# adelacvg/NS2VC

Measured on AMD Instinct MI355X. Metric: denoiser-steps/sec (10s@24kHz Vocos latent, bs32), higher is better.
Workload: dtype fp16; 1 GPU; 10 s utterance (T=938 Vocos frames), batch 32/GPU, prompt Lp=469, 20-step unipc order 2, hipGraph-captured loop, fp16 MFMA operands; timed job = set_condition + 20 steps; global_batch=32, frames=938, prompt_frames=469, solver=unipc, parallelism=dp1

## Files before the change

### include/ns2vc_hip.h

```cpp
#ifndef NS2VC_HIP_H
#define NS2VC_HIP_H

#include <stddef.h>
#include <stdint.h>

#ifdef __cplusplus
extern "C" {
#endif

#define NS2VC_ABI_VERSION 7
#define NS2VC_MAX_LEVELS 8
#define NS2VC_NCOEF 12

typedef struct ns2vc_unet ns2vc_unet;

typedef struct ns2vc_unet_cfg {
  int32_t latent_channels;
  int32_t content_channels;
  int32_t n_levels;
  int32_t block_out_channels[NS2VC_MAX_LEVELS];
  int32_t norm_num_groups;
  int32_t cross_attention_dim;
  int32_t heads;
  int32_t layers_per_block;
// ... 34 lines not shown
int ns2vc_unet_set_condition(ns2vc_unet* h, const float* content_bct, const float* prompt_blc, const uint8_t* mask_bl, void* stream);
int ns2vc_unet_set_content(ns2vc_unet* h, const float* content_bct, void* stream);
int ns2vc_unet_set_prompt(ns2vc_unet* h, const float* prompt_blc, const uint8_t* mask_bl, void* stream);
int ns2vc_unet_set_mask(ns2vc_unet* h, const uint8_t* mask_bl, void* stream);
int ns2vc_unet_set_lengths(ns2vc_unet* h, const int32_t* lengths_b, void* stream);
int ns2vc_unet_set_prompt_lengths(ns2vc_unet* h, const int32_t* plens_b, void* stream);

int ns2vc_unet_forward(ns2vc_unet* h, const float* x_bct, const float* t_b, float* out_bct, void* stream);

int ns2vc_sampler_load(ns2vc_unet* h, int steps, const float* coef_host);
int ns2vc_sampler_load_items(ns2vc_unet* h, int n_tables, const int32_t* table_rows, const float* coef_host, int n_items, const int32_t* item_table,
                             const int32_t* item_start, void* stream);
int ns2vc_sampler_run(ns2vc_unet* h, float* x_inout_bct, int use_graph, void* stream);
int ns2vc_sampler_begin(ns2vc_unet* h, const float* x_T_bct, void* stream);
int ns2vc_sampler_steps(ns2vc_unet* h, int n_steps, int use_graph, void* stream);
int ns2vc_sampler_end(ns2vc_unet* h, float* x_out_bct, void* stream);
int ns2vc_sampler_handoff(ns2vc_unet* dst, ns2vc_unet* src, void* stream);
int ns2vc_sampler_set_seeds(ns2vc_unet* h, const uint64_t* seeds_b, void* stream);
int ns2vc_sampler_set_guidance(ns2vc_unet* h, const float* scale_host, int n, void* stream);
int ns2vc_sampler_set_x0_correction(ns2vc_unet* h, int mode, float ratio, float max_val);
int ns2vc_sampler_peek(ns2vc_unet* h, float* x_out_bct, void* stream);
int ns2vc_unet_attn_fallbacks(ns2vc_unet* h, unsigned long long* count, int reset, void* stream);
int ns2vc_unet_gn_coop_alone(ns2vc_unet* h, unsigned long long* count, int reset, void* stream);
int ns2vc_unet_graph_captures(ns2vc_unet* h, unsigned long long* count);

int ns2vc_unet_set_debug(ns2vc_unet* h, int enable);
int ns2vc_unet_num_taps(ns2vc_unet* h);
int ns2vc_unet_tap_info(ns2vc_unet* h, int idx, char* name, int buflen, int* rows, int* cols);
int ns2vc_unet_tap_read(ns2vc_unet* h, int idx, float* host_dst);
int ns2vc_unet_num_launches(ns2vc_unet* h, int* per_forward, int* per_condition);
int ns2vc_unet_op_info(ns2vc_unet* h, int which, int idx, char* name, int buflen, int* kind, double* flops, double* bytes);
int ns2vc_unet_profile_forward(ns2vc_unet* h, float* ms, int n_ms, int reps, void* stream);

int ns2vc_dev_malloc(void** out, size_t bytes);
int ns2vc_dev_free(void* p);
int ns2vc_memcpy_h2d(void* dst, const void* src, size_t bytes);
int ns2vc_memcpy_d2h(void* dst, const void* src, size_t bytes);
int ns2vc_dev_sync(void);
int ns2vc_stream_create(void** out);
int ns2vc_stream_destroy(void* stream);
int ns2vc_stream_sync(void* stream);
int ns2vc_stream_create_cu_mask(void** out, const uint32_t* mask_words, int n_words);
int ns2vc_event_create(void** out);
int ns2vc_event_destroy(void* ev);
int ns2vc_event_record(void* ev, void* stream);
int ns2vc_event_elapsed_ms(void* start, void* stop, float* ms);

typedef struct ns2vc_gemm_args {
  const void* a0; const void* a1;
  int32_t lda0, lda1, c0, c1;
  int32_t B, Tin, Tout, M;
  int32_t taps, tmode;
  const void* w; int32_t K;
  int32_t N;
  const float* bias;
  const float* res; int32_t ldres;
  int32_t geglu;
  float* out_f32; int32_t ldo_f32;
  void* out_op; int32_t ldo_op;
  long long* stats;
  const void* a2; int32_t lda2, c2;
  float* rowstats;
  const float* ln_stats; const float* ln_wsum; float ln_eps; int32_t ln_dim;
  unsigned* ln_health;
  const float* gnp_x; int32_t gnp_ldx;
  const long long* gnp_stats; const float* gnp_gamma; const float* gnp_beta;
  const float* gnp_temb; int32_t gnp_ldtemb;
  float gnp_eps; int32_t gnp_G, gnp_silu;
  unsigned* gnp_sync;
  unsigned* gnp_alone;
  const float* gnp_x1; int32_t gnp_ldx1, gnp_c1;
  const long long* gnp_stats1;
  void* gnp_raw;
  int32_t algo;
  const void* w_tiled;
  const float* sol_coef; const int32_t* sol_step; int32_t sol_ncoef;
  float* sol_xe; void* sol_xe_op; float* sol_xbar; float* sol_d1; float* sol_mprev; int32_t sol_ld;
  int32_t conv_bn;
  int32_t gnp_pair, sol_op_pair;
  const int32_t* lens;
} ns2vc_gemm_args;

typedef struct ns2vc_attn_args {
  const void* q; const void* k; const void* v;
  int32_t ldq, ldk, ldv;
  int32_t B, H, Lq, Lk;
  const float* bias;
  float scale;
  void* out; int32_t ldo;
  int32_t pv_fp8;
  int32_t exact_only;
  unsigned* fallbacks;
  const int32_t* q_lens;
  const int32_t* k_lens;
} ns2vc_attn_args;

typedef struct ns2vc_ffn_args {
  const void* yn; int32_t ldy;
  const float* ln_stats; float ln_eps;
  const void* wstream; const float* consts; const float* bias2;
  const float* res; int32_t ldres;
  float* out_f32; int32_t ldo_f32;
  void* out_op; int32_t ldo_op;
  long long* stats;
  int32_t B, T, M, dim;
  unsigned* ln_health;
  const void* pre_a; int32_t pre_lda;
  const float* pre_bias;
  const float* pre_res; int32_t pre_ldres;
  const void* att_q; int32_t att_ldq;
  const void* att_kv; const float* att_bias; float att_scale; int32_t att_Lk;
  const int32_t* lens;
} ns2vc_ffn_args;
int ns2vc_pack_ffn(const float* w1_packed_host, const float* w2f_host, int dim, int precision, void** out_stream_dev);
int ns2vc_pack_ffn_pre(const float* w1_packed_host, const float* w2f_host, const float* w0_host, int dim, int precision, void** out_stream_dev);
int ns2vc_k_ffn(const ns2vc_ffn_args* a, int precision, void* stream);
size_t ns2vc_xattn_pack_bytes(int B, int Lk, int hd);
int ns2vc_k_xattn_pack(const void* k, int ldk, const void* v, int ldv, int B, int Lk, int hd, void* out, int precision, void* stream);

typedef struct ns2vc_geglu_args {
  const void* yn; int32_t ldy;
  const float* ln_stats; float ln_eps;
  const void* wstream; const float* consts;
  void* out_op; int32_t ldo;
  int32_t M, dim;
  unsigned* ln_health;
  int32_t T;
  const int32_t* lens;
} ns2vc_geglu_args;
int ns2vc_pack_geglu(const float* w1_packed_host, const float* bias1_packed_host, int dim, int precision, void** out_stream_dev, float** out_consts_dev);
int ns2vc_k_geglu(const ns2vc_geglu_args* a, int precision, void* stream);
int ns2vc_pack_geglu_host(const float* w1_packed_host, const float* bias1_packed_host, int dim, int precision, uint16_t* stream_out, float* consts_out);

typedef struct ns2vc_rowchain_args {
  const void* a_op; int32_t lda;
  const void* wstream; const float* bias1; const float* consts2;
  const float* res; int32_t ldres;
  float* out1_f32; int32_t ldo1;
  void* out2_op; int32_t ldo2;
  float ln_eps; int32_t M, dim, n2;
  unsigned* ln_health;
  const float* gn_x; int32_t ldx;
  const long long* gn_stats; const float* gn_gamma; const float* gn_beta;
  float gn_eps; int32_t T, G;
  int32_t slices;
  const int32_t* lens;
} ns2vc_rowchain_args;
int ns2vc_pack_rowchain(const float* w1_host, const float* w2_host, int dim, int n2, int precision, void** out_stream_dev);
int ns2vc_pack_rowchain_sliced(const float* w1_host, const float* w2_host, int dim, int n2, int slices, int precision, void** out_stream_dev);
int ns2vc_k_rowchain(const ns2vc_rowchain_args* a, int precision, void* stream);
int ns2vc_debug_set_geglu_min_rows(int rows);
int ns2vc_debug_set_attn_keys(int keys);
int ns2vc_debug_set_attn_optimistic(int on);
int ns2vc_debug_set_rowchain_tokens(int nt);

int ns2vc_to_operand(const float* host, size_t n, int precision, void** out_dev);
int ns2vc_from_operand(const void* dev, size_t n, int precision, float* host);
int ns2vc_round_to_operand(const float* host_in, size_t n, int precision, float* host_out);
int ns2vc_pack_weight(const float* rows_host, int N, int K, int precision, void** out_dev);
int ns2vc_k_gemm(const ns2vc_gemm_args* a, int precision, void* stream);
int ns2vc_pack_conv3_tiled(const float* rows_host, int N, int ctot, int c2, int precision, void** out_dev);
int ns2vc_weight_rowsum(const float* rows_host, int N, int K, int precision, float** out_dev);
int ns2vc_debug_set_gemm_trace(void* dev_u64_blocks_x8);
int ns2vc_debug_poison(unsigned pattern, int lds_bytes, void* stream);
int ns2vc_debug_placement(void* stream, int n_blocks, int spin, uint32_t* out_host);
int ns2vc_debug_kernel_table(int family, int* rows, int* unready);
int ns2vc_debug_set_gemm_tile(int bm, int bn, int stages);
int ns2vc_k_attention(const ns2vc_attn_args* a, int head_dim, int precision, void* stream);
int ns2vc_k_groupnorm(const float* a0, int lda0, int c0, const float* a1, int lda1, int c1, int B, int T, int G, float eps,
                      const float* gamma, const float* beta, const float* temb, int ldtemb, int temb_off, int silu,
                      void* out_op, void* raw_op, int precision, void* stream);
int ns2vc_k_groupnorm_stats(const float* a0, int lda0, int c0, const long long* stats0, int B, int T, int G, float eps, const float* gamma,
                            const float* beta, const float* temb, int ldtemb, int temb_off, int silu, void* out_op, int precision, void* stream);
int ns2vc_k_groupnorm_stats2(const float* a0, int lda0, int c0, const long long* stats0, const float* a1, int lda1, int c1, const long long* stats1,
                             int B, int T, int G, float eps, const float* gamma, const float* beta, const float* temb, int ldtemb, int temb_off,
                             int silu, void* out_op, void* raw_op, int precision, void* stream);
int ns2vc_k_layernorm_apply(const float* x, int ldx, int M, int C, float eps, void* out_op, int precision, void* stream);
int ns2vc_k_nct_to_btc(const float* src, int C, int T, int B, float* dst, int ldd, int cpad, void* stream);
int ns2vc_k_btc_to_nct(const float* src, int lds, int C, int T, int B, float* dst, void* stream);
int ns2vc_k_noise(const uint64_t* seeds_dev, int B, int C, int T, int ld, int step, const int32_t* lens_dev, float* out, void* stream);
int ns2vc_k_solver_update(const float* coef_dev, const int32_t* step_dev, const float* x0, float* xe, void* xe_op, int precision, float* xbar,
                          float* d1, float* mprev, float* mprev2, size_t n, int ld, void* stream);
int ns2vc_k_solver_update_guided(const float* coef_dev, const int32_t* step_dev, const float* x0, float* xe, void* xe_op, int precision, float* xbar,
                                 float* d1, float* mprev, float* mprev2, size_t n_half, int ld, const float* scale_dev, int T, const uint64_t* seeds_dev,
                                 const int32_t* lens_dev, int nc, void* stream);
int ns2vc_k_abs_quantile(const float* values, int n_items, int T, int ld, int nc, const int32_t* lens_dev, float p, float* thr, void* stream);
int ns2vc_k_solver_update_corrected(const float* coef_dev, const int32_t* step_dev, const float* x0, float* xe, void* xe_op, int precision, float* xbar,
                                    float* d1, float* mprev, float* mprev2, size_t n, int ld, int T, const float* scale_dev, const int32_t* lens_dev,
                                    int nc, int mode, float ratio, float max_val, float* thr_dev, void* stream);
int ns2vc_k_solver_update_items(const float* coef_dev, int n_rows, const int32_t* step_dev, const int32_t* items_host, int n_items, const float* x0, float* xe,
                                void* xe_op, int precision, float* xbar, float* d1, float* mprev, float* mprev2, size_t n, int ld, int T,
                                const float* scale_dev, const uint64_t* seeds_dev, const int32_t* lens_dev, int nc, int mode, float ratio, float max_val,
                                float* thr_dev, void* stream);

int ns2vc_sampler_open(ns2vc_unet* h, int history2, int noise, void* stream);
int ns2vc_sampler_rebase(ns2vc_unet* h, void* stream);
int ns2vc_sampler_write_rows(ns2vc_unet* h, int row0, int nrows, const float* coef_host, void* stream);
int ns2vc_sampler_admit(ns2vc_unet* h, int n, const int32_t* slots, const float* x_T_nct, const int32_t* records, void* stream);
int ns2vc_sampler_take(ns2vc_unet* h, int n, const int32_t* slots, float* x_out_nct, void* stream);
int ns2vc_sampler_slot_step(ns2vc_unet* h, int* loop_step);
int ns2vc_unet_set_condition_items(ns2vc_unet* h, int n, const int32_t* slots, const float* content_nct, const float* prompt_nlc, const uint8_t* mask_nl,
                                   void* stream);
int ns2vc_k_sampler_admit(const float* x_T, int C, int T, int n, const int32_t* slots_host, int n_items, float* xe, void* xe_op, int precision, float* xbar,
                          float* d1, float* mprev, float* mprev2, int ld, const int32_t* lens_dev, int guided, void* stream);
int ns2vc_k_sampler_take(const float* xe, int ld, int C, int T, int n, const int32_t* slots_host, int n_items, float* out, void* stream);

#ifdef __cplusplus
}
#endif
#endif
```

### ns2vc_amd/_lib.py

```python
from __future__ import annotations

import ctypes as C
import os
from typing import Optional

_HERE = os.path.dirname(os.path.abspath(__file__))
LIB_PATH = os.path.join(_HERE, "lib", "libns2vc_hip.so")
NCOEF = 12
MAX_LEVELS = 8
PREC_F32, PREC_BF16, PREC_F16 = 0, 1, 2
ABI_VERSION = 7


class Ns2vcError(RuntimeError):
    pass


class UnetCfg(C.Structure):
    _fields_ = [
        ("latent_channels", C.c_int32), ("content_channels", C.c_int32), ("n_levels", C.c_int32),
        ("block_out_channels", C.c_int32 * MAX_LEVELS), ("norm_num_groups", C.c_int32),
        ("cross_attention_dim", C.c_int32), ("heads", C.c_int32), ("layers_per_block", C.c_int32),
        ("pool_heads", C.c_int32),
    ]
# ... 32 lines not shown
class FfnArgs(C.Structure):
    _fields_ = [
        ("yn", C.c_void_p), ("ldy", C.c_int32),
        ("ln_stats", C.c_void_p), ("ln_eps", C.c_float),
        ("wstream", C.c_void_p), ("consts", C.c_void_p), ("bias2", C.c_void_p),
        ("res", C.c_void_p), ("ldres", C.c_int32),
        ("out_f32", C.c_void_p), ("ldo_f32", C.c_int32),
        ("out_op", C.c_void_p), ("ldo_op", C.c_int32),
        ("stats", C.c_void_p),
        ("B", C.c_int32), ("T", C.c_int32), ("M", C.c_int32), ("dim", C.c_int32),
        ("ln_health", C.c_void_p),
        ("pre_a", C.c_void_p), ("pre_lda", C.c_int32),
        ("pre_bias", C.c_void_p),
        ("pre_res", C.c_void_p), ("pre_ldres", C.c_int32),
        ("att_q", C.c_void_p), ("att_ldq", C.c_int32),
        ("att_kv", C.c_void_p), ("att_bias", C.c_void_p), ("att_scale", C.c_float), ("att_Lk", C.c_int32),
        ("lens", C.c_void_p),
    ]


class GegluArgs(C.Structure):
    _fields_ = [
        ("yn", C.c_void_p), ("ldy", C.c_int32),
        ("ln_stats", C.c_void_p), ("ln_eps", C.c_float),
        ("wstream", C.c_void_p), ("consts", C.c_void_p),
        ("out_op", C.c_void_p), ("ldo", C.c_int32),
        ("M", C.c_int32), ("dim", C.c_int32),
        ("ln_health", C.c_void_p),
        ("T", C.c_int32), ("lens", C.c_void_p),
    ]


class RowchainArgs(C.Structure):
    _fields_ = [
        ("a_op", C.c_void_p), ("lda", C.c_int32),
        ("wstream", C.c_void_p), ("bias1", C.c_void_p), ("consts2", C.c_void_p),
        ("res", C.c_void_p), ("ldres", C.c_int32),
        ("out1_f32", C.c_void_p), ("ldo1", C.c_int32),
        ("out2_op", C.c_void_p), ("ldo2", C.c_int32),
        ("ln_eps", C.c_float), ("M", C.c_int32), ("dim", C.c_int32), ("n2", C.c_int32),
        ("ln_health", C.c_void_p),
        ("gn_x", C.c_void_p), ("ldx", C.c_int32),
        ("gn_stats", C.c_void_p), ("gn_gamma", C.c_void_p), ("gn_beta", C.c_void_p),
        ("gn_eps", C.c_float), ("T", C.c_int32), ("G", C.c_int32),
        ("slices", C.c_int32),
        ("lens", C.c_void_p),
    ]


class AttnArgs(C.Structure):
    _fields_ = [
        ("q", C.c_void_p), ("k", C.c_void_p), ("v", C.c_void_p),
        ("ldq", C.c_int32), ("ldk", C.c_int32), ("ldv", C.c_int32),
        ("B", C.c_int32), ("H", C.c_int32), ("Lq", C.c_int32), ("Lk", C.c_int32),
        ("bias", C.c_void_p), ("scale", C.c_float),
        ("out", C.c_void_p), ("ldo", C.c_int32),
        ("pv_fp8", C.c_int32), ("exact_only", C.c_int32), ("fallbacks", C.c_void_p),
        ("q_lens", C.c_void_p), ("k_lens", C.c_void_p),
    ]


_P = C.c_void_p
_PP = C.POINTER(C.c_void_p)
_I = C.c_int
PROTOTYPES = {
    "ns2vc_abi_version": (_I, []),
    "ns2vc_sizeof_gemm_args": (_I, []),
    "ns2vc_sizeof_attn_args": (_I, []),
    "ns2vc_sizeof_rowchain_args": (_I, []),
    "ns2vc_sizeof_ffn_args": (_I, []),
    "ns2vc_sizeof_geglu_args": (_I, []),
    "ns2vc_last_error": (C.c_char_p, []),
    "ns2vc_device_count": (_I, [C.POINTER(_I)]),
    "ns2vc_set_device": (_I, [_I]),
    "ns2vc_device_xcd_round_robin": (_I, [C.POINTER(_I)]),
    "ns2vc_device_name": (_I, [C.c_char_p, _I]),
    "ns2vc_unet_create": (_I, [C.POINTER(UnetCfg), _PP]),
    "ns2vc_unet_destroy": (_I, [_P]),
    "ns2vc_unet_load_weight": (_I, [_P, C.c_char_p, _P, C.POINTER(C.c_int64), _I]),
    "ns2vc_unet_finalize_weights": (_I, [_P, _I]),
    "ns2vc_unet_num_missing_weights": (_I, [_P, C.c_char_p, _I]),
    "ns2vc_unet_prepare": (_I, [_P, _I, _I, _I]),
    "ns2vc_unet_workspace_bytes": (_I, [_P, C.POINTER(C.c_size_t)]),
    "ns2vc_unet_set_condition": (_I, [_P, _P, _P, _P, _P]),
    "ns2vc_unet_set_content": (_I, [_P, _P, _P]),
    "ns2vc_unet_set_prompt": (_I, [_P, _P, _P, _P]),
    "ns2vc_unet_set_mask": (_I, [_P, _P, _P]),
    "ns2vc_unet_set_lengths": (_I, [_P, _P, _P]),
    "ns2vc_unet_set_prompt_lengths": (_I, [_P, _P, _P]),
    "ns2vc_unet_forward": (_I, [_P, _P, _P, _P, _P]),
    "ns2vc_sampler_load": (_I, [_P, _I, C.POINTER(C.c_float)]),
    "ns2vc_sampler_load_items": (_I, [_P, _I, _P, C.POINTER(C.c_float), _I, _P, _P, _P]),
    "ns2vc_sampler_run": (_I, [_P, _P, _I, _P]),
    "ns2vc_sampler_begin": (_I, [_P, _P, _P]),
    "ns2vc_sampler_steps": (_I, [_P, _I, _I, _P]),
    "ns2vc_sampler_end": (_I, [_P, _P, _P]),
    "ns2vc_sampler_handoff": (_I, [_P, _P, _P]),
    "ns2vc_sampler_peek": (_I, [_P, _P, _P]),
    "ns2vc_sampler_set_seeds": (_I, [_P, _P, _P]),
    "ns2vc_sampler_set_guidance": (_I, [_P, _P, _I, _P]),
    "ns2vc_sampler_set_x0_correction": (_I, [_P, _I, C.c_float, C.c_float]),
    "ns2vc_unet_attn_fallbacks": (_I, [_P, C.POINTER(C.c_ulonglong), _I, _P]),
    "ns2vc_unet_gn_coop_alone": (_I, [_P, C.POINTER(C.c_ulonglong), _I, _P]),
    "ns2vc_unet_graph_captures": (_I, [_P, C.POINTER(C.c_ulonglong)]),
    "ns2vc_unet_set_debug": (_I, [_P, _I]),
    "ns2vc_unet_set_option": (_I, [_P, C.c_char_p, _I]),
    "ns2vc_unet_ln_ratio": (_I, [_P, C.POINTER(C.c_float), _P]),
    "ns2vc_unet_ln_ratio_post": (_I, [_P, _P]),
    "ns2vc_unet_ln_ratio_poll": (_I, [_P, C.POINTER(C.c_float), C.POINTER(_I)]),
    "ns2vc_unet_num_taps": (_I, [_P]),
    "ns2vc_unet_tap_info": (_I, [_P, _I, C.c_char_p, _I, C.POINTER(_I), C.POINTER(_I)]),
    "ns2vc_unet_tap_read": (_I, [_P, _I, _P]),
    "ns2vc_unet_num_launches": (_I, [_P, C.POINTER(_I), C.POINTER(_I)]),
    "ns2vc_unet_op_info": (_I, [_P, _I, _I, C.c_char_p, _I, C.POINTER(_I), C.POINTER(C.c_double), C.POINTER(C.c_double)]),
    "ns2vc_unet_profile_forward": (_I, [_P, C.POINTER(C.c_float), _I, _I, _P]),
    "ns2vc_dev_malloc": (_I, [_PP, C.c_size_t]),
    "ns2vc_dev_free": (_I, [_P]),
    "ns2vc_memcpy_h2d": (_I, [_P, _P, C.c_size_t]),
    "ns2vc_memcpy_d2h": (_I, [_P, _P, C.c_size_t]),
    "ns2vc_dev_sync": (_I, []),
    "ns2vc_stream_create": (_I, [_PP]),
    "ns2vc_stream_create_cu_mask": (_I, [_PP, C.POINTER(C.c_uint32), _I]),
    "ns2vc_stream_destroy": (_I, [_P]),
    "ns2vc_stream_sync": (_I, [_P]),
    "ns2vc_event_create": (_I, [_PP]),
    "ns2vc_event_destroy": (_I, [_P]),
    "ns2vc_event_record": (_I, [_P, _P]),
    "ns2vc_event_elapsed_ms": (_I, [_P, _P, C.POINTER(C.c_float)]),
    "ns2vc_pack_weight": (_I, [_P, _I, _I, _I, _PP]),
    "ns2vc_k_gemm": (_I, [C.POINTER(GemmArgs), _I, _P]),
    "ns2vc_pack_conv3_tiled": (_I, [_P, _I, _I, _I, _I, _PP]),
    "ns2vc_weight_rowsum": (_I, [_P, _I, _I, _I, _PP]),
    "ns2vc_debug_set_gemm_trace": (_I, [_P]),
    "ns2vc_debug_set_gemm_tile": (_I, [_I, _I, _I]),
    "ns2vc_debug_kernel_table": (_I, [_I, C.POINTER(C.c_int), C.POINTER(C.c_int)]),
    "ns2vc_debug_placement": (_I, [_P, _I, _I, C.POINTER(C.c_uint32)]),
    "ns2vc_debug_poison": (_I, [C.c_uint, _I, _P]),
    "ns2vc_k_attention": (_I, [C.POINTER(AttnArgs), _I, _I, _P]),
    "ns2vc_pack_ffn": (_I, [_P, _P, _I, _I, _PP]),
    "ns2vc_pack_ffn_pre": (_I, [_P, _P, _P, _I, _I, _PP]),
    "ns2vc_xattn_pack_bytes": (C.c_size_t, [_I, _I, _I]),
    "ns2vc_k_xattn_pack": (_I, [_P, _I, _P, _I, _I, _I, _I, _P, _I, _P]),
    "ns2vc_k_ffn": (_I, [C.POINTER(FfnArgs), _I, _P]),
    "ns2vc_pack_geglu": (_I, [_P, _P, _I, _I, _PP, _PP]),
    "ns2vc_k_geglu": (_I, [C.POINTER(GegluArgs), _I, _P]),
    "ns2vc_pack_geglu_host": (_I, [_P, _P, _I, _I, _P, _P]),
    "ns2vc_debug_set_geglu_min_rows": (_I, [_I]),
    "ns2vc_pack_rowchain": (_I, [_P, _P, _I, _I, _I, _PP]),
    "ns2vc_pack_rowchain_sliced": (_I, [_P, _P, _I, _I, _I, _I, _PP]),
    "ns2vc_k_rowchain": (_I, [C.POINTER(RowchainArgs), _I, _P]),
    "ns2vc_debug_set_rowchain_tokens": (_I, [_I]),
    "ns2vc_debug_set_attn_keys": (_I, [_I]),
    "ns2vc_debug_set_attn_optimistic": (_I, [_I]),
    "ns2vc_k_groupnorm_stats": (_I, [_P, _I, _I, _P, _I, _I, _I, C.c_float, _P, _P, _P, _I, _I, _I, _P, _I, _P]),
    "ns2vc_k_groupnorm_stats2": (_I, [_P, _I, _I, _P, _P, _I, _I, _P, _I, _I, _I, C.c_float, _P, _P, _P, _I, _I, _I, _P, _P, _I, _P]),
    "ns2vc_k_groupnorm": (_I, [_P, _I, _I, _P, _I, _I, _I, _I, _I, C.c_float, _P, _P, _P, _I, _I, _I, _P, _P, _I, _P]),
    "ns2vc_k_layernorm_apply": (_I, [_P, _I, _I, _I, C.c_float, _P, _I, _P]),
    "ns2vc_to_operand": (_I, [_P, C.c_size_t, _I, _PP]),
    "ns2vc_from_operand": (_I, [_P, C.c_size_t, _I, _P]),
    "ns2vc_round_to_operand": (_I, [_P, C.c_size_t, _I, _P]),
    "ns2vc_k_nct_to_btc": (_I, [_P, _I, _I, _I, _P, _I, _I, _P]),
    "ns2vc_k_btc_to_nct": (_I, [_P, _I, _I, _I, _I, _P, _P]),
    "ns2vc_k_noise": (_I, [_P, _I, _I, _I, _I, _I, _P, _P, _P]),
    "ns2vc_k_solver_update": (_I, [_P, _P, _P, _P, _P, _I, _P, _P, _P, _P, C.c_size_t, _I, _P]),
    "ns2vc_k_solver_update_guided": (_I, [_P, _P, _P, _P, _P, _I, _P, _P, _P, _P, C.c_size_t, _I, _P, _I, _P, _P, _I, _P]),
    "ns2vc_k_abs_quantile": (_I, [_P, _I, _I, _I, _I, _P, C.c_float, _P, _P]),
    "ns2vc_k_solver_update_corrected": (_I, [_P, _P, _P, _P, _P, _I, _P, _P, _P, _P, C.c_size_t, _I, _I, _P, _P, _I, _I, C.c_float, C.c_float, _P, _P]),
    "ns2vc_k_solver_update_items": (_I, [_P, _I, _P, _P, _I, _P, _P, _P, _I, _P, _P, _P, _P, C.c_size_t, _I, _I, _P, _P, _P, _I, _I, C.c_float, C.c_float,
                                         _P, _P]),
    "ns2vc_sampler_open": (_I, [_P, _I, _I, _P]),
    "ns2vc_sampler_rebase": (_I, [_P, _P]),
    "ns2vc_sampler_write_rows": (_I, [_P, _I, _I, C.POINTER(C.c_float), _P]),
    "ns2vc_sampler_admit": (_I, [_P, _I, _P, _P, _P, _P]),
    "ns2vc_sampler_take": (_I, [_P, _I, _P, _P, _P]),
    "ns2vc_sampler_slot_step": (_I, [_P, C.POINTER(_I)]),
    "ns2vc_unet_set_condition_items": (_I, [_P, _I, _P, _P, _P, _P, _P]),
    "ns2vc_k_sampler_admit": (_I, [_P, _I, _I, _I, _P, _I, _P, _P, _I, _P, _P, _P, _P, _I, _P, _I, _P]),
    "ns2vc_k_sampler_take": (_I, [_P, _I, _I, _I, _I, _P, _I, _P, _P]),
}

_lib: Optional[C.CDLL] = None


def load(path: Optional[str] = None) -> C.CDLL:
    global _lib
    if _lib is not None and path is None:
        return _lib
    p = path or os.environ.get("NS2VC_LIB") or LIB_PATH
    if not os.path.exists(p):
        raise Ns2vcError(f"{p} not found: the HIP engine is not built. Run __graft_entry__.build() "
                         f"(or `make -C ns2vc_amd/csrc`). There is no CPU fallback.")
    try:
        import torch
    except Exception:
        pass
    lib = C.CDLL(p)
    for name, (res, args) in PROTOTYPES.items():
        fn = getattr(lib, name)
        fn.restype = res
        fn.argtypes = args
    if lib.ns2vc_abi_version() != ABI_VERSION:
        raise Ns2vcError(f"ABI version mismatch: library reports {lib.ns2vc_abi_version()}, binding expects {ABI_VERSION}")
    if lib.ns2vc_sizeof_gemm_args() != C.sizeof(GemmArgs):
        raise Ns2vcError(f"ns2vc_gemm_args: library has {lib.ns2vc_sizeof_gemm_args()} bytes, binding {C.sizeof(GemmArgs)}")
    if lib.ns2vc_sizeof_attn_args() != C.sizeof(AttnArgs):
        raise Ns2vcError(f"ns2vc_attn_args: library has {lib.ns2vc_sizeof_attn_args()} bytes, binding {C.sizeof(AttnArgs)}")
    if lib.ns2vc_sizeof_rowchain_args() != C.sizeof(RowchainArgs):
        raise Ns2vcError(f"ns2vc_rowchain_args: library has {lib.ns2vc_sizeof_rowchain_args()} bytes, binding {C.sizeof(RowchainArgs)}")
    if lib.ns2vc_sizeof_ffn_args() != C.sizeof(FfnArgs):
        raise Ns2vcError(f"ns2vc_ffn_args: library has {lib.ns2vc_sizeof_ffn_args()} bytes, binding {C.sizeof(FfnArgs)}")
    if lib.ns2vc_sizeof_geglu_args() != C.sizeof(GegluArgs):
        raise Ns2vcError(f"ns2vc_geglu_args: library has {lib.ns2vc_sizeof_geglu_args()} bytes, binding {C.sizeof(GegluArgs)}")
    if path is None:
        _lib = lib
    return lib


def check(rc: int, what: str = "") -> None:
    if rc != 0:
        msg = load().ns2vc_last_error()
        raise Ns2vcError(f"{what}: {msg.decode() if msg else 'unknown error'}")
```

### ns2vc_amd/csrc/abi_kernels.cpp

```cpp
#include "engine_internal.h"
#include "kernel_table.h"

#include <algorithm>
#include <cstring>
#include <mutex>

using namespace ns2vc;

hipError_t ns2vc::init_all_attributes() {
  hipError_t e = init_gemm_attributes();
  if (e == hipSuccess) e = init_convts_attributes();
  if (e == hipSuccess) e = init_attn_attributes();
  if (e == hipSuccess) e = init_ffn_attributes();
  if (e == hipSuccess) e = init_geglu_attributes();
  if (e == hipSuccess) e = init_rowchain_attributes();
  return e;
}
static int init_attributes(hipError_t (*init)(), bool* once = nullptr) {
  if (once && *once) return 0;
  const hipError_t e = init();
  if (e != hipSuccess) return fail("kernel attribute setup failed: %s", hipGetErrorString(e));
  if (once) *once = true;
  return 0;
}
static int upload(const void* src, size_t bytes, void** out_dev) {
  void* d = nullptr;
  HIPCHK(hipMalloc(&d, std::max<size_t>(bytes, 1)));
  HIPCHK(hipMemcpy(d, src, bytes, hipMemcpyHostToDevice));
  *out_dev = d;
  return 0;
}
static int launched(hipError_t e, const char* what) { return e == hipSuccess ? 0 : fail("%s: %s", what, hipGetErrorString(e)); }
static int upload_u16(const std::vector<unsigned short>& v, void** out_dev) { return upload(v.data(), v.size() * 2, out_dev); }

int ns2vc::xcd_round_robin_of_current_device() {
  static std::mutex mu;
  static std::map<int, int> seen;
  int dev = 0;
  if (hipGetDevice(&dev) != hipSuccess) return -1;
  std::lock_guard<std::mutex> lock(mu);
  auto it = seen.find(dev);
  if (it != seen.end()) return it->second;
  const int r = probe_xcd_round_robin();
  seen[dev] = r;
  return r;
}

extern "C" {

int ns2vc_abi_version(void) { return NS2VC_ABI_VERSION; }
int ns2vc_sizeof_gemm_args(void) { return (int)sizeof(ns2vc_gemm_args); }
int ns2vc_sizeof_attn_args(void) { return (int)sizeof(ns2vc_attn_args); }
int ns2vc_sizeof_rowchain_args(void) { return (int)sizeof(ns2vc_rowchain_args); }
int ns2vc_sizeof_ffn_args(void) { return (int)sizeof(ns2vc_ffn_args); }
int ns2vc_sizeof_geglu_args(void) { return (int)sizeof(ns2vc_geglu_args); }
const char* ns2vc_last_error(void) { return g_err.c_str(); }

int ns2vc_device_count(int* out_count) {
  int n = 0;
  hipError_t e = hipGetDeviceCount(&n);
  if (e != hipSuccess) { *out_count = 0; return fail("hipGetDeviceCount: %s", hipGetErrorString(e)); }
  *out_count = n;
  return 0;
}
int ns2vc_set_device(int device) { HIPCHK(hipSetDevice(device)); return 0; }
int ns2vc_device_name(char* buf, int buflen) {
  hipDeviceProp_t p;
  int dev = 0;
  HIPCHK(hipGetDevice(&dev));
  HIPCHK(hipGetDeviceProperties(&p, dev));
  snprintf(buf, buflen, "%s|%s|CUs=%d|clock_khz=%d|mem_gb=%.1f", p.name, p.gcnArchName, p.multiProcessorCount, p.clockRate,
           (double)p.totalGlobalMem / 1e9);
  return 0;
}

int ns2vc_device_xcd_round_robin(int* out) {
  if (!out) return fail("null argument");
  *out = xcd_round_robin_of_current_device();
  return 0;
}

int ns2vc_dev_malloc(void** out, size_t bytes) { HIPCHK(hipMalloc(out, bytes ? bytes : 1)); return 0; }
int ns2vc_dev_free(void* p) { HIPCHK(hipFree(p)); return 0; }
int ns2vc_memcpy_h2d(void* dst, const void* src, size_t bytes) { HIPCHK(hipMemcpy(dst, src, bytes, hipMemcpyHostToDevice)); return 0; }
int ns2vc_memcpy_d2h(void* dst, const void* src, size_t bytes) { HIPCHK(hipMemcpy(dst, src, bytes, hipMemcpyDeviceToHost)); return 0; }
int ns2vc_dev_sync(void) { HIPCHK(hipDeviceSynchronize()); return 0; }
int ns2vc_stream_create(void** out) { hipStream_t s; HIPCHK(hipStreamCreateWithFlags(&s, hipStreamNonBlocking)); *out = s; return 0; }
int ns2vc_stream_create_cu_mask(void** out, const uint32_t* mask_words, int n_words) {
  if (!out || !mask_words || n_words <= 0) return fail("null argument");
  int dev = 0, cus = 0;
  HIPCHK(hipGetDevice(&dev));
  HIPCHK(hipDeviceGetAttribute(&cus, hipDeviceAttributeMultiprocessorCount, dev));
  if (n_words > (cus + 31) / 32) return fail("CU mask of %d words for a device with %d CUs (at most %d words)", n_words, cus, (cus + 31) / 32);
  bool any = false;
  for (int w = 0; w < n_words; ++w)
    for (int b = 0; b < 32; ++b)
      if (mask_words[w] >> b & 1u) {
        if (w * 32 + b >= cus) return fail("CU mask bit %d set, the device has %d CUs", w * 32 + b, cus);
        any = true;
      }
  if (!any) return fail("empty CU mask");
  hipStream_t s;
  HIPCHK(hipExtStreamCreateWithCUMask(&s, (uint32_t)n_words, mask_words));
  *out = s;
  return 0;
}
int ns2vc_stream_destroy(void* s) { HIPCHK(hipStreamDestroy((hipStream_t)s)); return 0; }
int ns2vc_stream_sync(void* s) { HIPCHK(hipStreamSynchronize((hipStream_t)s)); return 0; }
int ns2vc_event_create(void** out) { hipEvent_t e; HIPCHK(hipEventCreate(&e)); *out = e; return 0; }
int ns2vc_event_destroy(void* e) { HIPCHK(hipEventDestroy((hipEvent_t)e)); return 0; }
int ns2vc_event_record(void* e, void* s) { HIPCHK(hipEventRecord((hipEvent_t)e, (hipStream_t)s)); return 0; }
int ns2vc_event_elapsed_ms(void* a, void* b, float* ms) {
  HIPCHK(hipEventSynchronize((hipEvent_t)b));
  HIPCHK(hipEventElapsedTime(ms, (hipEvent_t)a, (hipEvent_t)b));
  return 0;
}

int ns2vc_pack_weight(const float* rows_host, int N, int K, int precision, void** out_dev) {
  if (!rows_host || !out_dev || N <= 0 || K <= 0) return fail("bad argument");
  static bool inited = false;
  if (init_attributes(init_all_attributes, &inited)) return 1;
  return ns2vc_to_operand(rows_host, (size_t)N * K, precision, out_dev);
}
int ns2vc_pack_conv3_tiled(const float* rows_host, int N, int ctot, int c2, int precision, void** out_dev) {
  if (!rows_host || !out_dev || N <= 0) return fail("bad argument");
  std::vector<unsigned char> img;
  if (pack_conv3_tiled(rows_host, N, ctot, c2, precision, img) != hipSuccess) return fail("pack_conv3_tiled: ctot / c2 must be multiples of the chunk (64 elements; 32 for fp32)");
  return upload(img.data(), img.size(), out_dev);
}
int ns2vc_weight_rowsum(const float* rows_host, int N, int K, int precision, float** out_dev) {
  if (!rows_host || !out_dev || N <= 0 || K <= 0) return fail("bad argument");
  const std::vector<float> ws = rounded_rowsum(rows_host, N, K, N, precision);
  return upload(ws.data(), ws.size() * sizeof(float), (void**)out_dev);
}
int ns2vc_debug_set_attn_optimistic(int on) {
  set_attn_optimistic(on);
  return 0;
}
int ns2vc_debug_set_gemm_trace(void* dev_u64_blocks_x8) {
  set_gemm_trace((unsigned long long*)dev_u64_blocks_x8);
  set_ffn_trace((unsigned long long*)dev_u64_blocks_x8);
  set_rc_trace((unsigned long long*)dev_u64_blocks_x8);
  set_ts_trace((unsigned long long*)dev_u64_blocks_x8);
  set_gg_trace((unsigned long long*)dev_u64_blocks_x8);
  return 0;
}
int ns2vc_debug_poison(unsigned pattern, int lds_bytes, void* stream) {
  static unsigned* sink = nullptr;
  if (lds_bytes < 4 || lds_bytes > 160 * 1024) return fail("poison: LDS bytes out of range");
  if (!sink) HIPCHK(hipMalloc((void**)&sink, 64));
  return launched(launch_poison(pattern, lds_bytes & ~3, sink, (hipStream_t)stream), "launch_poison");
}
int ns2vc_debug_placement(void* stream, int n_blocks, int spin, uint32_t* out_host) {
  if (!out_host || n_blocks <= 0 || n_blocks > (1 << 20)) return fail("bad argument");
  unsigned* d = nullptr;
  HIPCHK(hipMalloc((void**)&d, (size_t)n_blocks * 2 * sizeof(unsigned)));
  hipError_t e = launch_placement(d, n_blocks, spin, (hipStream_t)stream);
  if (e == hipSuccess) e = hipStreamSynchronize((hipStream_t)stream);
  if (e == hipSuccess) e = hipMemcpy(out_host, d, (size_t)n_blocks * 2 * sizeof(unsigned), hipMemcpyDeviceToHost);
  (void)hipFree(d);
  if (e != hipSuccess) return fail("placement probe: %s", hipGetErrorString(e));
  return 0;
}
int ns2vc_debug_set_gemm_tile(int bm, int bn, int stages) { set_forced_gemm_tile(bm, bn, stages); return 0; }
int ns2vc_debug_kernel_table(int family, int* rows, int* unready) {
  static const struct { const KernelTable& (*table)(); hipError_t (*init)(); } fam[] = {
      {gemm2_kernel_table, init_gemm_attributes}, {gemm4_kernel_table, init_gemm_attributes}, {conv3ts_kernel_table, init_convts_attributes},
      {attn_kernel_table, init_attn_attributes},  {ffn_kernel_table, init_ffn_attributes},    {geglu_kernel_table, init_geglu_attributes},
      {rowchain_kernel_table, init_rowchain_attributes}};
  constexpr int NF = (int)(sizeof(fam) / sizeof(fam[0]));
  if (family < 0 || family >= NF || !rows) return fail("kernel table: family 0 .. %d, rows not NULL", NF - 1);
  const KernelTable& t = fam[family].table();
  *rows = t.n;
  if (!unready) return 0;
  if (init_attributes(fam[family].init)) return 1;
  *unready = 0;
  for (int i = 0; i < t.n; ++i) {
    hipFuncAttributes fa;
    HIPCHK(hipFuncGetAttributes(&fa, t.rows[i].fn));
    if (fa.maxDynamicSharedSizeBytes < (int)t.rows[i].lds || t.rows[i].lds > 160 * 1024) ++*unready;
  }
  return 0;
}
int ns2vc_k_gemm(const ns2vc_gemm_args* a, int precision, void* stream) {
  if (!a) return fail("null args");
  hipError_t e = launch_gemm(*a, precision, (hipStream_t)stream);
  if (e != hipSuccess) {
    const int line = last_gemm_refusal_line();
    if (line) return fail("launch_gemm: %s (refused by the argument check at gemm.hip:%d)", hipGetErrorString(e), line);
    return fail("launch_gemm: %s", hipGetErrorString(e));
  }
  return 0;
}
int ns2vc_pack_ffn(const float* w1_packed_host, const float* w2f_host, int dim, int precision, void** out_stream_dev) {
  if (!w1_packed_host || !w2f_host || !out_stream_dev) return fail("null argument");
  static bool inited = false;
  if (init_attributes(init_ffn_attributes, &inited)) return 1;
  std::vector<unsigned short> st;
  if (pack_ffn_stream(w1_packed_host, w2f_host, nullptr, dim, precision, st) != hipSuccess) return fail("ffn: dim must be 128 or 256 and the precision 16-bit");
  return upload_u16(st, out_stream_dev);
}
int ns2vc_pack_ffn_pre(const float* w1_packed_host, const float* w2f_host, const float* w0_host, int dim, int precision, void** out_stream_dev) {
  if (!w1_packed_host || !w2f_host || !w0_host || !out_stream_dev) return fail("null argument");
  if (init_attributes(init_ffn_attributes)) return 1;
  std::vector<unsigned short> st;
  if (pack_ffn_stream(w1_packed_host, w2f_host, w0_host, dim, precision, st) != hipSuccess) return fail("ffn: dim must be 128 or 256 and the precision 16-bit");
  return upload_u16(st, out_stream_dev);
}
int ns2vc_pack_rowchain(const float* w1_host, const float* w2_host, int dim, int n2, int precision, void** out_stream_dev) {
  if (!w1_host || !w2_host || !out_stream_dev) return fail("null argument");
  static bool inited = false;
  if (init_attributes(init_rowchain_attributes, &inited)) return 1;
  std::vector<unsigned short> st;
  if (pack_rowchain_stream(w1_host, w2_host, dim, n2, precision, st) != hipSuccess)
    return fail("rowchain: dim must be 128, 256 or 384, n2 = dim or 3 dim, and the precision 16-bit");
  return upload_u16(st, out_stream_dev);
}
int ns2vc_pack_rowchain_sliced(const float* w1_host, const float* w2_host, int dim, int n2, int slices, int precision, void** out_stream_dev) {
  if (!w1_host || !w2_host || !out_stream_dev) return fail("null argument");
  static bool inited = false;
  if (init_attributes(init_rowchain_attributes, &inited)) return 1;
  std::vector<unsigned short> st;
  if (pack_rowchain_stream(w1_host, w2_host, dim, n2, precision, st, slices) != hipSuccess)
    return fail("rowchain (sliced): dim 384, n2 = dim or 3 dim, 2 slices, 16-bit precision");
  return upload_u16(st, out_stream_dev);
}
int ns2vc_debug_set_attn_keys(int keys) {
  if (keys != 0 && keys != 64 && keys != 128) return fail("attention K/V tile: 0 (heuristic), 64 or 128 keys");
  set_forced_attn_keys(keys);
  return 0;
}
int ns2vc_debug_set_rowchain_tokens(int nt) {
  if (nt < 0 || nt > 2) return fail("rowchain tokens: 0 (heuristic), 1 (64-token blocks) or 2 (128-token blocks)");
  set_forced_rowchain_tokens(nt);
  return 0;
}
int ns2vc_k_rowchain(const ns2vc_rowchain_args* a, int precision, void* stream) {
  if (!a) return fail("null args");
  return launched(launch_rowchain(*a, precision, (hipStream_t)stream), "launch_rowchain");
}
size_t ns2vc_xattn_pack_bytes(int B, int Lk, int hd) { return xattn_pack_bytes(B, Lk, hd); }
int ns2vc_k_xattn_pack(const void* k, int ldk, const void* v, int ldv, int B, int Lk, int hd, void* out, int precision, void* stream) {
  hipError_t e = launch_xattn_pack(k, ldk, v, ldv, B, Lk, hd, out, precision, (hipStream_t)stream);
  if (e != hipSuccess) return fail("xattn_pack: %s (16-bit precisions, head dim 16 | 32, 8 heads, 16-byte aligned k rows)", hipGetErrorString(e));
  return 0;
}
int ns2vc_k_ffn(const ns2vc_ffn_args* a, int precision, void* stream) {
  if (!a) return fail("null args");
  return launched(launch_ffn(*a, precision, (hipStream_t)stream), "launch_ffn");
}
int ns2vc_pack_geglu(const float* w1_packed_host, const float* bias1_packed_host, int dim, int precision, void** out_stream_dev, float** out_consts_dev) {
  if (!w1_packed_host || !out_stream_dev || !out_consts_dev) return fail("null argument");
  if (init_attributes(init_geglu_attributes)) return 1;
  std::vector<unsigned short> st;
  std::vector<float> cs;
  if (pack_geglu_stream(w1_packed_host, bias1_packed_host, dim, precision, st, cs) != hipSuccess) return fail("geglu: dim must be 384 and the precision 16-bit");
  if (upload_u16(st, out_stream_dev)) return 1;
  return upload(cs.data(), cs.size() * 4, (void**)out_consts_dev);
}
int ns2vc_debug_set_geglu_min_rows(int rows) { g_geglu_min_rows = rows < 0 ? 4608 : rows; return 0; }
int ns2vc_pack_geglu_host(const float* w1_packed_host, const float* bias1_packed_host, int dim, int precision, uint16_t* stream_out, float* consts_out) {
  if (!w1_packed_host || !stream_out || !consts_out) return fail("null argument");
  std::vector<unsigned short> st;
  std::vector<float> cs;
  if (pack_geglu_stream(w1_packed_host, bias1_packed_host, dim, precision, st, cs) != hipSuccess) return fail("geglu: dim must be 384 and the precision 16-bit");
  memcpy(stream_out, st.data(), st.size() * 2);
  memcpy(consts_out, cs.data(), cs.size() * 4);
  return 0;
}
int ns2vc_k_geglu(const ns2vc_geglu_args* a, int precision, void* stream) {
  if (!a) return fail("null args");
  return launched(launch_geglu(*a, precision, (hipStream_t)stream), "launch_geglu");
}
int ns2vc_k_attention(const ns2vc_attn_args* a, int head_dim, int precision, void* stream) {
  if (!a) return fail("null args");
  if (a->q_lens || a->k_lens) {
    if (a->B <= 0) return fail("attention: B=%d", a->B);
    std::vector<int32_t> host((size_t)a->B);
    HIPCHK(hipStreamSynchronize((hipStream_t)stream));
    const struct { const int32_t* dev; int max; const char* name; } tabs[2] = {{a->q_lens, a->Lq, "q_lens"}, {a->k_lens, a->Lk, "k_lens"}};
    for (const auto& t : tabs) {
      if (!t.dev) continue;
      HIPCHK(hipMemcpy(host.data(), t.dev, host.size() * sizeof(int32_t), hipMemcpyDeviceToHost));
      for (int b = 0; b < a->B; ++b)
        if (host[b] < 1 || host[b] > t.max) return fail("attention: %s[%d]=%d outside 1..%d", t.name, b, host[b], t.max);
    }
  }
  return launched(launch_attention(*a, head_dim, precision, (hipStream_t)stream), "launch_attention");
}
int ns2vc_k_groupnorm(const float* a0, int lda0, int c0, const float* a1, int lda1, int c1, int B, int T, int G, float eps,
                      const float* gamma, const float* beta, const float* temb, int ldtemb, int temb_off, int silu, void* out_op,
                      void* raw_op, int precision, void* stream) {
  const int rows = 32, nchunk = (T + rows - 1) / rows;
  double* part = nullptr;
  HIPCHK(hipMalloc((void**)&part, (size_t)B * nchunk * G * 2 * sizeof(double)));
  hipError_t e = launch_gn_partial(a0, lda0, c0, a1, lda1, c1, B, T, G, part, nchunk, rows, (hipStream_t)stream);
  if (e == hipSuccess)
    e = launch_gn_apply(a0, lda0, c0, a1, lda1, c1, B, T, G, eps, part, nchunk, nullptr, nullptr, gamma, beta, temb, ldtemb, temb_off, silu,
                        out_op, raw_op, precision, (hipStream_t)stream);
  hipError_t e2 = hipStreamSynchronize((hipStream_t)stream);
  (void)hipFree(part);
  if (e != hipSuccess) return fail("groupnorm launch: %s", hipGetErrorString(e));
  if (e2 != hipSuccess) return fail("groupnorm sync: %s", hipGetErrorString(e2));
  return 0;
}
int ns2vc_k_groupnorm_stats(const float* a0, int lda0, int c0, const long long* stats0, int B, int T, int G, float eps, const float* gamma,
                            const float* beta, const float* temb, int ldtemb, int temb_off, int silu, void* out_op, int precision, void* stream) {
  if (!stats0 || (c0 % G) || ((c0 / G) & 15)) return fail("groupnorm_stats: needs the int64 epilogue statistics and groups of whole 16-channel blocks");
  return launched(launch_gn_apply(a0, lda0, c0, nullptr, 0, 0, B, T, G, eps, nullptr, 0, stats0, nullptr, gamma, beta, temb, ldtemb, temb_off, silu,
                                 out_op, nullptr, precision, (hipStream_t)stream), "groupnorm_stats launch");
}
int ns2vc_k_groupnorm_stats2(const float* a0, int lda0, int c0, const long long* stats0, const float* a1, int lda1, int c1, const long long* stats1,
                             int B, int T, int G, float eps, const float* gamma, const float* beta, const float* temb, int ldtemb, int temb_off,
                             int silu, void* out_op, void* raw_op, int precision, void* stream) {
  if (!stats0 || !a1 || !stats1 || (c0 & 15) || (c1 & 15) || ((c0 + c1) % G) || (((c0 + c1) / G) & 15))
    return fail("groupnorm_stats2: needs both sources' int64 epilogue statistics, whole 16-channel blocks per source and per group");
  return launched(launch_gn_apply(a0, lda0, c0, a1, lda1, c1, B, T, G, eps, nullptr, 0, stats0, stats1, gamma, beta, temb, ldtemb, temb_off, silu,
                                 out_op, raw_op, precision, (hipStream_t)stream), "groupnorm_stats2 launch");
}
int ns2vc_k_layernorm_apply(const float* x, int ldx, int M, int C, float eps, void* out_op, int precision, void* stream) {
  return launched(launch_ln_apply_op(x, ldx, M, C, eps, out_op, precision, (hipStream_t)stream), "ln_apply launch");
}
int ns2vc_to_operand(const float* host, size_t n, int precision, void** out_dev) {
  if (!host || !out_dev) return fail("null argument");
  if (precision == NS2VC_PREC_F32) return upload(host, n * 4, out_dev);
  std::vector<uint16_t> q(n);
  for (size_t i = 0; i < n; ++i) q[i] = f32_to_op16_bits(host[i], precision);
  return upload(q.data(), n * 2, out_dev);
}
int ns2vc_round_to_operand(const float* host_in, size_t n, int precision, float* host_out) {
  if (!host_in || !host_out) return fail("null argument");
  if (precision != NS2VC_PREC_F32 && precision != NS2VC_PREC_BF16 && precision != NS2VC_PREC_F16) return fail("unknown precision %d", precision);
  for (size_t i = 0; i < n; ++i)
    host_out[i] = precision == NS2VC_PREC_F32 ? host_in[i] : op16_bits_to_f32(f32_to_op16_bits(host_in[i], precision), precision);
  return 0;
}
int ns2vc_from_operand(const void* dev, size_t n, int precision, float* host) {
  if (!dev || !host) return fail("null argument");
  HIPCHK(hipDeviceSynchronize());
  if (precision != NS2VC_PREC_F32) {
    std::vector<uint16_t> q(n);
    HIPCHK(hipMemcpy(q.data(), dev, n * 2, hipMemcpyDeviceToHost));
    for (size_t i = 0; i < n; ++i) host[i] = op16_bits_to_f32(q[i], precision);
  } else {
    HIPCHK(hipMemcpy(host, dev, n * 4, hipMemcpyDeviceToHost));
  }
  return 0;
}
int ns2vc_k_nct_to_btc(const float* src, int C, int T, int B, float* dst, int ldd, int cpad, void* stream) {
  return launched(launch_nct_to_btc(src, C, T, B, dst, nullptr, PREC_F32, ldd, cpad, (hipStream_t)stream), "nct_to_btc launch");
}
int ns2vc_k_btc_to_nct(const float* src, int lds, int C, int T, int B, float* dst, void* stream) {
  return launched(launch_btc_to_nct(src, lds, C, T, B, dst, (hipStream_t)stream), "btc_to_nct launch");
}
int ns2vc_k_solver_update(const float* coef_dev, const int32_t* step_dev, const float* x0, float* xe, void* xe_op, int precision, float* xbar,
                          float* d1, float* mprev, float* mprev2, size_t n, int ld, void* stream) {
  if (!coef_dev || !step_dev || !x0 || !xe || !xe_op || !xbar || !d1 || !mprev) return fail("null argument");
  if (ld <= 0 || (ld & 3) || n % (size_t)ld) return fail("n (%zu) must be a multiple of ld (%d), ld a multiple of 4", n, ld);
  return launched(launch_solver_update(coef_dev, step_dev, NS2VC_NCOEF, x0, xe, xe_op, precision, xbar, d1, mprev, n, (hipStream_t)stream,
                                      precision != PREC_F32 ? ld : 0, SolverNoise(), mprev2), "solver_update launch");
}
int ns2vc_k_solver_update_guided(const float* coef_dev, const int32_t* step_dev, const float* x0, float* xe, void* xe_op, int precision, float* xbar,
                                 float* d1, float* mprev, float* mprev2, size_t n_half, int ld, const float* scale_dev, int T, const uint64_t* seeds_dev,
                                 const int32_t* lens_dev, int nc, void* stream) {
  if (!coef_dev || !step_dev || !x0 || !xe || !xe_op || !xbar || !d1 || !mprev || !scale_dev) return fail("null argument");
  if (ld <= 0) return fail("ld (%d) must be positive", ld);
  SolverGuide gd;
  gd.scale = scale_dev; gd.T = T; gd.ld = ld;
  SolverNoise nz;
  if (seeds_dev) { nz.seeds = reinterpret_cast<const unsigned long long*>(seeds_dev); nz.lens = lens_dev; nz.T = T; nz.ld = ld; nz.nc = nc; }
  return launched(launch_solver_update(coef_dev, step_dev, NS2VC_NCOEF, x0, xe, xe_op, precision, xbar, d1, mprev, n_half, (hipStream_t)stream,
                                      precision != PREC_F32 ? ld : 0, nz, mprev2, gd), "guided solver_update launch");
}
int ns2vc_k_abs_quantile(const float* values, int n_items, int T, int ld, int nc, const int32_t* lens_dev, float p, float* thr, void* stream) {
  if (!values || !thr) return fail("null argument");
  QuantArgs q;
  q.v = values; q.lens = lens_dev; q.T = T; q.ld = ld; q.nc = nc; q.p = p;
  return launched(launch_abs_quantile(q, n_items, thr, (hipStream_t)stream), "abs_quantile launch");
}
int ns2vc_k_solver_update_corrected(const float* coef_dev, const int32_t* step_dev, const float* x0, float* xe, void* xe_op, int precision, float* xbar,
                                    float* d1, float* mprev, float* mprev2, size_t n, int ld, int T, const float* scale_dev, const int32_t* lens_dev,
                                    int nc, int mode, float ratio, float max_val, float* thr_dev, void* stream) {
// ... 116 lines not shown
```

### ns2vc_amd/csrc/attn.hip

```cpp
#include "common.h"
#include "mma.h"
#include "kernel_table.h"
#include <cstdlib>

namespace ns2vc {

template <typename T> struct AMma;
template <> struct AMma<float> {
  static constexpr int SZ = 4;
  __device__ static __forceinline__ void mma(f32x16_t& acc, const u32x4_t& a, const u32x4_t& b) {
    acc = __builtin_amdgcn_mfma_f32_32x32x2f32(__uint_as_float(a.x), __uint_as_float(b.x), acc, 0, 0, 0);
    acc = __builtin_amdgcn_mfma_f32_32x32x2f32(__uint_as_float(a.y), __uint_as_float(b.y), acc, 0, 0, 0);
    acc = __builtin_amdgcn_mfma_f32_32x32x2f32(__uint_as_float(a.z), __uint_as_float(b.z), acc, 0, 0, 0);
    acc = __builtin_amdgcn_mfma_f32_32x32x2f32(__uint_as_float(a.w), __uint_as_float(b.w), acc, 0, 0, 0);
  }
  __device__ static __forceinline__ f32x16_t mma0(const u32x4_t& a, const u32x4_t& b) {
    f32x16_t acc = __builtin_amdgcn_mfma_f32_32x32x2f32(__uint_as_float(a.x), __uint_as_float(b.x), f32x16_t{0.f, 0.f, 0.f, 0.f, 0.f, 0.f, 0.f, 0.f, 0.f, 0.f, 0.f, 0.f, 0.f, 0.f, 0.f, 0.f}, 0, 0, 0);
    acc = __builtin_amdgcn_mfma_f32_32x32x2f32(__uint_as_float(a.y), __uint_as_float(b.y), acc, 0, 0, 0);
    acc = __builtin_amdgcn_mfma_f32_32x32x2f32(__uint_as_float(a.z), __uint_as_float(b.z), acc, 0, 0, 0);
    acc = __builtin_amdgcn_mfma_f32_32x32x2f32(__uint_as_float(a.w), __uint_as_float(b.w), acc, 0, 0, 0);
    return acc;
  }
  __device__ static __forceinline__ int vpos(int key) { return key; }
};
template <typename TM> struct AMma16 {
  static constexpr int SZ = 2;
  __device__ static __forceinline__ void mma(f32x16_t& acc, const u32x4_t& a, const u32x4_t& b) { MmaT<TM>::mma(acc, a, b); }
  __device__ static __forceinline__ f32x16_t mma0(const u32x4_t& a, const u32x4_t& b) {
    f32x16_t acc = {0.f, 0.f, 0.f, 0.f, 0.f, 0.f, 0.f, 0.f, 0.f, 0.f, 0.f, 0.f, 0.f, 0.f, 0.f, 0.f};
    MmaT<TM>::mma(acc, a, b);
    return acc;
  }
  __device__ static __forceinline__ int vpos(int key) { return (key & ~12) | ((key & 4) << 1) | ((key & 8) >> 1); }
};
template <> struct AMma<bf16_t> : AMma16<bf16_t> {};
template <> struct AMma<f16_t> : AMma16<f16_t> {};

template <typename TM> __device__ __forceinline__ void vt_scatter(char* vp, int rowb, const u32x4_t& v);
template <> __device__ __forceinline__ void vt_scatter<float>(char* vp, int rowb, const u32x4_t& v) {
  *reinterpret_cast<uint32_t*>(vp) = v.x;
  *reinterpret_cast<uint32_t*>(vp + rowb) = v.y;
  *reinterpret_cast<uint32_t*>(vp + 2 * rowb) = v.z;
  *reinterpret_cast<uint32_t*>(vp + 3 * rowb) = v.w;
}
__device__ __forceinline__ void vt_scatter16(char* vp, int rowb, const u32x4_t& v) {
  *reinterpret_cast<uint16_t*>(vp) = (uint16_t)v.x;
  *reinterpret_cast<uint16_t*>(vp + rowb) = (uint16_t)(v.x >> 16);
  *reinterpret_cast<uint16_t*>(vp + 2 * rowb) = (uint16_t)v.y;
  *reinterpret_cast<uint16_t*>(vp + 3 * rowb) = (uint16_t)(v.y >> 16);
  *reinterpret_cast<uint16_t*>(vp + 4 * rowb) = (uint16_t)v.z;
  *reinterpret_cast<uint16_t*>(vp + 5 * rowb) = (uint16_t)(v.z >> 16);
  *reinterpret_cast<uint16_t*>(vp + 6 * rowb) = (uint16_t)v.w;
  *reinterpret_cast<uint16_t*>(vp + 7 * rowb) = (uint16_t)(v.w >> 16);
}
template <> __device__ __forceinline__ void vt_scatter<bf16_t>(char* vp, int rowb, const u32x4_t& v) { vt_scatter16(vp, rowb, v); }
template <> __device__ __forceinline__ void vt_scatter<f16_t>(char* vp, int rowb, const u32x4_t& v) { vt_scatter16(vp, rowb, v); }

__device__ __forceinline__ float half_max(float v) {
  const auto r = __builtin_amdgcn_permlane32_swap(__float_as_uint(v), __float_as_uint(v), false, false);
  return fmaxf(__uint_as_float(r[0]), __uint_as_float(r[1]));
}
__device__ __forceinline__ float half_sum(float v) {
  const auto r = __builtin_amdgcn_permlane32_swap(__float_as_uint(v), __float_as_uint(v), false, false);
  return __uint_as_float(r[0]) + __uint_as_float(r[1]);
}

template <typename TM> __device__ __forceinline__ float round_op(float x);
template <> __device__ __forceinline__ float round_op<float>(float x) { return x; }
template <> __device__ __forceinline__ float round_op<bf16_t>(float x) { return __uint_as_float(pack_bf16x2(0.f, x) & 0xffff0000u); }
template <> __device__ __forceinline__ float round_op<f16_t>(float x) { return f16_lo(pack_f16x2(x, 0.f)); }
template <typename TM> __device__ __forceinline__ u32x4_t aux_chunk(float e0, float e1);
template <> __device__ __forceinline__ u32x4_t aux_chunk<float>(float e0, float e1) { return u32x4_t{__float_as_uint(e0), __float_as_uint(e1), 0u, 0u}; }
template <> __device__ __forceinline__ u32x4_t aux_chunk<bf16_t>(float e0, float e1) { return u32x4_t{pack_bf16x2(e0, e1), 0u, 0u, 0u}; }
template <> __device__ __forceinline__ u32x4_t aux_chunk<f16_t>(float e0, float e1) { return u32x4_t{pack_f16x2(e0, e1), 0u, 0u, 0u}; }
template <typename TM> __device__ __forceinline__ TM op_from_float(float x);
template <> __device__ __forceinline__ float op_from_float<float>(float x) { return x; }
template <> __device__ __forceinline__ bf16_t op_from_float<bf16_t>(float x) { bf16_t r; r.v = (uint16_t)pack_bf16x2(x, 0.f); return r; }
template <> __device__ __forceinline__ f16_t op_from_float<f16_t>(float x) { f16_t r; r.v = (uint16_t)pack_f16x2(x, 0.f); return r; }

__device__ __forceinline__ uint32_t pack_fp8x4(float a, float b, float c, float d) {
  int v = __builtin_amdgcn_cvt_pk_fp8_f32(a, b, 0, false);
  v = __builtin_amdgcn_cvt_pk_fp8_f32(c, d, v, true);
  return (uint32_t)v;
}
typedef int i32x8_t __attribute__((ext_vector_type(8)));
#ifndef NS2VC_ATTN_OPT
#define NS2VC_ATTN_OPT 1
#endif
template <bool B> struct OptTag { static constexpr bool value = B; };
__device__ int g_attn_exact_only = 0;
__device__ __forceinline__ int vpos8(int key) { return ((key & 4) << 3) | ((key & 32) >> 1) | ((key & 24) >> 1) | (key & 3); }
template <typename TM, int HD, int KEYS, bool P8, bool MASKED = false>
__global__ __launch_bounds__(256) void attn_kernel(const AttnArgs a) {
  op_mode_init<TM>();
  static_assert(!P8 || (sizeof(TM) == 2 && KEYS == 64), "the fp8 PV path: 16-bit operand types, one 64-key tile per f8f6f4 MFMA");
  constexpr int NSUB = KEYS / 32;
  constexpr int SZ = AMma<TM>::SZ;
  constexpr int EPC = 16 / SZ;
  constexpr int NS = HD * SZ / 32;
  constexpr int KROWB = HD * SZ + 48;
  constexpr int VSZ = P8 ? 1 : SZ;
  constexpr int VROWB = KEYS * VSZ + 16;
  constexpr int HDX = (HD + 1 + 31) / 32 * 32;
  constexpr int DT = HDX / 32;
  constexpr int NSL = SZ;
  constexpr int KBYTES = KEYS * KROWB, VBYTES = HDX * VROWB;
  constexpr int STAGE = KBYTES + VBYTES;
  constexpr int PPR = HD * SZ / 16;
  constexpr int NPIECE = KEYS * PPR;
  constexpr int UPT = (NPIECE + 255) / 256;
  constexpr float THRESH = P8 ? 8.0f : 12.0f;
  extern __shared__ __attribute__((aligned(16))) char smem[];

  const int tid = threadIdx.x, lane = tid & 63, wave = tid >> 6;
  const int l31 = lane & 31, hi = lane >> 5;
  const int nqb = (a.Lq + 127) >> 7;
  int b, h, qb;
  {
    const int nwg = gridDim.x, bid = blockIdx.x;
    const int qn = nwg >> 3, rn = nwg & 7, xcd = bid & 7, idx = bid >> 3;
    const int swz = (xcd < rn ? xcd * (qn + 1) : rn * (qn + 1) + (xcd - rn) * qn) + idx;
    b = swz / (a.H * nqb);
    const int rem = swz - b * (a.H * nqb);
    h = rem / nqb;
    qb = rem - h * nqb;
  }
  const int q = qb * 128 + wave * 32 + l31;
  int Lqb = a.Lq, Lkb = a.Lk;
  if constexpr (MASKED) {
    if (a.q_lens) Lqb = min(max(a.q_lens[b], 0), a.Lq);
    if (a.k_lens) Lkb = min(max(a.k_lens[b], 1), a.Lk);
    if (qb * 128 >= Lqb) {
      if (q < a.Lq) {
        char* zp = reinterpret_cast<char*>(a.out) + ((size_t)(b * a.Lq + q) * a.ldo + h * HD) * SZ;
#pragma unroll
        for (int pc = hi; pc < PPR; pc += 2) *reinterpret_cast<u32x4_t*>(zp + pc * 16) = u32x4_t{0, 0, 0, 0};
      }
      return;
    }
  }
  const float LOG2E = 1.4426950408889634f;
  const float sc2 = a.scale * LOG2E;

  for (int i = tid * 16; i < 2 * STAGE; i += 256 * 16) *reinterpret_cast<u32x4_t*>(smem + i) = u32x4_t{0, 0, 0, 0};
  __syncthreads();
  for (int i = tid; i < 2 * KEYS; i += 256) {
    const int st = i / KEYS, key = i - st * KEYS;
    *reinterpret_cast<TM*>(smem + st * STAGE + key * KROWB + HD * SZ) = op_from_float<TM>(1.0f);
    if constexpr (P8) *reinterpret_cast<uint8_t*>(smem + st * STAGE + KBYTES + HD * VROWB + key) = (uint8_t)0x38;
    else *reinterpret_cast<TM*>(smem + st * STAGE + KBYTES + HD * VROWB + key * SZ) = op_from_float<TM>(1.0f);
  }

  u32x4_t qf[NS];
  {
    const TM* qp = reinterpret_cast<const TM*>(a.q) + ((size_t)(b * a.Lq + min(q, Lqb - 1)) * a.ldq + h * HD);
#pragma unroll
    for (int s = 0; s < NS; ++s) {
      const u32x4_t raw = *reinterpret_cast<const u32x4_t*>(qp + s * 2 * EPC + hi * EPC);
      if constexpr (SZ == 4) {
        qf[s] = u32x4_t{__float_as_uint(__uint_as_float(raw.x) * sc2), __float_as_uint(__uint_as_float(raw.y) * sc2),
                        __float_as_uint(__uint_as_float(raw.z) * sc2), __float_as_uint(__uint_as_float(raw.w) * sc2)};
      } else {
        auto sc = [&](uint32_t w) __attribute__((always_inline)) { return Op16<TM>::pack(Op16<TM>::lo(w) * sc2, Op16<TM>::hi(w) * sc2); };
        qf[s] = u32x4_t{sc(raw.x), sc(raw.y), sc(raw.z), sc(raw.w)};
      }
      if (q >= Lqb) qf[s] = u32x4_t{0, 0, 0, 0};
    }
  }
  float m_ref = 0.f;
  u32x4_t qaux = hi == 0 ? aux_chunk<TM>(-m_ref, 1.0f) : u32x4_t{0, 0, 0, 0};
  constexpr bool CINIT = HD == 16 && SZ == 2 && !P8;
  f32x16_t cinit;
#pragma unroll
  for (int r = 0; r < 16; ++r) cinit[r] = 0.f;

  const TM* kbase = reinterpret_cast<const TM*>(a.k) + (size_t)b * a.Lk * a.ldk + h * HD;
  const TM* vbase = reinterpret_cast<const TM*>(a.v) + (size_t)b * a.Lk * a.ldv + h * HD;
  const float* bias = a.bias ? a.bias + (size_t)b * a.Lk : nullptr;

  u32x4_t kraw[UPT], vraw[UPT];
  float braw = 0.f;
  auto load_tile = [&](int t) __attribute__((always_inline)) {
    const int key0 = t * KEYS;
#pragma unroll
    for (int i = 0; i < UPT; ++i) {
      const int u = tid + 256 * i;
      if (u < NPIECE) {
        {
          const int key = u / PPR, pc = u - key * PPR;
          const int kk = min(key0 + key, Lkb - 1);
          kraw[i] = *reinterpret_cast<const u32x4_t*>(kbase + (size_t)kk * a.ldk + pc * EPC);
        }
        {
          const int key = u % KEYS, pc = u / KEYS;
          const int kk = min(key0 + key, Lkb - 1);
          vraw[i] = *reinterpret_cast<const u32x4_t*>(vbase + (size_t)kk * a.ldv + pc * EPC);
        }
      }
    }
    if (tid < KEYS && bias) braw = bias[min(key0 + tid, Lkb - 1)];
  };
  auto store_tile = [&](int stage, int key0s) __attribute__((always_inline)) {
    char* Ks = smem + stage * STAGE;
    char* Vs = Ks + KBYTES;
#pragma unroll
    for (int i = 0; i < UPT; ++i) {
      const int u = tid + 256 * i;
      if (u < NPIECE) {
        {
          const int key = u / PPR, pc = u - key * PPR;
          *reinterpret_cast<u32x4_t*>(Ks + key * KROWB + pc * 16) = kraw[i];
        }
        {
          const int key = u % KEYS, pc = u / KEYS;
          if constexpr (P8) {
            const u32x4_t w = vraw[i];
            const uint32_t b0 = pack_fp8x4(Op16<TM>::lo(w.x), Op16<TM>::hi(w.x), Op16<TM>::lo(w.y), Op16<TM>::hi(w.y));
            const uint32_t b1 = pack_fp8x4(Op16<TM>::lo(w.z), Op16<TM>::hi(w.z), Op16<TM>::lo(w.w), Op16<TM>::hi(w.w));
            uint8_t* vp = reinterpret_cast<uint8_t*>(Vs + (pc * EPC) * VROWB + vpos8(key));
#pragma unroll
            for (int j = 0; j < 4; ++j) { vp[j * VROWB] = (uint8_t)(b0 >> (8 * j)); vp[(4 + j) * VROWB] = (uint8_t)(b1 >> (8 * j)); }
          } else {
            const int pos = (key & ~31) + AMma<TM>::vpos(key & 31);
            vt_scatter<TM>(Vs + (pc * EPC) * VROWB + pos * SZ, VROWB, vraw[i]);
          }
        }
      }
    }
    if (tid < KEYS) {
      const float bl = (key0s + tid < Lkb) ? (bias ? braw * LOG2E : 0.f) : -INFINITY;
      *reinterpret_cast<TM*>(Ks + tid * KROWB + HD * SZ + SZ) = op_from_float<TM>(bl);
    }
  };

  f32x16_t o[DT];
  const int ntile = (Lkb + KEYS - 1) / KEYS;
  constexpr bool OPT = NS2VC_ATTN_OPT && !P8 && sizeof(TM) == 2;
  constexpr float OPT_MARGIN = 4.0f;
  auto run = [&](auto optimistic, const bool compute) __attribute__((always_inline)) {
  constexpr bool O = decltype(optimistic)::value;
  if (compute) {
#pragma unroll
    for (int d = 0; d < DT; ++d)
#pragma unroll
      for (int r = 0; r < 16; ++r) o[d][r] = 0.f;
    m_ref = 0.f;
    qaux = hi == 0 ? aux_chunk<TM>(-m_ref, 1.0f) : u32x4_t{0, 0, 0, 0};
    if constexpr (CINIT) {
#pragma unroll
      for (int r = 0; r < 16; ++r) cinit[r] = 0.f;
    }
  }
  load_tile(0);
  __syncthreads();
  store_tile(0, 0);
  __syncthreads();

  for (int t = 0; t < ntile; ++t) {
    if (t + 1 < ntile) load_tile(t + 1);
    const char* Ks = smem + (t & 1) * STAGE;
    const char* Vs = Ks + KBYTES;
    if (compute) {

    f32x16_t s[NSUB];
    if (CINIT && !bias && (t + 1 < ntile || Lkb % KEYS == 0)) {
#pragma unroll
      for (int k2 = 0; k2 < NSUB; ++k2) {
        const char* kr = Ks + (k2 * 32 + l31) * KROWB + hi * 16;
        s[k2] = cinit;
#pragma unroll
        for (int sl = 0; sl < NS; ++sl) AMma<TM>::mma(s[k2], *reinterpret_cast<const u32x4_t*>(kr + sl * 32), qf[sl]);
      }
    } else {
#pragma unroll
    for (int k2 = 0; k2 < NSUB; ++k2) {
      const char* kr = Ks + (k2 * 32 + l31) * KROWB + hi * 16;
      s[k2] = AMma<TM>::mma0(*reinterpret_cast<const u32x4_t*>(kr + NS * 32), qaux);
#pragma unroll
      for (int sl = 0; sl < NS; ++sl) AMma<TM>::mma(s[k2], *reinterpret_cast<const u32x4_t*>(kr + sl * 32), qf[sl]);
    }
    }
    if (!O || t == 0) {
      float mx = s[0][0];
#pragma unroll
      for (int k2 = 0; k2 < NSUB; ++k2)
#pragma unroll
        for (int r = 0; r < 16; ++r) mx = fmaxf(mx, s[k2][r]);
      mx = half_max(mx);
      if (t == 0 || __any(mx > THRESH)) {
        float target = t == 0 ? mx : fmaxf(mx, 0.f);
        if (!(target > -INFINITY)) target = 0.f;
        if (O) target += OPT_MARGIN;
        const float m_new = round_op<TM>(m_ref + target);
        const float dsh = m_new - m_ref;
        if (t > 0) {
          const float alpha = __builtin_amdgcn_exp2f(-dsh);
#pragma unroll
          for (int d = 0; d < DT; ++d)
#pragma unroll
            for (int r = 0; r < 16; ++r) o[d][r] *= alpha;
        }
#pragma unroll
        for (int k2 = 0; k2 < NSUB; ++k2)
#pragma unroll
          for (int r = 0; r < 16; ++r) s[k2][r] -= dsh;
        m_ref = m_new;
        if (hi == 0) qaux = aux_chunk<TM>(-m_ref, 1.0f);
        if constexpr (CINIT) {
#pragma unroll
          for (int r = 0; r < 16; ++r) cinit[r] = -m_ref;
        }
      }
    }
#pragma unroll
    for (int k2 = 0; k2 < NSUB; ++k2)
#pragma unroll
      for (int r = 0; r < 16; ++r) s[k2][r] = __builtin_amdgcn_exp2f(s[k2][r]);

    if constexpr (P8) {
      i32x8_t pf;
#pragma unroll
      for (int v = 0; v < 8; ++v)
        pf[v] = (int)pack_fp8x4(s[v >> 2][4 * (v & 3) + 0], s[v >> 2][4 * (v & 3) + 1], s[v >> 2][4 * (v & 3) + 2], s[v >> 2][4 * (v & 3) + 3]);
#pragma unroll
      for (int d = 0; d < DT; ++d) {
        const char* vr = Vs + (d * 32 + l31) * VROWB + hi * 32;
        const u32x4_t v0 = *reinterpret_cast<const u32x4_t*>(vr), v1 = *reinterpret_cast<const u32x4_t*>(vr + 16);
        const i32x8_t vf = {(int)v0.x, (int)v0.y, (int)v0.z, (int)v0.w, (int)v1.x, (int)v1.y, (int)v1.z, (int)v1.w};
        o[d] = __builtin_amdgcn_mfma_scale_f32_32x32x64_f8f6f4(vf, pf, o[d], 0, 0, 0, 0x7f7f7f7f, 0, 0x7f7f7f7f);
      }
    } else {
#pragma unroll
    for (int k2 = 0; k2 < NSUB; ++k2) {
#pragma unroll
      for (int sl = 0; sl < NSL; ++sl) {
        u32x4_t pf;
        if constexpr (SZ == 4) {
          pf = u32x4_t{__float_as_uint(s[k2][4 * sl + 0]), __float_as_uint(s[k2][4 * sl + 1]),
                       __float_as_uint(s[k2][4 * sl + 2]), __float_as_uint(s[k2][4 * sl + 3])};
        } else {
          pf = u32x4_t{Op16<TM>::pack(s[k2][8 * sl + 0], s[k2][8 * sl + 1]), Op16<TM>::pack(s[k2][8 * sl + 2], s[k2][8 * sl + 3]),
                       Op16<TM>::pack(s[k2][8 * sl + 4], s[k2][8 * sl + 5]), Op16<TM>::pack(s[k2][8 * sl + 6], s[k2][8 * sl + 7])};
        }
#pragma unroll
        for (int d = 0; d < DT; ++d) {
          const u32x4_t vf = *reinterpret_cast<const u32x4_t*>(Vs + (d * 32 + l31) * VROWB + k2 * 32 * SZ + sl * 32 + hi * 16);
          AMma<TM>::mma(o[d], vf, pf);
        }
      }
    }
    }
    }
    if (t + 1 < ntile) store_tile((t + 1) & 1, (t + 1) * KEYS);
    __syncthreads();
  }
  };

  constexpr int LB = HD / 32, LR = ((HD % 32) / 8) * 4;
  static_assert(HD % 32 == 0 || HD % 32 == 16, "ones row must sit at row 0 or 16 of its 32-row block");
  if (OPT && !g_attn_exact_only && !a.exact_only) {
    run(OptTag<true>{}, true);
    const float lq = o[LB][LR];
    const int bad = (hi == 0 && q < Lqb && !(lq > 0.f && lq < 16384.f)) ? 1 : 0;
    const bool wave_bad = __any(bad) != 0;
    if (__syncthreads_or(bad)) {
      if (a.fallbacks && threadIdx.x == 0) atomicAdd(a.fallbacks, 1u);
      run(OptTag<false>{}, wave_bad);
    }
  } else {
    run(OptTag<false>{}, true);
  }

  const auto lsw = __builtin_amdgcn_permlane32_swap(__float_as_uint(o[LB][LR]), __float_as_uint(o[LB][LR]), false, false);
  const float l_tot = __uint_as_float(lsw[0]);
  const float inv = 1.0f / l_tot;
  TM* op = reinterpret_cast<TM*>(a.out) + ((size_t)(b * a.Lq + min(q, a.Lq - 1)) * a.ldo + h * HD);
  const bool padded = MASKED && q >= Lqb;
  if constexpr (SZ == 2) {
#pragma unroll
    for (int d = 0; d < DT; ++d)
#pragma unroll
      for (int gp = 0; gp < 2; ++gp) {
        if (d * 32 + 16 * gp < HD) {
          const uint32_t a0 = Op16<TM>::pack(o[d][8 * gp] * inv, o[d][8 * gp + 1] * inv), a1 = Op16<TM>::pack(o[d][8 * gp + 2] * inv, o[d][8 * gp + 3] * inv);
          const uint32_t b0 = Op16<TM>::pack(o[d][8 * gp + 4] * inv, o[d][8 * gp + 5] * inv), b1 = Op16<TM>::pack(o[d][8 * gp + 6] * inv, o[d][8 * gp + 7] * inv);
          const auto x0 = __builtin_amdgcn_permlane32_swap(a0, b0, false, false);
          const auto x1 = __builtin_amdgcn_permlane32_swap(a1, b1, false, false);
#if defined(NS2VC_ATTN_ABLATE_STORE)
          asm volatile("" :: "v"(x0[0]), "v"(x1[0]), "v"(x0[1]), "v"(x1[1]));
#else
          if (q < a.Lq) *reinterpret_cast<u32x4_t*>(op + d * 32 + 8 * (2 * gp + hi)) = padded ? u32x4_t{0, 0, 0, 0} : u32x4_t{x0[0], x1[0], x0[1], x1[1]};
#endif
        }
      }
  } else if (q < a.Lq) {
#pragma unroll
    for (int d = 0; d < DT; ++d)
#pragma unroll
      for (int gq = 0; gq < 4; ++gq) {
        const int d0 = d * 32 + 8 * gq + 4 * hi;
        if (d0 < HD) store_op4<TM>(op + d0, padded ? 0.f : o[d][4 * gq] * inv, padded ? 0.f : o[d][4 * gq + 1] * inv, padded ? 0.f : o[d][4 * gq + 2] * inv,
                                   padded ? 0.f : o[d][4 * gq + 3] * inv);
      }
  }
}

template <typename TM, int HD, int KEYS> static constexpr size_t attn_lds() {
  constexpr int SZ = AMma<TM>::SZ;
  constexpr int HDX = (HD + 1 + 31) / 32 * 32;
  return 2 * (size_t)(KEYS * (HD * SZ + 48) + HDX * (KEYS * SZ + 16));
}

#define NS2VC_ATTN_ROW(TM, PREC, HD, KEYS, FP8, MK) \
  {kernel_key(PREC, HD, KEYS, FP8, MK), reinterpret_cast<const void*>(attn_kernel<TM, HD, KEYS, FP8, MK>), (uint32_t)attn_lds<TM, HD, KEYS>(), 256}
#define NS2VC_ATTN_ROW2(TM, PREC, HD, KEYS) NS2VC_ATTN_ROW(TM, PREC, HD, KEYS, false, false), NS2VC_ATTN_ROW(TM, PREC, HD, KEYS, false, true)
#define NS2VC_ATTN_ROWS16(TM, PREC)                                                                                            \
  NS2VC_ATTN_ROW2(TM, PREC, 16, 64), NS2VC_ATTN_ROW2(TM, PREC, 16, 128), NS2VC_ATTN_ROW(TM, PREC, 16, 64, true, false),         \
  NS2VC_ATTN_ROW2(TM, PREC, 32, 64), NS2VC_ATTN_ROW2(TM, PREC, 32, 128), NS2VC_ATTN_ROW(TM, PREC, 32, 64, true, false),         \
  NS2VC_ATTN_ROW2(TM, PREC, 48, 64), NS2VC_ATTN_ROW(TM, PREC, 48, 64, true, false),                                             \
  NS2VC_ATTN_ROW2(TM, PREC, 64, 64), NS2VC_ATTN_ROW(TM, PREC, 64, 64, true, false)
static const KernelRow attn_rows[] = {
  NS2VC_ATTN_ROW2(float, PREC_F32, 16, 64), NS2VC_ATTN_ROW2(float, PREC_F32, 32, 64), NS2VC_ATTN_ROW2(float, PREC_F32, 48, 64), NS2VC_ATTN_ROW2(float, PREC_F32, 64, 64),
  NS2VC_ATTN_ROWS16(bf16_t, PREC_BF16),
  NS2VC_ATTN_ROWS16(f16_t, PREC_F16),
};
#undef NS2VC_ATTN_ROWS16
#undef NS2VC_ATTN_ROW2
#undef NS2VC_ATTN_ROW
static const KernelTable k_attn_table(attn_rows);
const KernelTable& attn_kernel_table() { return k_attn_table; }

static int g_force_keys = 0;
void set_forced_attn_keys(int keys) { g_force_keys = keys; }
void set_attn_optimistic(int on) { const int v = on ? 0 : 1; (void)hipMemcpyToSymbol(HIP_SYMBOL(g_attn_exact_only), &v, sizeof(v)); }

hipError_t init_attn_attributes() { return set_lds_all(k_attn_table); }

bool attention_masks_rows(const AttnArgs& a, int head_dim, int prec) {
  return find(k_attn_table, kernel_key(prec, head_dim, 64, a.pv_fp8 != 0, true)) != nullptr;
}

hipError_t launch_attention(const AttnArgs& a, int head_dim, int prec, hipStream_t s) {
  const int al = prec == PREC_F32 ? 3 : 7;
  if (!a.q || !a.k || !a.v || !a.out) return hipErrorInvalidValue;
  const bool masked = a.q_lens || a.k_lens, fp8 = a.pv_fp8 != 0;
  if (masked && !attention_masks_rows(a, head_dim, prec)) return hipErrorInvalidValue;
  if (a.Lq <= 0 || a.Lk <= 0 || (a.ldq & al) || (a.ldk & al) || (a.ldv & al) || (a.ldo & al)) return hipErrorInvalidValue;
  if (reinterpret_cast<uintptr_t>(a.out) & 15) return hipErrorInvalidValue;
  const int keys = !fp8 && g_force_keys == 128 && find(k_attn_table, kernel_key(prec, head_dim, 128, false, masked)) ? 128 : 64;
  const KernelRow* row = find(k_attn_table, kernel_key(prec, head_dim, keys, fp8, masked));
  if (!row) return hipErrorInvalidValue;
  return launch(*row, dim3(((a.Lq + 127) / 128) * a.H * a.B), s, a);
}

}
```

### ns2vc_amd/csrc/common.h

```cpp
#pragma once
#include <hip/hip_runtime.h>
#include <stdint.h>
#include <stddef.h>
#include <vector>
#include "../../include/ns2vc_hip.h"

namespace ns2vc {

typedef __attribute__((ext_vector_type(8))) __bf16 bf16x8_t;
typedef __attribute__((ext_vector_type(16))) float f32x16_t;
typedef __attribute__((ext_vector_type(4))) float f32x4_t;
typedef __attribute__((ext_vector_type(4))) unsigned int u32x4_t;

struct bf16_t { uint16_t v; };
struct f16_t { uint16_t v; };

__host__ __device__ inline uint16_t f32_to_bf16_bits(float f) {
  union { float f; uint32_t u; } x;
  x.f = f;
  uint32_t u = x.u;
  if ((u & 0x7fffffffu) > 0x7f800000u) return (uint16_t)((u >> 16) | 0x40);
  u += 0x7fffu + ((u >> 16) & 1u);
  return (uint16_t)(u >> 16);
}
// ... 94 lines not shown
template <> __device__ __forceinline__ void store_op4<f16_t>(f16_t* p, float a, float b, float c, float d) {
  *reinterpret_cast<uint2*>(p) = make_uint2(pack_f16x2(a, b), pack_f16x2(c, d));
}
#ifndef NS2VC_WT_STORES
#define NS2VC_WT_STORES 1
#endif
#ifndef NS2VC_WT_MODE
#define NS2VC_WT_MODE 1
#endif
#ifndef NS2VC_WT_MOD
#if NS2VC_WT_MODE == 2
#define NS2VC_WT_MOD "sc1 nt"
#elif NS2VC_WT_MODE == 3
#define NS2VC_WT_MOD "nt"
#elif NS2VC_WT_MODE == 4
#define NS2VC_WT_MOD "sc0 sc1"
#else
#define NS2VC_WT_MOD "sc1"
#endif
#endif
__device__ __forceinline__ void out_store16(void* p, uint32_t a, uint32_t b, uint32_t c, uint32_t d) {
#if NS2VC_WT_STORES
  const u32x4_t v = {a, b, c, d};
  asm volatile("global_store_dwordx4 %0, %1, off " NS2VC_WT_MOD "\n\ts_nop 1" ::"v"(p), "v"(v) : "memory");
#else
  *reinterpret_cast<uint4*>(p) = make_uint4(a, b, c, d);
#endif
}
__device__ __forceinline__ void out_store8(void* p, uint32_t a, uint32_t b) {
#if NS2VC_WT_STORES
  typedef unsigned u32x2_t __attribute__((ext_vector_type(2)));
  const u32x2_t v = {a, b};
  asm volatile("global_store_dwordx2 %0, %1, off " NS2VC_WT_MOD "\n\ts_nop 1" ::"v"(p), "v"(v) : "memory");
#else
  *reinterpret_cast<uint2*>(p) = make_uint2(a, b);
#endif
}
__device__ __forceinline__ void out_f4(float* p, float a, float b, float c, float d) {
  out_store16(p, __float_as_uint(a), __float_as_uint(b), __float_as_uint(c), __float_as_uint(d));
}
template <typename TM> __device__ __forceinline__ void out_op4(TM* p, float a, float b, float c, float d);
template <> __device__ __forceinline__ void out_op4<float>(float* p, float a, float b, float c, float d) { out_f4(p, a, b, c, d); }
template <> __device__ __forceinline__ void out_op4<bf16_t>(bf16_t* p, float a, float b, float c, float d) { out_store8(p, pack_bf16x2(a, b), pack_bf16x2(c, d)); }
template <> __device__ __forceinline__ void out_op4<f16_t>(f16_t* p, float a, float b, float c, float d) { out_store8(p, pack_f16x2(a, b), pack_f16x2(c, d)); }
template <typename TM> __device__ __forceinline__ void store_op2(TM* p, float a, float b);
template <> __device__ __forceinline__ void store_op2<float>(float* p, float a, float b) { *reinterpret_cast<float2*>(p) = make_float2(a, b); }
template <> __device__ __forceinline__ void store_op2<bf16_t>(bf16_t* p, float a, float b) { *reinterpret_cast<uint32_t*>(p) = pack_bf16x2(a, b); }
template <> __device__ __forceinline__ void store_op2<f16_t>(f16_t* p, float a, float b) { *reinterpret_cast<uint32_t*>(p) = pack_f16x2(a, b); }
#endif

__device__ __forceinline__ float fast_rcp(float x) { return __builtin_amdgcn_rcpf(x); }
__device__ __forceinline__ float silu_f(float v) { return v * fast_rcp(1.0f + __expf(-v)); }
__device__ __forceinline__ float erf_as(float x) {
  const float ax = fabsf(x);
  const float t = fast_rcp(1.0f + 0.3275911f * ax);
  float p = 1.061405429f;
  p = fmaf(p, t, -1.453152027f);
  p = fmaf(p, t, 1.421413741f);
  p = fmaf(p, t, -0.284496736f);
  p = fmaf(p, t, 0.254829592f);
  const float e = 1.0f - p * t * __expf(-ax * ax);
  return copysignf(e, x);
}
__device__ __forceinline__ float gelu_erf_f(float v) { return 0.5f * v * (1.0f + erf_as(v * 0.70710678118654752440f)); }

enum { TMODE_SAME = 0, TMODE_DOWN2 = 1, TMODE_UP2 = 2 };
enum { PRO_NONE = 0, PRO_BC = 1, PRO_ROW = 2 };

typedef ::ns2vc_gemm_args GemmArgs;
typedef ::ns2vc_attn_args AttnArgs;

enum Precision { PREC_F32 = 0, PREC_BF16 = 1, PREC_F16 = 2 };
inline size_t operand_bytes(int prec) { return prec == PREC_F32 ? 4 : 2; }
inline uint16_t f32_to_op16_bits(float v, int prec) { return prec == PREC_BF16 ? f32_to_bf16_bits(v) : f32_to_f16_bits(v); }
inline float op16_bits_to_f32(uint16_t b, int prec) { return prec == PREC_BF16 ? bf16_bits_to_f32(b) : f16_bits_to_f32(b); }
struct SolverCoef { float alpha, sigma, g0, g1, A, Bc, d1c, pc; };
__device__ __forceinline__ SolverCoef solver_coef(const float* __restrict__ c) { return SolverCoef{c[1], c[2], c[3], c[4], c[5], c[6], c[7], c[8]}; }
__device__ __forceinline__ float solver_m(const SolverCoef& k, float vx0, float vxe) {
  const float eps = (vxe - k.alpha * vx0) / k.sigma;
  return (vxe - k.sigma * eps) / k.alpha;
}
template <int TH> __device__ __forceinline__ float solver_correct(float m, float s) {
  const float c = fminf(fmaxf(m, -s), s);
  return TH == 1 ? c / s : c;
}
template <bool H2, int TH>
__device__ __forceinline__ void solver_elem(const SolverCoef& k, float s, float d2c, float vx0, float vxe, float vxb, float vd1, float vmp, float vmp2,
                                            float& oxb, float& od1, float& om) {
  float m = solver_m(k, vx0, vxe);
  if constexpr (TH != 0) m = solver_correct<TH>(m, s);
  const float x = vxb - k.g0 * vd1 - k.g1 * (m - vmp);
  oxb = k.A * x - k.Bc * m;
  od1 = H2 ? k.d1c * (vmp - m) + d2c * (vmp2 - m) : k.d1c * (vmp - m);
  om = m;
}
template <bool H2>
__device__ __forceinline__ float solver_xe(const SolverCoef& k, float pe, float oxb, float od1, float om, float vmp2) {
  return H2 ? oxb - k.pc * od1 - pe * (vmp2 - om) : oxb - k.pc * od1;
}
__device__ __forceinline__ void solver_upd(const SolverCoef& k, float vx0, float vxe, float vxb, float vd1, float vmp, float& oxe, float& oxb, float& od1, float& om) {
  solver_elem<false, 0>(k, 0.f, 0.f, vx0, vxe, vxb, vd1, vmp, 0.f, oxb, od1, om);
  oxe = solver_xe<false>(k, 0.f, oxb, od1, om, 0.f);
}

__device__ __forceinline__ float guided_x0(float x0u, float x0c, float s) { return s == 1.0f ? x0c : x0u + s * (x0c - x0u); }

__device__ __forceinline__ uint4 philox4x32_10(uint4 c, uint32_t k0, uint32_t k1) {
#pragma unroll
  for (int r = 0; r < 10; ++r) {
    if (r) { k0 += 0x9E3779B9u; k1 += 0xBB67AE85u; }
    const uint32_t lo0 = 0xD2511F53u * c.x, hi0 = __umulhi(0xD2511F53u, c.x);
    const uint32_t lo1 = 0xCD9E8D57u * c.z, hi1 = __umulhi(0xCD9E8D57u, c.z);
    c = make_uint4(hi1 ^ c.y ^ k0, lo1, hi0 ^ c.w ^ k1, lo0);
  }
  return c;
}
__device__ __forceinline__ void box_muller(uint32_t a, uint32_t b, float& z0, float& z1) {
  const float u1 = ((float)a + 1.0f) * 0x1p-32f;
  const float u2 = (float)b * 0x1p-32f;
  const float r = sqrtf(-2.0f * logf(u1));
  float sn, cs;
  sincosf(u2 * 6.2831853071795864769f, &sn, &cs);
  z0 = r * cs; z1 = r * sn;
}
__device__ __forceinline__ float4 philox_gauss4(unsigned long long seed, uint32_t t, uint32_t q, uint32_t step) {
  const uint4 x = philox4x32_10(make_uint4(t, q, step, 0u), (uint32_t)seed, (uint32_t)(seed >> 32));
  float4 z;
  box_muller(x.x, x.y, z.x, z.y);
  box_muller(x.z, x.w, z.z, z.w);
  return z;
}

struct SolverItem { int row0, steps, start, flags; };
constexpr int SOLVER_ITEM_HIST2 = 1;
constexpr int SOLVER_ITEM_NOISE = 2;
__device__ __forceinline__ int solver_item_row(const SolverItem& it, int r, bool& active) {
  const int j = r - it.start;
  active = j >= 0 && j < it.steps;
  return it.row0 + min(max(j, 0), it.steps - 1);
}

constexpr int SOLVER_ITEM_NEVER = 0x7fffffff;
__host__ __device__ __forceinline__ SolverItem solver_item_idle() { return SolverItem{0, 1, SOLVER_ITEM_NEVER, 0}; }

constexpr double GN_SUM_SCALE = 268435456.0;
constexpr double GN_SQ_SCALE = 65536.0;

hipError_t launch_gemm(const GemmArgs& g, int prec, hipStream_t s);
size_t xattn_pack_bytes(int B, int Lk, int hd);
hipError_t launch_xattn_pack(const void* k, int ldk, const void* v, int ldv, int B, int Lk, int hd, void* out, int prec, hipStream_t s);
bool gemm_masks_rows(const GemmArgs& g, int prec);
bool gemm_uses_convts(const GemmArgs& g, int prec);
int last_gemm_refusal_line();
hipError_t launch_attention(const AttnArgs& a, int head_dim, int prec, hipStream_t s);
bool attention_masks_rows(const AttnArgs& a, int head_dim, int prec);
hipError_t init_gemm_attributes();
bool convts_eligible(const GemmArgs& g, int prec);
int convts_default_bn(const GemmArgs& g);
int convts_bn_for(const GemmArgs& g, int bn128_min);
void set_convts_bn128_min(int wgs);
int convts_row_blocks(const GemmArgs& g);
hipError_t launch_convts(const GemmArgs& g, int prec, int bn, int nl, int ks, hipStream_t s);
hipError_t init_convts_attributes();
hipError_t pack_conv3_tiled(const float* rows, int N, int ctot, int c2, int prec, std::vector<unsigned char>& out);
void set_forced_gemm_tile(int bm, int bn, int stages);
void set_gemm_trace(unsigned long long* p);
hipError_t init_attn_attributes();
void set_forced_attn_keys(int keys);
hipError_t launch_ffn(const ::ns2vc_ffn_args& a, int prec, hipStream_t s);
bool ffn_eligible(int dim, int T, int prec);
bool ffn_masks_rows(const ::ns2vc_ffn_args& a, int prec);
hipError_t init_ffn_attributes();
hipError_t pack_ffn_stream(const float* w1p, const float* w2f, const float* w0, int dim, int prec, std::vector<unsigned short>& out);
void set_ffn_trace(unsigned long long* p);
bool geglu_eligible(int dim, int T, int prec);
hipError_t pack_geglu_stream(const float* w1p, const float* bias1p, int dim, int prec, std::vector<unsigned short>& stream, std::vector<float>& consts);
hipError_t launch_geglu(const ::ns2vc_geglu_args& a, int prec, hipStream_t s);
bool geglu_masks_rows(const ::ns2vc_geglu_args& a, int prec);
hipError_t init_geglu_attributes();
void set_gg_trace(unsigned long long* p);
void set_ts_trace(unsigned long long* p);
void set_attn_optimistic(int on);

hipError_t launch_gn_partial(const float* a0, int lda0, int c0, const float* a1, int lda1, int c1,
                             int B, int T, int G, double* partial, int nchunk, int rows_per_chunk, hipStream_t s);
hipError_t launch_gn_apply(const float* a0, int lda0, int c0, const float* a1, int lda1, int c1, int B, int T, int G, float eps,
                           const double* partial, int nchunk, const long long* st0, const long long* st1, const float* gamma,
                           const float* beta, const float* temb, int ldtemb, int temb_off, int silu, void* out_op, void* raw_op,
                           int prec, hipStream_t s, int pair = 0,
                           const int* lens = nullptr);
hipError_t launch_mask_rows(void* dst, size_t ldd_bytes, size_t row_bytes, int B, int T, const int* lens, hipStream_t s, const void* src = nullptr,
                            size_t lds_bytes = 0, int Tsrc = 0, int up = 0);
hipError_t launch_ln_apply_op(const float* x, int ldx, int M, int C, float eps, void* out_op, int prec, hipStream_t s);
hipError_t launch_cast_op(const float* x, size_t n, void* out_op, int prec, hipStream_t s, int split = 0);
hipError_t launch_time_embed(const float* t_ptr, int t_stride, const int* step_ptr, int coef_stride,
                             const float* w1t, const float* b1, const float* w2t, const float* b2,
                             const float* aug, float* emb, void* emb_act_op, int prec, int B, int tdim, int edim, hipStream_t s);
hipError_t launch_rowchain(const ::ns2vc_rowchain_args& a, int prec, hipStream_t s);
bool rowchain_eligible(int dim, int n2, int T, int prec);
bool rowchain_masks_rows(const ::ns2vc_rowchain_args& a, int prec);
hipError_t init_rowchain_attributes();
hipError_t pack_rowchain_stream(const float* w1, const float* w2, int dim, int n2, int prec, std::vector<unsigned short>& out, int slices = 1);
int rowchain_slice_blocks(int n2, int slices);
void set_rc_trace(unsigned long long* p);
void set_forced_rowchain_tokens(int nt);
hipError_t launch_emb_from_table(const float* table, const int* step_ptr, const float* aug, float* emb, void* emb_act_op, int prec, int B,
                                 int edim, hipStream_t s);
int probe_xcd_round_robin(unsigned* map8 = nullptr);
hipError_t launch_zero(void* p, size_t bytes, hipStream_t s, int* counter = nullptr);
hipError_t launch_copy16(const void* src, void* dst, size_t bytes, hipStream_t s);
hipError_t launch_poison(unsigned pattern, int lds_bytes, unsigned* sink, hipStream_t s);
hipError_t launch_nct_to_btc(const float* src, int C, int T, int B, float* dst_f32, void* dst_op, int prec, int ldd, int cpad, hipStream_t s,
                             int ldd_op = 0, int split = 0);
hipError_t launch_btc_to_nct(const float* src, int lds, int C, int T, int B, float* dst, hipStream_t s);
hipError_t launch_mask_bias(const uint8_t* mask, int n, float* bias, hipStream_t s);
hipError_t launch_prompt_bias(const uint8_t* mask, const int* plens, int B, int Lp, float* bias, hipStream_t s);
hipError_t launch_ln_apply(const float* x, int M, int C, float eps, const float* gamma, const float* beta,
                           float* out, int L, int Lout_stride_rows, hipStream_t s);
hipError_t launch_pool_cls(float* seq, int B, int L, int C, const float* pos, hipStream_t s, const int* plens = nullptr);
hipError_t launch_pool_attn(const float* qkv, int B, int L1, int C, int heads, float* pooled, hipStream_t s, const int* plens = nullptr);
hipError_t launch_pool_proj(const float* pooled, int B, int C, const float* wt, const float* b, int E,
                            const float* gamma, const float* beta, float eps, float* out, hipStream_t s);
struct SolverNoise { const unsigned long long* seeds = nullptr; const int* lens = nullptr; int T = 0, ld = 0, nc = 0; };
struct SolverGuide { const float* scale = nullptr; int T = 0, ld = 0; };
struct SolverCorrect { int mode = 0; const float* thr = nullptr; float max_val = 1.0f; int T = 0, ld = 0; };
struct QuantArgs {
  const float* v = nullptr; const float* xe = nullptr; const float* coef = nullptr; const int* step_ptr = nullptr; int ncoef = 0;
  const float* scale = nullptr; size_t half = 0; const int* lens = nullptr; int T = 0, ld = 0, nc = 0; float p = 0.995f;
};
hipError_t launch_abs_quantile(const QuantArgs& q, int n_items, float* thr, hipStream_t s);
hipError_t launch_solver_update(const float* coef, const int* step_ptr, int ncoef, const float* x0,
                                float* xe, void* xe_op, int prec, float* xbar, float* d1, float* mprev, size_t n, hipStream_t s,
                                int split = 0,
                                const SolverNoise& noise = SolverNoise(),
                                float* mprev2 = nullptr,
                                const SolverGuide& guide = SolverGuide(),
                                const SolverCorrect& correct = SolverCorrect());
struct SolverItems { const SolverItem* rec = nullptr; int T = 0, ld = 0; };
hipError_t launch_solver_update_items(const float* coef, const int* step_ptr, int ncoef, const SolverItems& items, const float* x0, float* xe, void* xe_op,
                                      int prec, float* xbar, float* d1, float* mprev, size_t n, hipStream_t s, int split, const SolverNoise& noise,
                                      float* mprev2, const SolverGuide& guide, const SolverCorrect& correct);
hipError_t launch_abs_quantile_items(const QuantArgs& q, const SolverItem* items, int n_items, float* thr, hipStream_t s);
hipError_t launch_emb_items_from_table(const float* table, const int* step_ptr, const SolverItem* items, int n_items, const float* aug, float* emb,
                                       void* emb_act_op, int prec, int B, int edim, hipStream_t s);
hipError_t launch_sampler_admit(const float* x_T, int C, int T, int n, const int* slots, int nslots, const SolverItem* rec_in, SolverItem* rec, float* xe,
                                void* xe_op, int prec, float* xbar, float* d1, float* mprev, float* mprev2, int ld, int split, const int* lens, int half,
                                hipStream_t s);
hipError_t launch_sampler_take(const float* xe, int ld, int C, int T, int n, const int* slots, int nslots, float* dst, SolverItem* rec, hipStream_t s);
hipError_t launch_condition_items(const float* content, int Cc, int T, const float* prompt, int Lp, int Cx, const uint8_t* mask, int n, const int* slots,
                                  int nslots, void* content_op, int prec, int split, float* content_f32, const int* lens, float* prompt_dst,
                                  uint8_t* mask_dst, hipStream_t s);
hipError_t launch_noise(const unsigned long long* seeds, int B, int nc, int T, int ld, int step, const int* lens, float* out, hipStream_t s);
hipError_t launch_fill_i32(int* p, int v, hipStream_t s);
hipError_t launch_placement(unsigned* dev_out, int n_blocks, int spin, hipStream_t s);
hipError_t launch_snapshot_u32(unsigned* src, unsigned* dst, hipStream_t s);

}
```

### ns2vc_amd/csrc/engine.cpp

```cpp
#include "engine_internal.h"

#include <algorithm>
#include <cstdlib>
#include <cstring>

using namespace ns2vc;

static int bind_device(ns2vc_unet* h) {
  int cur = -1;
  HIPCHK(hipGetDevice(&cur));
  if (cur != h->device) HIPCHK(hipSetDevice(h->device));
  return 0;
}
int ns2vc::check_ready(ns2vc_unet* h, bool need_plan) {
  if (!h) return fail("null engine handle");
  if (bind_device(h)) return 1;
  if (!h->finalized) return fail("weights not finalized (call ns2vc_unet_finalize_weights)");
  if (need_plan && !h->arena) return fail("engine not prepared (call ns2vc_unet_prepare)");
  return 0;
}

int ns2vc::load_state(ns2vc_unet* h, const float* x_bct, hipStream_t s, int items) {
  const int B = items > 0 ? items : h->B;
  HIPCHK(launch_nct_to_btc(x_bct, h->cfg.latent_channels, h->T, B, h->xe, h->xe_op, h->prec, h->CP, h->CP, s, h->pair_width(), h->pair_off()));
  if (!h->lens.masked) return 0;
  const size_t ob = (size_t)h->pair_width() * operand_bytes(h->prec);
  HIPCHK(launch_mask_rows(h->xe, (size_t)h->CP * 4, (size_t)h->CP * 4, B, h->T, h->lens.dev, s));
  HIPCHK(launch_mask_rows(h->xe_op, ob, ob, B, h->T, h->lens.dev, s));
  return 0;
}

static const struct { const char* name; const char* env; bool ns2vc_unet::* member; } kOptions[] = {
  {"ln_linear", "NS2VC_LN_LINEAR", &ns2vc_unet::ln_linear}, {"fold_ff", "NS2VC_FOLD_FF", &ns2vc_unet::fold_ff},
  {"fuse_ffn", "NS2VC_FUSE_FFN", &ns2vc_unet::fuse_ffn}, {"fuse_ffn_pre", "NS2VC_FUSE_FFN_PRE", &ns2vc_unet::fuse_ffn_pre},
  {"fuse_geglu", "NS2VC_FUSE_GEGLU", &ns2vc_unet::fuse_geglu}, {"fuse_rows", "NS2VC_FUSE_ROWS", &ns2vc_unet::fuse_rows},
  {"fuse_rows_gn", "NS2VC_FUSE_ROWS_GN", &ns2vc_unet::fuse_rows_gn}, {"fuse_gn_gemm", "NS2VC_FUSE_GN_GEMM", &ns2vc_unet::fuse_gn_gemm},
  {"fuse_gn_cat", "NS2VC_FUSE_GN_CAT", &ns2vc_unet::fuse_gn_cat}, {"gn_coop", "NS2VC_GN_COOP", &ns2vc_unet::gn_coop},
  {"slice_rows", "NS2VC_SLICE_ROWS", &ns2vc_unet::slice_rows}, {"attn_fp8", "NS2VC_ATTN_FP8", &ns2vc_unet::attn_fp8},
  {"attn_optimistic", "NS2VC_ATTN_OPTIMISTIC", &ns2vc_unet::attn_optimistic}, {"conv_ts", "NS2VC_CONV_TS", &ns2vc_unet::conv_ts},
  {"conv_wtiled", "NS2VC_CONV_WTILED", &ns2vc_unet::conv_wtiled}, {"gn_inloop", "NS2VC_GN_INLOOP", &ns2vc_unet::gn_inloop},
  {"fuse_solver", "NS2VC_FUSE_SOLVER", &ns2vc_unet::fuse_solver}, {"fuse_xattn", "NS2VC_FUSE_XATTN", &ns2vc_unet::fuse_xattn},
  {"fork_temb", "NS2VC_FORK_TEMB", &ns2vc_unet::fork_temb}, {"exact_io", "NS2VC_EXACT_IO", &ns2vc_unet::exact_io},
  {"split_io", "NS2VC_SPLIT_IO", &ns2vc_unet::split_io}, {"masked_fuse", "NS2VC_MASKED_FUSE", &ns2vc_unet::masked_fuse},
  {"masked_attn", "NS2VC_MASKED_ATTN", &ns2vc_unet::masked_attn}, {"masked_rows", "NS2VC_MASKED_ROWS", &ns2vc_unet::masked_rows},
  {"masked_ffn", "NS2VC_MASKED_FFN", &ns2vc_unet::masked_ffn}, {"masked_geglu", "NS2VC_MASKED_GEGLU", &ns2vc_unet::masked_geglu}};
static bool* option_ptr(ns2vc_unet* h, const char* name) {
  for (const auto& o : kOptions)
    if (!strcmp(name, o.name)) return &(h->*o.member);
  return nullptr;
}

extern "C" {

int ns2vc_unet_create(const ns2vc_unet_cfg* cfg, ns2vc_unet** out) {
  if (!cfg || !out) return fail("null argument");
  if (cfg->n_levels < 2 || cfg->n_levels > NS2VC_MAX_LEVELS) return fail("n_levels=%d out of range (2..%d)", cfg->n_levels, NS2VC_MAX_LEVELS);
  if (cfg->latent_channels <= 0 || cfg->latent_channels > 128) return fail("latent_channels=%d must be in 1..128", cfg->latent_channels);
  if (cfg->content_channels <= 0 || cfg->content_channels % 64)
    return fail("content_channels=%d must be a positive multiple of 64", cfg->content_channels);
  if (cfg->cross_attention_dim <= 0 || cfg->cross_attention_dim % 128)
    return fail("cross_attention_dim=%d must be a positive multiple of 128", cfg->cross_attention_dim);
  if (cfg->heads < 1) return fail("heads=%d must be >= 1", cfg->heads);
  if (cfg->norm_num_groups < 1 || cfg->norm_num_groups > 8) return fail("norm_num_groups=%d unsupported (1..8)", cfg->norm_num_groups);
  if (cfg->layers_per_block < 1) return fail("layers_per_block=%d must be >= 1", cfg->layers_per_block);
  if (cfg->pool_heads < 1 || cfg->cross_attention_dim % cfg->pool_heads || cfg->cross_attention_dim / cfg->pool_heads > 8)
    return fail("cross_attention_dim=%d over pool_heads=%d: the pool head width must be a whole number <= 8", cfg->cross_attention_dim, cfg->pool_heads);
  if (cfg->block_out_channels[0] != 128) return fail("block_out_channels[0]=%d must be 128 (padded latent width)", cfg->block_out_channels[0]);
  for (int l = 0; l < cfg->n_levels; ++l) {
    const int c = cfg->block_out_channels[l];
    if (c <= 0 || c % 128 || c > 512) return fail("block_out_channels[%d]=%d must be a multiple of 128 in 128..512", l, c);
    if (c % cfg->heads) return fail("block_out_channels[%d]=%d not divisible by heads=%d", l, c, cfg->heads);
    const int hd = c / cfg->heads;
    if (hd != 16 && hd != 32 && hd != 48 && hd != 64)
      return fail("heads=%d gives head width %d at block_out_channels[%d]=%d (16/32/48/64 supported)", cfg->heads, hd, l, c);
    if (c % cfg->norm_num_groups || (c / cfg->norm_num_groups) % 4)
      return fail("block_out_channels[%d]=%d incompatible with norm_num_groups=%d (group width must be a multiple of 4)", l, c, cfg->norm_num_groups);
  }
  for (const BlockW& b : make_topology(*cfg))
    for (const ResnetW& r : b.res)
      if (r.cin / cfg->norm_num_groups > 128)
        return fail("norm_num_groups=%d: the GroupNorm over the %d input channels of %s has groups of %d channels (<= 128 supported)",
                    cfg->norm_num_groups, r.cin, r.prefix.c_str(), r.cin / cfg->norm_num_groups);
  const hipError_t e = init_all_attributes();
  if (e != hipSuccess) return fail("kernel attribute setup failed: %s (is a gfx950 GPU visible?)", hipGetErrorString(e));
  auto* h = new ns2vc_unet();
  h->cfg = *cfg;
  if (hipGetDevice(&h->device) != hipSuccess) { delete h; return fail("hipGetDevice failed"); }
  {
    hipDeviceProp_t prop;
    if (hipGetDeviceProperties(&prop, h->device) == hipSuccess && prop.multiProcessorCount > 0) h->cus = prop.multiProcessorCount;
    h->bn128_min = h->cus * 5 / 8;
  }
  h->xcd_probe = xcd_round_robin_of_current_device();
  h->gn_coop = h->xcd_probe == 1;
  if (const char* dbg = getenv("NS2VC_DEBUG_ENV"); dbg && atoi(dbg) != 0) {
    for (const auto& o : kOptions)
      if (const char* v = getenv(o.env)) h->*o.member = atoi(v) != 0;
    if (h->xcd_probe != 1) h->gn_coop = false;
    {
      const char* nl = getenv("NS2VC_TS_NL");
      const char* ks = getenv("NS2VC_TS_KS");
      if (nl || ks) set_forced_gemm_tile(-4, ks ? (atoi(ks) ? 1 : 2) : 0, nl ? atoi(nl) : 0);
    }
    if (const char* v = getenv("NS2VC_GN_COOP_MIN")) h->gn_coop_min = atoi(v);
    if (const char* v = getenv("NS2VC_TS_BN128_MIN")) h->bn128_min = atoi(v) > 0 ? atoi(v) : h->bn128_min;
  }
  h->blocks = make_topology(*cfg);
  build_expected(h);
  *out = h;
  return 0;
}

int ns2vc_unet_destroy(ns2vc_unet* h) {
  if (h) (void)bind_device(h);
  delete h;
  return 0;
}

int ns2vc_unet_load_weight(ns2vc_unet* h, const char* key, const void* data, const int64_t* shape, int ndim) {
  if (!h || !key || !data) return fail("null argument");
  if (bind_device(h)) return 1;
  std::string k(key);
  const std::vector<int64_t>* want = nullptr;
  for (const auto& e : h->expected) if (e.first == k) { want = &e.second; break; }
  if (!want) return fail("unexpected weight key '%s'", key);
  if ((int)want->size() != ndim) return fail("%s: ndim %d != expected %zu", key, ndim, want->size());
  for (int i = 0; i < ndim; ++i) if (shape[i] != (*want)[i]) return fail("%s: shape[%d]=%lld != expected %lld", key, i, (long long)shape[i], (long long)(*want)[i]);
  HostTensor t;
  t.shape.assign(shape, shape + ndim);
  t.data.resize(t.numel());
  HIPCHK(hipMemcpy(t.data.data(), data, t.numel() * sizeof(float), hipMemcpyDefault));
  h->raw[k] = std::move(t);
  h->finalized = false;
  return 0;
}

int ns2vc_unet_num_missing_weights(ns2vc_unet* h, char* first_missing, int buflen) {
  int n = 0;
  for (const auto& e : h->expected)
    if (!h->raw.count(e.first)) {
      if (n == 0 && first_missing && buflen > 0) snprintf(first_missing, buflen, "%s", e.first.c_str());
      ++n;
    }
  return n;
}

int ns2vc_unet_finalize_weights(ns2vc_unet* h, int precision) {
  if (!h) return fail("null engine handle");
  if (bind_device(h)) return 1;
  if (precision != NS2VC_PREC_F32 && precision != NS2VC_PREC_BF16 && precision != NS2VC_PREC_F16) return fail("unknown precision %d", precision);
  char first[256] = {0};
  const int miss = ns2vc_unet_num_missing_weights(h, first, sizeof(first));
  if (miss) return fail("%d weights missing, first: %s", miss, first);
  for (void* p : h->weight_allocs) (void)hipFree(p);
  h->weight_allocs.clear();
  h->prec = precision;
  if (pack_all(h)) return 1;
  h->finalized = true;
  h->temb_table_valid = false;
  drop_plan(h);
  return 0;
}

int ns2vc_unet_set_debug(ns2vc_unet* h, int enable) {
  if (!h) return fail("null engine handle");
  if (bind_device(h)) return 1;
  if (h->debug != (enable != 0)) {
    h->debug = enable != 0;
    drop_plan(h);
  }
  return 0;
}

int ns2vc_unet_set_option(ns2vc_unet* h, const char* name, int value) {
  if (!h || !name) return fail("null argument");
  if (bind_device(h)) return 1;
  if (!strcmp(name, "temb_join_skip")) {
    if (h->tfork.join_skip != std::max(value, 0)) { h->tfork.join_skip = std::max(value, 0); drop_plan(h); }
    return 0;
  }
  bool* opt = option_ptr(h, name);
  if (!opt) {
    std::string names;
    for (const auto& o : kOptions) names += (names.empty() ? "" : ", ") + std::string(o.name);
    return fail("unknown option '%s' (%s)", name, names.c_str());
  }
  if (opt == &h->gn_coop && value != 0 && h->xcd_probe != 1) return fail("gn_coop needs workgroup ids 8 apart on one XCD; the placement probe of this device returned %d", h->xcd_probe);
  if (*opt != (value != 0)) { *opt = value != 0; drop_plan(h); }
  return 0;
}

int ns2vc_unet_ln_ratio_post(ns2vc_unet* h, void* stream) {
  if (check_ready(h, true)) return 1;
  hipStream_t s = (hipStream_t)stream;
  if (!h->ln_out.mail) {
    HIPCHK(hipHostMalloc((void**)&h->ln_out.mail, 64, hipHostMallocDefault));
    h->ln_out.mail[0] = 0;
  }
// ... 329 lines not shown
```

### ns2vc_amd/csrc/engine_internal.h

```cpp
#pragma once
#include "common.h"

#include <cstdarg>
#include <cstdio>
#include <functional>
#include <map>
#include <string>
#include <vector>

namespace ns2vc {

inline thread_local std::string g_err;

inline int fail(const char* fmt, ...) {
  char buf[1024];
  va_list ap;
  va_start(ap, fmt);
  vsnprintf(buf, sizeof(buf), fmt, ap);
  va_end(ap);
  g_err = buf;
  return 1;
}
#define HIPCHK(expr)                                                                                       \
  do {                                                                                                     \
// ... 18 lines not shown
  std::vector<float> data;
  std::vector<int64_t> shape;
  size_t numel() const { size_t n = 1; for (auto s : shape) n *= (size_t)s; return n; }
};

struct PackedW {
  void* w = nullptr;
  void* wt = nullptr;
  float* bias = nullptr;
  float* wsum = nullptr;
  int N = 0, K = 0;
};

struct ResnetW {
  std::string prefix;
  int cin = 0, cout = 0, temb_off = 0;
  bool shortcut = false;
  float *n1g = nullptr, *n1b = nullptr, *n2g = nullptr, *n2b = nullptr;
  PackedW conv1, conv2, sc;
};
struct AttnW {
  std::string prefix;
  int dim = 0, kv_off = 0;
  float *ng = nullptr, *nb = nullptr;
  PackedW proj_in, qkv, o1, q2, o2, ff1, ff2, proj_out;
  PackedW ffpo;
  void* ffn_pre_stream = nullptr;
  void* ffn_stream = nullptr;
  float* ffn_consts = nullptr;
  void* geglu_stream = nullptr;
  float* geglu_consts = nullptr;
  void *chain_in = nullptr, *chain_mid = nullptr;
  void* chain_in_s2 = nullptr;
  float *chain_in_consts = nullptr, *chain_mid_consts = nullptr;
};
struct BlockW {
  std::string kind;
  int index = 0, level = 0, channels = 0;
  std::vector<ResnetW> res;
  std::vector<AttnW> attn;
  int sampler = 0;
  PackedW samp;
};

struct Op {
  std::string name;
  std::function<hipError_t(hipStream_t)> fn;
  int kind = 0;
  double flops = 0.0;
  double bytes = 0.0;
  std::function<hipError_t(hipStream_t)> rearm;
};
struct Tap {
  std::string name;
  float* copy = nullptr;
  int rows = 0, cols = 0;
};

struct Staged {
  void* buf = nullptr;
  size_t cap = 0;
  hipEvent_t event = nullptr;
  bool pending = false;
  int reserve(size_t bytes) {
    if (!event) HIPCHK(hipEventCreateWithFlags(&event, hipEventDisableTiming));
    if (pending) { HIPCHK(hipEventSynchronize(event)); pending = false; }
    if (cap < bytes) {
      if (buf) HIPCHK(hipHostFree(buf));
      buf = nullptr; cap = 0;
      HIPCHK(hipHostMalloc(&buf, bytes, hipHostMallocDefault));
      cap = bytes;
    }
    return 0;
  }
  int record(hipStream_t s) {
    HIPCHK(hipEventRecord(event, s));
    pending = true;
    return 0;
  }
  ~Staged() {
    if (pending) (void)hipEventSynchronize(event);
    if (event) (void)hipEventDestroy(event);
    if (buf) (void)hipHostFree(buf);
  }
};

}

struct ns2vc_unet {
  ns2vc_unet_cfg cfg{};
  std::map<std::string, ns2vc::HostTensor> raw;
  std::vector<std::pair<std::string, std::vector<int64_t>>> expected;
  int prec = -1;
  bool finalized = false;
  std::vector<void*> weight_allocs;

  std::vector<ns2vc::BlockW> blocks;
  ns2vc::PackedW conv_in_x, conv_in_c, conv_out, temb_all, kv_all, pool_qkv;
  ns2vc::PackedW conv_in_xp, conv_in_cp, conv_outp;
  ns2vc::PackedW conv_in_x32, conv_in_c32, conv_out32, temb_all32;
  float *t_w1t = nullptr, *t_b1 = nullptr, *t_w2t = nullptr, *t_b2 = nullptr;
  float *p_n1g = nullptr, *p_n1b = nullptr, *p_pos = nullptr, *p_projT = nullptr, *p_projb = nullptr, *p_n2g = nullptr, *p_n2b = nullptr;
  float *out_ng = nullptr, *out_nb = nullptr;
  int n_temb = 0, n_kv = 0;
  int CP = 128;

  int B = 0, T = 0, Lp = 0;
  void* arena = nullptr;
  size_t arena_bytes = 0, arena_used = 0;
  std::vector<ns2vc::Op> cond_ops, fwd_ops;
  size_t cond_split = 0;
  bool debug = false;
  int device = 0;
  bool ln_linear = true;
  bool fold_ff = true;
  bool fuse_ffn = true;
  bool fuse_rows = true;
  bool attn_fp8 = false;
  bool fuse_ffn_pre = true;
  bool fuse_geglu = true;
  bool fuse_rows_gn = true;
  bool fuse_gn_gemm = true;
  bool fuse_gn_cat = true;
  bool gn_coop = true;
  bool conv_ts = true;
  bool conv_wtiled = true;
  bool split_io = true;
  bool exact_io = false;
  float* content_f32 = nullptr;
  float* emb_act_f32 = nullptr;
  int conv_out_prec = -1;
  bool fork_temb = false;
  struct TembFork {
    int begin = -1, end = -1, join = -1;
    int first = -1, readers = 0;
    bool ok = false;
    int join_skip = 0;
    hipStream_t side_stream = nullptr;
    hipEvent_t ev_fork = nullptr, ev_join = nullptr;
  } tfork;
  bool fuse_xattn = false;
  bool fuse_solver = false;
  ns2vc::GemmArgs conv_out_g;
  int conv_out_idx = -1;
  bool warned_wtiled = false;
  int bn128_min = 160;
  bool gn_inloop = false;
  int gn_coop_min = 2;
  int cus = 256;
  int xcd_probe = -1;
  bool slice_rows = true;
  unsigned* ln_health = nullptr;
  bool attn_optimistic = true;
  unsigned* attn_fallbacks = nullptr;
  unsigned long long coef_hash = 0;
  std::vector<ns2vc::Tap> taps;
  bool has_mask = false;
  bool masked_fuse = false;
  bool masked_attn = false;
  bool masked_rows = false;
  bool masked_ffn = false;
  bool masked_geglu = false;
  struct Lengths {
    bool masked = false;
    int* dev = nullptr;
    size_t off = 0;
    float* selfbias = nullptr;
    std::vector<int32_t> applied;
    ns2vc::Staged stage;
  } lens;
  struct PromptLengths {
    bool on = false;
    int* dev = nullptr;
    std::vector<int32_t> applied;
    ns2vc::Staged stage;
  } plens;
  struct Seeds {
    unsigned long long* dev = nullptr;
    int cap = 0;
    bool set = false;
    ns2vc::Staged stage;
  } seeds;
  bool stochastic = false;
  struct Guidance {
    bool on = false;
    int n = 0;
    float* dev = nullptr;
    int cap = 0;
    ns2vc::Staged stage;
  } guide;
  int loop_items() const { return guide.on ? guide.n : B; }
  struct History2 {
    bool on = false;
    float* mprev2 = nullptr;
    size_t n = 0;
  } hist2;
  struct ItemSchedules {
    bool on = false;
    int n = 0, rows = 0;
    ns2vc::SolverItem* dev = nullptr;
    int cap = 0;
    ns2vc::Staged stage;
  } items;
  struct SlotLoop {
    static constexpr int kRing = 8;
    bool on = false;
    std::vector<ns2vc::SolverItem> rec;
    std::vector<char> busy;
    std::vector<float> coef;
    int* list_dev = nullptr;
    int cap = 0;
    ns2vc::Staged ring[kRing];
    int ring_next = 0;
    ns2vc::Staged coef_ring[kRing];
    int coef_next = 0;
    bool any_busy() const { for (char b : busy) if (b) return true; return false; }
  } slots;
  bool in_slot_loop() const { return slots.on && next_step >= 0; }
  struct X0Correction {
    int mode = 0;
    float ratio = 0.995f, max_val = 1.0f;
    float* thr = nullptr;
    int cap = 0;
  } x0c;

  float *xe = nullptr, *xbar = nullptr, *d1 = nullptr, *mprev = nullptr, *x0 = nullptr;
  float *content_conv = nullptr, *prompt = nullptr, *maskbias = nullptr;
  float *aug = nullptr, *emb = nullptr, *temb = nullptr;
  float *seq = nullptr, *pool_qkv_buf = nullptr, *pooled = nullptr;
  void *xe_op = nullptr, *content_op = nullptr, *prompt_op = nullptr, *emb_act_op = nullptr, *kv = nullptr, *seq_op = nullptr;
  float *t_dev = nullptr;
  uint8_t* mask_dev = nullptr;
  int* step_dev = nullptr;
  size_t stats_bytes = 8;
  float* coef_dev = nullptr;
  float* temb_table = nullptr;
  bool temb_table_valid = false;
  int steps = 0;
  int next_step = -1;
  bool use_step_table = false;
  struct LnReadout {
    unsigned* mail = nullptr;
    hipEvent_t event = nullptr;
    bool posted = false;
  } ln_out;

  hipStream_t cap_stream = nullptr;
  hipGraphExec_t step_graph = nullptr;
  unsigned long long graph_captures = 0;

  int pair_width() const { return prec != ns2vc::PREC_F32 ? 2 * CP : CP; }
  int pair_off() const { return prec != ns2vc::PREC_F32 ? CP : 0; }

  ~ns2vc_unet() {
    if (seeds.dev) (void)hipFree(seeds.dev);
    if (guide.dev) (void)hipFree(guide.dev);
    if (hist2.mprev2) (void)hipFree(hist2.mprev2);
    if (x0c.thr) (void)hipFree(x0c.thr);
    if (items.dev) (void)hipFree(items.dev);
    if (slots.list_dev) (void)hipFree(slots.list_dev);
    if (step_graph) (void)hipGraphExecDestroy(step_graph);
    if (cap_stream) (void)hipStreamDestroy(cap_stream);
    if (tfork.side_stream) (void)hipStreamDestroy(tfork.side_stream);
    if (tfork.ev_fork) (void)hipEventDestroy(tfork.ev_fork);
    if (tfork.ev_join) (void)hipEventDestroy(tfork.ev_join);
    if (ln_out.event) (void)hipEventDestroy(ln_out.event);
    if (ln_out.mail) (void)hipHostFree(ln_out.mail);
    if (arena) (void)hipFree(arena);
    if (coef_dev) (void)hipFree(coef_dev);
    if (temb_table) (void)hipFree(temb_table);
    for (void* p : weight_allocs) (void)hipFree(p);
  }
};

namespace ns2vc {

std::vector<BlockW> make_topology(const ns2vc_unet_cfg& c);
void build_expected(ns2vc_unet* h);
std::vector<float> rounded_rowsum(const float* rows, int N, int K, int Np, int prec);
int pack_all(ns2vc_unet* h);
extern int g_geglu_min_rows;
std::vector<int> level_lengths(int T, int n_levels);
int build_plan(ns2vc_unet* h, bool sizing);
int run_ops(const std::vector<Op>& ops, hipStream_t s, size_t first = 0, size_t last = (size_t)-1);
bool temb_forks(const ns2vc_unet* h, size_t last);
void drop_step_graph(ns2vc_unet* h);
void drop_plan(ns2vc_unet* h);
int check_ready(ns2vc_unet* h, bool need_plan);
int load_state(ns2vc_unet* h, const float* x_bct, hipStream_t s, int items = 0);
bool solver_in_conv_out(ns2vc_unet* h, GemmArgs& g);
int stage_slot_list(ns2vc_unet* h, int n, const int32_t* slots, int nslots, const SolverItem* rec, hipStream_t s, const int** slots_dev,
                    const SolverItem** rec_dev);
hipError_t init_all_attributes();
int xcd_round_robin_of_current_device();

}
```

### ns2vc_amd/csrc/kernel_table.h

```cpp
#pragma once
#include <hip/hip_runtime.h>

#include <cstdint>

namespace ns2vc {

constexpr uint64_t KEY_NONE = ~0ull;
constexpr uint64_t kernel_key() { return 0; }
template <typename... I> constexpr uint64_t kernel_key(int f, I... rest) {
  static_assert(sizeof...(I) < 6, "six fields of ten bits");
  const uint64_t r = kernel_key(rest...);
  return ((unsigned)f >> 10) || r == KEY_NONE ? KEY_NONE : (r << 10 | (unsigned)f);
}

struct KernelRow {
  uint64_t key;
  const void* fn;
  uint32_t lds;
  uint32_t threads;
};
struct KernelTable {
  const KernelRow* rows;
  int n;
  template <int N> constexpr KernelTable(const KernelRow (&r)[N]) : rows(r), n(N) {}
};

inline const KernelRow* find(const KernelTable& t, uint64_t key) {
  for (int i = 0; i < t.n; ++i)
    if (t.rows[i].key == key) return &t.rows[i];
  return nullptr;
}
inline hipError_t set_lds_all(const KernelTable& t) {
  for (int i = 0; i < t.n; ++i) {
    const hipError_t e = hipFuncSetAttribute(t.rows[i].fn, hipFuncAttributeMaxDynamicSharedMemorySize, (int)t.rows[i].lds);
    if (e != hipSuccess) return e;
  }
  return hipSuccess;
}
template <typename... A> hipError_t launch(const KernelRow& r, dim3 grid, hipStream_t s, const A&... args) {
  void* p[] = {const_cast<void*>(static_cast<const void*>(&args))...};
  (void)hipLaunchKernel(r.fn, grid, dim3(r.threads), p, r.lds, s);
  return hipGetLastError();
}

const KernelTable& gemm2_kernel_table();
const KernelTable& gemm4_kernel_table();
const KernelTable& conv3ts_kernel_table();
const KernelTable& attn_kernel_table();
const KernelTable& ffn_kernel_table();
const KernelTable& geglu_kernel_table();
const KernelTable& rowchain_kernel_table();

}
```

### ns2vc_amd/csrc/plan.cpp

```cpp
#include "engine_internal.h"

#include <algorithm>
#include <cmath>
#include <cstring>

namespace ns2vc {

int g_geglu_min_rows = 4608;

std::vector<int> level_lengths(int T, int n_levels) {
  std::vector<int> Ts(n_levels);
  Ts[0] = T;
  for (int l = 1; l < n_levels; ++l) Ts[l] = (Ts[l - 1] + 1) / 2;
  return Ts;
}

namespace {

struct Planner {
  ns2vc_unet* h;
  std::vector<Op>* ops;
  bool sizing = false;
  size_t off = 0;
  int B, T, Lp, G, prec;
// ... 84 lines not shown
    add("tap:" + name, [=](hipStream_t s) { return hipMemcpyAsync(cp, src, bytes, hipMemcpyDeviceToDevice, s); }, 4, 0.0, 2.0 * bytes);
  }

  void gemm(const std::string& name, GemmArgs g, int pr_override = -1) {
    const int pr = pr_override >= 0 ? pr_override : prec;
    const double osz = (double)opsz;
    const double nout = g.geglu ? g.N / 2 : g.N;
    const bool pair = g.c1 && g.a1 == g.a0 && g.c0 == 2 * g.c1 && g.c2 == 0;
    const double Kalg = pair ? g.K / 3.0 : (double)g.K, cin = pair ? g.c1 : g.c0 + g.c1 + g.c2, cgn = pair ? g.c1 : g.c0;
    const double flops = 2.0 * g.M * (double)g.N * Kalg;
    const double in_rows = (double)g.B * g.Tin;
    const double bytes = in_rows * cin * osz + (double)g.N * Kalg * osz + (g.out_f32 ? g.M * nout * 4.0 : 0.0) +
                         (g.out_op ? g.M * nout * osz : 0.0) + (g.res ? g.M * nout * 4.0 : 0.0);
    const double pro = g.gnp_x ? in_rows * cgn * (4.0 + osz * (g.gnp_raw ? 2.0 : 1.0)) : 0.0;
    if (g.taps == 3 && g.tmode == TMODE_SAME && !g.conv_bn) g.conv_bn = convts_bn_for(g, h->bn128_min);
    const bool self_mask = fused && ops == &h->fwd_ops && g.Tout > 1 && level_of(g.Tout) >= 0 && gemm_masks_rows(g, pr);
    if (self_mask) {
      g.lens = lens_of(g.Tout);
      if (g.gnp_x && g.algo == 0) g.algo = 2;
    } else if (masked && g.stats) { stats_of.erase(g.out_f32); g.stats = nullptr; }
    if (g.gnp_temb) temb_reader();
    add(g.gnp_x ? name + "[+norm]" : name, [=](hipStream_t s) { return launch_gemm(g, pr, s); }, 1, flops, bytes + pro);
    if (!sizing && g.gnp_x && g.gnp_sync) {
      unsigned* words = g.gnp_sync;
      const size_t nbytes = (((size_t)g.B * g.Tin + 63) / 64) * 8;
      ops->back().rearm = [=](hipStream_t s) { return launch_zero(words, (nbytes + 15) & ~(size_t)15, s); };
    }
    if (g.Tout > 1 && !self_mask) {
      const int nc = g.geglu ? g.N / 2 : g.N;
      mask(name, g.out_f32, g.ldo_f32, nc, 4, g.Tout);
      mask(name, g.out_op, g.ldo_op, nc, operand_bytes(pr), g.Tout);
    }
  }
  GemmArgs base(const void* a0, int lda0, int c0, int Tin, int Tout, const PackedW& w, float* out_f32, void* out_op, int ldo) {
    GemmArgs g;
    memset(&g, 0, sizeof(g));
    g.a0 = a0; g.lda0 = lda0; g.c0 = c0;
    g.B = B; g.Tin = Tin; g.Tout = Tout; g.M = B * Tout;
    g.taps = 1; g.tmode = TMODE_SAME;
    g.w = w.w; g.K = w.K; g.N = w.N; g.bias = w.bias;
    g.w_tiled = h->conv_wtiled ? w.wt : nullptr;
    g.out_f32 = out_f32; g.ldo_f32 = ldo;
    g.out_op = out_op; g.ldo_op = ldo;
    g.algo = h->conv_ts ? (h->gn_inloop ? 0 : 2) : 1;
    return g;
  }
  struct GnPro { const float* x = nullptr; int ldx = 0; const long long* st = nullptr; const float* gamma = nullptr; const float* beta = nullptr;
                 const float* temb = nullptr; int ldtemb = 0; float eps = 0.f; int G = 0, silu = 0; unsigned* sync = nullptr; unsigned* alone = nullptr;
                 const float* x1 = nullptr; int ldx1 = 0, c1 = 0; const long long* st1 = nullptr; void* raw = nullptr; };
  static void gn_fuse(GemmArgs& g, const GnPro& p) {
    if (!p.x) return;
    g.gnp_x = p.x; g.gnp_ldx = p.ldx; g.gnp_stats = p.st; g.gnp_gamma = p.gamma; g.gnp_beta = p.beta;
    g.gnp_temb = p.temb; g.gnp_ldtemb = p.ldtemb; g.gnp_eps = p.eps; g.gnp_G = p.G; g.gnp_silu = p.silu;
    g.gnp_sync = p.sync; g.gnp_alone = p.alone;
    g.gnp_x1 = p.x1; g.gnp_ldx1 = p.ldx1; g.gnp_c1 = p.c1; g.gnp_stats1 = p.st1; g.gnp_raw = p.raw;
  }
  GnPro groupnorm(const std::string& name, const float* a0, int lda0, int c0, const float* a1, int lda1, int c1, int Tl, float eps,
                  const float* gamma, const float* beta, const float* temb, int temb_off, int cout, int silu, void* dst, void* raw,
                  int consumer_n = 0, int consumer_taps = 1, int pair = 0) {
    (void)cout;
    const int nchunk = (Tl + gn_rows - 1) / gn_rows, rows = gn_rows, Bq = B, Gq = G, ldt = h->temb_all.N, pr = prec;
    double* part = gn_partial;
    const double n = (double)Bq * Tl * (c0 + c1);
    const long long* st0 = find_stats(a0);
    const long long* st1 = a1 ? find_stats(a1) : nullptr;
    const bool epi = st0 && (!a1 || st1) && (((c0 + c1) / Gq) % 16 == 0) && (c0 % 16 == 0);
    bool pro_ok = !masked;
    if (masked && fused && consumer_taps == 3 && consumer_n > 0) {
      GemmArgs t;
      memset(&t, 0, sizeof(t));
      t.taps = 3; t.tmode = TMODE_SAME; t.B = Bq; t.Tin = t.Tout = Tl; t.M = Bq * Tl; t.N = consumer_n;
      t.c0 = pair ? 2 * (c0 + c1) : c0 + c1; t.c1 = pair ? c0 + c1 : 0;
      t.algo = h->conv_ts ? 2 : 1;
      pro_ok = gemm_uses_convts(t, prec);
    }
    if (epi && pro_ok && h->fuse_gn_gemm && consumer_n > 0 && (consumer_n % 128) == 0 && (h->fuse_gn_cat || (!a1 && !raw)) && Tl >= 66 && c0 + c1 <= 1024 &&
        (!pair || (h->conv_ts && consumer_taps == 3 && ((c0 + c1) % 64) == 0)) &&
        ((c0 + c1) % Gq) == 0 && Gq <= 8 && (lda0 & 3) == 0 && (!a1 || ((lda1 & 3) == 0 && (c1 & 15) == 0))) {
      GnPro p;
      p.x = a0; p.ldx = lda0; p.st = st0;
      if (a1) { p.x1 = a1; p.ldx1 = lda1; p.c1 = c1; p.st1 = st1; }
      p.raw = raw;
      p.gamma = gamma; p.beta = beta; p.temb = temb ? temb + temb_off : nullptr; p.ldtemb = ldt;
      p.eps = eps; p.G = Gq; p.silu = silu;
      int nshare = consumer_n / 128;
      if (consumer_taps == 3 && h->conv_ts && Tl >= 66) {
        GemmArgs t;
        memset(&t, 0, sizeof(t));
        t.B = Bq; t.Tin = t.Tout = Tl; t.N = consumer_n;
        nshare = consumer_n / convts_bn_for(t, h->bn128_min);
      }
      if (h->gn_coop && nshare >= std::max(2, h->gn_coop_min)) { p.sync = new_sync(((size_t)Bq * Tl + 63) / 64); p.alone = (p.sync && h->ln_health) ? h->ln_health + 48 : nullptr; }
      return p;
    }
    if (!epi) {
      st0 = st1 = nullptr;
      add(name + ".gn_stats", [=](hipStream_t s) { return launch_gn_partial(a0, lda0, c0, a1, lda1, c1, Bq, Tl, Gq, part, nchunk, rows, s); },
          3, 3.0 * n, 4.0 * n);
    }
    if (temb) temb_reader();
    const int* lens = masked ? lens_of(Tl) : nullptr;
    add(name + ".gn_apply", [=](hipStream_t s) {
      return launch_gn_apply(a0, lda0, c0, a1, lda1, c1, Bq, Tl, Gq, eps, part, nchunk, st0, st1, gamma, beta, temb, ldt, temb_off, silu, dst,
                             raw, pr, s, pair, lens);
    }, 3, 4.0 * n, n * (4.0 + opsz * (raw ? 2.0 : 1.0) + opsz * (pair ? 1.0 : 0.0)));
    return GnPro();
  }

  void resnet(const ResnetW& r, const float* a0, int lda0, int c0, const float* a1, int lda1, int c1, int Tl, float* h1, void* hn,
              float* out, void* out_op) {
    const int cin = c0 + c1;
    const GnPro p1 = groupnorm(r.prefix + ".norm1", a0, lda0, c0, a1, lda1, c1, Tl, 1e-5f, r.n1g, r.n1b, nullptr, 0, 0, 1, xn,
                               r.shortcut ? xr : nullptr, r.conv1.N, 3);
    GemmArgs g = base(xn, cin, cin, Tl, Tl, r.conv1, h1, nullptr, r.cout);
    g.taps = 3;
    gn_fuse(g, p1);
    g.stats = new_stats(h1, Tl, r.cout);
    gemm(r.prefix + ".conv1", g);
    const GnPro p2 = groupnorm(r.prefix + ".norm2", h1, r.cout, r.cout, nullptr, 0, 0, Tl, 1e-5f, r.n2g, r.n2b, h->temb, r.temb_off, r.cout, 1, hn,
                               nullptr, r.conv2.N, 3);
    GemmArgs g2 = base(hn, r.cout, r.cout, Tl, Tl, r.conv2, out, out_op, r.cout);
    g2.taps = 3;
    gn_fuse(g2, p2);
    if (r.shortcut) {
      g2.a2 = xr; g2.lda2 = cin; g2.c2 = cin;
    } else {
      g2.res = a0; g2.ldres = lda0;
    }
    g2.stats = new_stats(out, Tl, r.cout);
    gemm(r.prefix + ".conv2", g2);
  }

  void attention(const std::string& name, const void* q, int ldq, const void* k, int ldk, const void* v, int ldv, int Lq, int Lk,
                 const float* bias, int hd, void* out, int ldo, bool self = false, const int* cross_lens = nullptr) {
    AttnArgs a;
    memset(&a, 0, sizeof(a));
    a.q = q; a.k = k; a.v = v; a.ldq = ldq; a.ldk = ldk; a.ldv = ldv;
    a.B = B; a.H = h->cfg.heads; a.Lq = Lq; a.Lk = Lk; a.bias = bias;
    a.scale = 1.0f / std::sqrt((float)hd);
    a.out = out; a.ldo = ldo;
    a.pv_fp8 = (h->attn_fp8 && prec != PREC_F32) ? 1 : 0;
    a.exact_only = h->attn_optimistic ? 0 : 1;
    a.fallbacks = h->attn_fallbacks;
    const int pr = prec;
    const bool self_mask = masked && h->masked_attn && ops == &h->fwd_ops && level_of(Lq) >= 0 && attention_masks_rows(a, hd, pr);
    if (self_mask) {
      a.q_lens = lens_of(Lq);
      if (self) a.k_lens = lens_of(Lk);
    } else if (self) a.bias = selfbias_of(Lk);
    if (cross_lens && (self_mask || (h->masked_attn && ops == &h->fwd_ops && attention_masks_rows(a, hd, pr)))) {
      a.k_lens = cross_lens;
      if (!h->has_mask) a.bias = nullptr;
    }
    add(name, [=](hipStream_t s) { return launch_attention(a, hd, pr, s); }, 2, 4.0 * B * a.H * (double)Lq * Lk * hd,
        (double)opsz * B * a.H * hd * (2.0 * Lq + 2.0 * Lk));
    if (!self_mask) mask(name, out, ldo, a.H * hd, opsz, Lq);
  }

  std::map<std::string, void*> xattn_vt;
  bool xattn_fused(const AttnW& a, int Tl) const {
    const int d = a.dim;
    const bool lin = h->ln_linear && (d % 128 == 0) && d <= 512 && !masked;
    return h->fuse_xattn && lin && h->fold_ff && h->fuse_ffn && a.ffn_stream && ffn_eligible(d, Tl, prec) && h->fuse_ffn_pre && a.ffn_pre_stream &&
           h->cfg.heads == 8 && (d == 128 || d == 256);
  }
  void transformer(const AttnW& a, const float* x, int Tl, float* y, void* yn, void* qkv, void* ao, void* qb, void* ffh, float* out,
                   void* out_op) {
    const int d = a.dim, M = B * Tl, hd = d / h->cfg.heads, pr = prec;
    const std::string t = a.prefix + ".transformer_blocks.0";
    GemmArgs g;
    auto layernorm = [&](const std::string& nm) {
      add(nm, [=](hipStream_t s) { return launch_ln_apply_op(y, d, M, d, 1e-5f, yn, pr, s); }, 3, 8.0 * M * d, (4.0 + opsz) * M * d);
    };
    const bool lin_dense = h->ln_linear && (d % 128 == 0) && d <= 512;
    const bool lin = lin_dense && !masked;
    const bool lens_rows = masked && h->masked_rows && ops == &h->fwd_ops && level_of(Tl) >= 0;
    auto consume = [&](GemmArgs& gg, float* rs, const PackedW& w) {
      if (rs) { gg.ln_stats = rs; gg.ln_wsum = w.wsum; gg.ln_eps = 1e-5f; gg.ln_dim = d; gg.ln_health = h->ln_health; }
    };
    float* r1 = lin ? rs1 : nullptr;
    auto rowchain = [&](const std::string& nm, const void* a_op, const long long* gn_st, void* stream, const float* bias1, const float* consts2,
                        const float* res, void* z_op, int n2) {
      ns2vc_rowchain_args c;
      memset(&c, 0, sizeof(c));
      c.a_op = a_op; c.lda = d; c.wstream = stream; c.bias1 = bias1; c.consts2 = consts2;
      c.res = res; c.ldres = d; c.out1_f32 = y; c.ldo1 = d; c.out2_op = z_op; c.ldo2 = n2;
      c.ln_eps = 1e-5f; c.M = M; c.dim = d; c.n2 = n2; c.ln_health = h->ln_health;
      if (gn_st) {
        c.a_op = nullptr; c.gn_x = x; c.ldx = d; c.gn_stats = gn_st; c.gn_gamma = a.ng; c.gn_beta = a.nb; c.gn_eps = 1e-6f; c.T = Tl; c.G = G;
      }
      if (!res && stream == a.chain_in && a.chain_in_s2 && h->slice_rows && 2 * ((M + 63) / 64) <= h->cus + 8) { c.wstream = a.chain_in_s2; c.slices = 2; }
      if (lens_rows) { c.lens = lens_of(Tl); c.T = Tl; }
      add(c.slices == 2 ? nm + "[2 slices]" : nm, [=](hipStream_t s) { return launch_rowchain(c, pr, s); }, 1, 2.0 * M * (double)d * (d + n2),
          (double)M * (d * ((gn_st ? 4.0 : opsz) + 4.0 + (res ? 4.0 : 0.0)) + n2 * opsz) + (double)(d + n2) * d * opsz);
    };
    auto chains_mask_rows = [&]() {
      ns2vc_rowchain_args c;
      memset(&c, 0, sizeof(c));
      c.M = M; c.dim = d; c.T = Tl;
      c.n2 = 3 * d;
      const bool in_ok = rowchain_masks_rows(c, pr);
      c.n2 = d;
      return in_ok && rowchain_masks_rows(c, pr);
    };
    const bool rows_ok = (masked ? lin_dense && lens_rows && chains_mask_rows() : lin) && h->fuse_rows && a.chain_in && a.chain_mid &&
                         rowchain_eligible(d, d, Tl, pr);
    const long long* xst = (rows_ok && h->fuse_rows_gn && Tl >= 64 && (d % G) == 0 && ((d / G) % 16) == 0) ? find_stats(x) : nullptr;
    GnPro pn;
    if (!xst) pn = groupnorm(a.prefix + ".norm", x, d, d, nullptr, 0, 0, Tl, 1e-6f, a.ng, a.nb, nullptr, 0, 0, 0, xn, nullptr, rows_ok ? 0 : a.proj_in.N);
    if (rows_ok) {
      rowchain(a.prefix + (xst ? ".rows[norm+proj_in+qkv]" : ".rows[proj_in+qkv]"), xn, xst, a.chain_in, a.proj_in.bias, a.chain_in_consts, nullptr, qkv,
               3 * d);
    } else {
      g = base(xn, d, d, Tl, Tl, a.proj_in, y, r1 ? yn : nullptr, d);
      gn_fuse(g, pn);
      g.rowstats = r1;
      gemm(a.prefix + ".proj_in", g);
      if (!r1) layernorm(t + ".norm1");
      g = base(yn, d, d, Tl, Tl, a.qkv, nullptr, qkv, 3 * d);
      consume(g, r1, a.qkv);
      gemm(t + ".attn1.qkv", g);
    }
    attention(t + ".attn1.sdpa", qkv, 3 * d, op_off(qkv, d), 3 * d, op_off(qkv, 2 * d), 3 * d, Tl, Tl, nullptr, hd, ao, d, true);
    float* r2 = lin ? rs2 : nullptr;
    if (rows_ok) {
      rowchain(t + ".rows[attn1.to_out+attn2.to_q]", ao, nullptr, a.chain_mid, a.o1.bias, a.chain_mid_consts, y, qb, d);
    } else {
      g = base(ao, d, d, Tl, Tl, a.o1, y, r2 ? yn : nullptr, d);
      g.res = y; g.ldres = d;
      g.rowstats = r2;
      gemm(t + ".attn1.to_out", g);
      if (!r2) layernorm(t + ".norm2");
      g = base(yn, d, d, Tl, Tl, a.q2, nullptr, qb, d);
      consume(g, r2, a.q2);
      gemm(t + ".attn2.to_q", g);
    }
    const int nkv = h->kv_all.N;
    const bool xatt = xattn_fused(a, Tl) && xattn_vt.count(a.prefix);
    if (!xatt)
      attention(t + ".attn2.sdpa", qb, d, op_off(h->kv, a.kv_off), nkv, op_off(h->kv, a.kv_off + d), nkv, Tl, Lp,
                (h->has_mask || h->plens.on) ? h->maskbias : nullptr, hd, ao, d, false, h->plens.on ? h->plens.dev : nullptr);
    float* r3 = lin ? rs3 : nullptr;
    const bool fold = h->fold_ff;
    void* yraw = r3 ? yn : (fold ? qb : nullptr);
    auto ffn_masks = [&]() {
      ns2vc_ffn_args f;
      memset(&f, 0, sizeof(f));
      f.B = B; f.T = Tl; f.M = M; f.dim = d;
      return ffn_masks_rows(f, pr);
    };
    const bool lens_ffn = masked && h->masked_ffn && ops == &h->fwd_ops && level_of(Tl) >= 0 && lin_dense && fold && h->fuse_ffn && a.ffn_stream &&
                          h->fuse_ffn_pre && a.ffn_pre_stream && ffn_eligible(d, Tl, pr) && ffn_masks();
    const bool ffn_ok = lens_ffn || (fold && r3 && h->fuse_ffn && a.ffn_stream && ffn_eligible(d, Tl, pr));
    const bool ffn_pre = ffn_ok && h->fuse_ffn_pre && a.ffn_pre_stream;
    if (!ffn_pre) {
      g = base(ao, d, d, Tl, Tl, a.o2, y, yraw, d);
      g.res = y; g.ldres = d;
      g.rowstats = r3;
      gemm(t + ".attn2.to_out", g);
    }
    if (ffn_ok) {
      ns2vc_ffn_args f;
      memset(&f, 0, sizeof(f));
      f.yn = yn; f.ldy = d; f.ln_stats = r3; f.ln_eps = 1e-5f;
      f.wstream = a.ffn_stream; f.consts = a.ffn_consts; f.bias2 = a.ffpo.bias;
      if (ffn_pre) {
        f.yn = nullptr; f.ln_stats = nullptr; f.wstream = a.ffn_pre_stream;
        f.pre_a = ao; f.pre_lda = d; f.pre_bias = a.o2.bias; f.pre_res = y; f.pre_ldres = d;
      }
      if (xatt) {
        f.pre_a = nullptr;
        f.att_q = qb; f.att_ldq = d; f.att_kv = xattn_vt[a.prefix];
        f.att_bias = (h->has_mask || h->plens.on) ? h->maskbias : nullptr; f.att_scale = 1.0f / std::sqrt((float)hd); f.att_Lk = Lp;
      }
      f.res = x; f.ldres = d;
      f.out_f32 = out; f.ldo_f32 = d; f.out_op = out_op; f.ldo_op = d;
      f.stats = new_stats(out, Tl, d);
      f.B = B; f.T = Tl; f.M = M; f.dim = d; f.ln_health = h->ln_health;
      if (lens_ffn) f.lens = lens_of(Tl);
      const double fl = 2.0 * M * (double)d * ((ffn_pre ? 14.0 : 13.0) * d) + (xatt ? 4.0 * B * h->cfg.heads * (double)Tl * Lp * hd : 0.0);
      add(a.prefix + (xatt ? ".ffn[attn2.sdpa+to_out+geglu+ff.out+proj_out]" : ffn_pre ? ".ffn[attn2.to_out+geglu+ff.out+proj_out]" : ".ffn[geglu+ff.out+proj_out]"),
          [=](hipStream_t s) { return launch_ffn(f, pr, s); }, 1, fl,
          (double)M * d * (opsz + 8.0 + (ffn_pre ? 4.0 : 0.0) + (out_op ? opsz : 0.0)) + (ffn_pre ? 14.0 : 13.0) * d * d * opsz +
              (xatt ? (double)opsz * B * d * 2.0 * Lp : 0.0));
      return;
    }
    auto geglu_masks = [&]() {
      ns2vc_geglu_args f;
      memset(&f, 0, sizeof(f));
      f.M = M; f.dim = d; f.T = Tl;
      return geglu_masks_rows(f, pr);
    };
    const bool lens_geglu = masked && h->masked_geglu && ops == &h->fwd_ops && level_of(Tl) >= 0 && lin_dense && fold && h->fuse_geglu &&
                            a.geglu_stream && geglu_eligible(d, Tl, pr) && M >= g_geglu_min_rows && geglu_masks();
    if (!r3 && !lens_geglu) layernorm(t + ".norm3");
    if (lens_geglu || (r3 && h->fuse_geglu && a.geglu_stream && geglu_eligible(d, Tl, pr) && M >= g_geglu_min_rows)) {
      ns2vc_geglu_args f;
      memset(&f, 0, sizeof(f));
      f.yn = yn; f.ldy = d; f.ln_stats = r3; f.ln_eps = 1e-5f;
      if (lens_geglu) { f.yn = qb; f.ln_stats = nullptr; f.T = Tl; f.lens = lens_of(Tl); }
      f.wstream = a.geglu_stream; f.consts = a.geglu_consts;
      f.out_op = ffh; f.ldo = 4 * d; f.M = M; f.dim = d; f.ln_health = h->ln_health;
      add(t + ".ff.geglu[token-stationary]", [=](hipStream_t s) { return launch_geglu(f, pr, s); }, 1, 2.0 * M * (double)d * 8.0 * d,
          (double)M * d * opsz * 5.0 + (double)M * (d / 64) * 8.0 + 8.0 * d * d * opsz);
    } else {
      g = base(yn, d, d, Tl, Tl, a.ff1, nullptr, ffh, 4 * d);
      g.geglu = 1;
// ... 336 lines not shown
```

Measured before the change: 281.0 denoiser-steps/s (batch 32 per GPU, whole job).

## Add LDS-resident attention kernel that loads each head's K/V once

Adds a resident attention kernel for head dims 16/32 in 16-bit precision. One 1024-thread block per (batch, head) stages the whole K/V sequence in LDS once, and its waves then iterate over all query tiles. This is meant to remove the repeated K/V global reloads and the double-buffer synchronisation of the per-query-tile kernel when B*H is at least the CU count. It shares tile helpers with the existing kernel, which is refactored into AttnTile, and costs large LDS use and lower occupancy per block.

```diff
diff --git a/include/ns2vc_hip.h b/include/ns2vc_hip.h
--- a/include/ns2vc_hip.h
+++ b/include/ns2vc_hip.h
@@ -210,6 +210,9 @@
 int ns2vc_debug_set_geglu_min_rows(int rows);
 int ns2vc_debug_set_attn_keys(int keys);
 int ns2vc_debug_set_attn_optimistic(int on);
+int ns2vc_debug_set_attn_resident(int mode);
+unsigned long long ns2vc_debug_attn_resident_launches(void);
+int ns2vc_debug_attnres_table(int* rows);
 int ns2vc_debug_set_rowchain_tokens(int nt);
 
 int ns2vc_to_operand(const float* host, size_t n, int precision, void** out_dev);
diff --git a/ns2vc_amd/_lib.py b/ns2vc_amd/_lib.py
--- a/ns2vc_amd/_lib.py
+++ b/ns2vc_amd/_lib.py
@@ -208,6 +208,9 @@
     "ns2vc_debug_set_rowchain_tokens": (_I, [_I]),
     "ns2vc_debug_set_attn_keys": (_I, [_I]),
     "ns2vc_debug_set_attn_optimistic": (_I, [_I]),
+    "ns2vc_debug_set_attn_resident": (_I, [_I]),
+    "ns2vc_debug_attnres_table": (_I, [C.POINTER(_I)]),
+    "ns2vc_debug_attn_resident_launches": (C.c_ulonglong, []),
     "ns2vc_k_groupnorm_stats": (_I, [_P, _I, _I, _P, _I, _I, _I, C.c_float, _P, _P, _P, _I, _I, _I, _P, _I, _P]),
     "ns2vc_k_groupnorm_stats2": (_I, [_P, _I, _I, _P, _P, _I, _I, _P, _I, _I, _I, C.c_float, _P, _P, _P, _I, _I, _I, _P, _P, _I, _P]),
     "ns2vc_k_groupnorm": (_I, [_P, _I, _I, _P, _I, _I, _I, _I, _I, C.c_float, _P, _P, _P, _I, _I, _I, _P, _P, _I, _P]),
diff --git a/ns2vc_amd/csrc/abi_kernels.cpp b/ns2vc_amd/csrc/abi_kernels.cpp
--- a/ns2vc_amd/csrc/abi_kernels.cpp
+++ b/ns2vc_amd/csrc/abi_kernels.cpp
@@ -11,6 +11,7 @@
   hipError_t e = init_gemm_attributes();
   if (e == hipSuccess) e = init_convts_attributes();
   if (e == hipSuccess) e = init_attn_attributes();
+  if (e == hipSuccess) e = init_attnres_attributes();
   if (e == hipSuccess) e = init_ffn_attributes();
   if (e == hipSuccess) e = init_geglu_attributes();
   if (e == hipSuccess) e = init_rowchain_attributes();
@@ -228,6 +229,17 @@
 int ns2vc_debug_set_attn_keys(int keys) {
   if (keys != 0 && keys != 64 && keys != 128) return fail("attention K/V tile: 0 (heuristic), 64 or 128 keys");
   set_forced_attn_keys(keys);
+  return 0;
+}
+int ns2vc_debug_set_attn_resident(int mode) {
+  if (mode < -1 || mode > 1) return fail("resident attention: -1 (the rule), 0 (never) or 1 (whenever the launch fits)");
+  set_attn_resident_mode(mode);
+  return 0;
+}
+unsigned long long ns2vc_debug_attn_resident_launches(void) { return attn_resident_launches(); }
+int ns2vc_debug_attnres_table(int* rows) {
+  if (!rows) return fail("attnres table: rows not NULL");
+  *rows = attnres_kernel_table().n;
   return 0;
 }
 int ns2vc_debug_set_rowchain_tokens(int nt) {
diff --git a/ns2vc_amd/csrc/attn.hip b/ns2vc_amd/csrc/attn.hip
--- a/ns2vc_amd/csrc/attn.hip
+++ b/ns2vc_amd/csrc/attn.hip
@@ -1,115 +1,18 @@
-#include "common.h"
-#include "mma.h"
+#include "attn_common.h"
 #include "kernel_table.h"
 #include <cstdlib>
 
 namespace ns2vc {
 
-template <typename T> struct AMma;
-template <> struct AMma<float> {
-  static constexpr int SZ = 4;
-  __device__ static __forceinline__ void mma(f32x16_t& acc, const u32x4_t& a, const u32x4_t& b) {
-    acc = __builtin_amdgcn_mfma_f32_32x32x2f32(__uint_as_float(a.x), __uint_as_float(b.x), acc, 0, 0, 0);
-    acc = __builtin_amdgcn_mfma_f32_32x32x2f32(__uint_as_float(a.y), __uint_as_float(b.y), acc, 0, 0, 0);
-    acc = __builtin_amdgcn_mfma_f32_32x32x2f32(__uint_as_float(a.z), __uint_as_float(b.z), acc, 0, 0, 0);
-    acc = __builtin_amdgcn_mfma_f32_32x32x2f32(__uint_as_float(a.w), __uint_as_float(b.w), acc, 0, 0, 0);
-  }
-  __device__ static __forceinline__ f32x16_t mma0(const u32x4_t& a, const u32x4_t& b) {
-    f32x16_t acc = __builtin_amdgcn_mfma_f32_32x32x2f32(__uint_as_float(a.x), __uint_as_float(b.x), f32x16_t{0.f, 0.f, 0.f, 0.f, 0.f, 0.f, 0.f, 0.f, 0.f, 0.f, 0.f, 0.f, 0.f, 0.f, 0.f, 0.f}, 0, 0, 0);
-    acc = __builtin_amdgcn_mfma_f32_32x32x2f32(__uint_as_float(a.y), __uint_as_float(b.y), acc, 0, 0, 0);
-    acc = __builtin_amdgcn_mfma_f32_32x32x2f32(__uint_as_float(a.z), __uint_as_float(b.z), acc, 0, 0, 0);
-    acc = __builtin_amdgcn_mfma_f32_32x32x2f32(__uint_as_float(a.w), __uint_as_float(b.w), acc, 0, 0, 0);
-    return acc;
-  }
-  __device__ static __forceinline__ int vpos(int key) { return key; }
-};
-template <typename TM> struct AMma16 {
-  static constexpr int SZ = 2;
-  __device__ static __forceinline__ void mma(f32x16_t& acc, const u32x4_t& a, const u32x4_t& b) { MmaT<TM>::mma(acc, a, b); }
-  __device__ static __forceinline__ f32x16_t mma0(const u32x4_t& a, const u32x4_t& b) {
-    f32x16_t acc = {0.f, 0.f, 0.f, 0.f, 0.f, 0.f, 0.f, 0.f, 0.f, 0.f, 0.f, 0.f, 0.f, 0.f, 0.f, 0.f};
-    MmaT<TM>::mma(acc, a, b);
-    return acc;
-  }
-  __device__ static __forceinline__ int vpos(int key) { return (key & ~12) | ((key & 4) << 1) | ((key & 8) >> 1); }
-};
-template <> struct AMma<bf16_t> : AMma16<bf16_t> {};
-template <> struct AMma<f16_t> : AMma16<f16_t> {};
-
-template <typename TM> __device__ __forceinline__ void vt_scatter(char* vp, int rowb, const u32x4_t& v);
-template <> __device__ __forceinline__ void vt_scatter<float>(char* vp, int rowb, const u32x4_t& v) {
-  *reinterpret_cast<uint32_t*>(vp) = v.x;
-  *reinterpret_cast<uint32_t*>(vp + rowb) = v.y;
-  *reinterpret_cast<uint32_t*>(vp + 2 * rowb) = v.z;
-  *reinterpret_cast<uint32_t*>(vp + 3 * rowb) = v.w;
-}
-__device__ __forceinline__ void vt_scatter16(char* vp, int rowb, const u32x4_t& v) {
-  *reinterpret_cast<uint16_t*>(vp) = (uint16_t)v.x;
-  *reinterpret_cast<uint16_t*>(vp + rowb) = (uint16_t)(v.x >> 16);
-  *reinterpret_cast<uint16_t*>(vp + 2 * rowb) = (uint16_t)v.y;
-  *reinterpret_cast<uint16_t*>(vp + 3 * rowb) = (uint16_t)(v.y >> 16);
-  *reinterpret_cast<uint16_t*>(vp + 4 * rowb) = (uint16_t)v.z;
-  *reinterpret_cast<uint16_t*>(vp + 5 * rowb) = (uint16_t)(v.z >> 16);
-  *reinterpret_cast<uint16_t*>(vp + 6 * rowb) = (uint16_t)v.w;
-  *reinterpret_cast<uint16_t*>(vp + 7 * rowb) = (uint16_t)(v.w >> 16);
-}
-template <> __device__ __forceinline__ void vt_scatter<bf16_t>(char* vp, int rowb, const u32x4_t& v) { vt_scatter16(vp, rowb, v); }
-template <> __device__ __forceinline__ void vt_scatter<f16_t>(char* vp, int rowb, const u32x4_t& v) { vt_scatter16(vp, rowb, v); }
-
-__device__ __forceinline__ float half_max(float v) {
-  const auto r = __builtin_amdgcn_permlane32_swap(__float_as_uint(v), __float_as_uint(v), false, false);
-  return fmaxf(__uint_as_float(r[0]), __uint_as_float(r[1]));
-}
-__device__ __forceinline__ float half_sum(float v) {
-  const auto r = __builtin_amdgcn_permlane32_swap(__float_as_uint(v), __float_as_uint(v), false, false);
-  return __uint_as_float(r[0]) + __uint_as_float(r[1]);
-}
-
-template <typename TM> __device__ __forceinline__ float round_op(float x);
-template <> __device__ __forceinline__ float round_op<float>(float x) { return x; }
-template <> __device__ __forceinline__ float round_op<bf16_t>(float x) { return __uint_as_float(pack_bf16x2(0.f, x) & 0xffff0000u); }
-template <> __device__ __forceinline__ float round_op<f16_t>(float x) { return f16_lo(pack_f16x2(x, 0.f)); }
-template <typename TM> __device__ __forceinline__ u32x4_t aux_chunk(float e0, float e1);
-template <> __device__ __forceinline__ u32x4_t aux_chunk<float>(float e0, float e1) { return u32x4_t{__float_as_uint(e0), __float_as_uint(e1), 0u, 0u}; }
-template <> __device__ __forceinline__ u32x4_t aux_chunk<bf16_t>(float e0, float e1) { return u32x4_t{pack_bf16x2(e0, e1), 0u, 0u, 0u}; }
-template <> __device__ __forceinline__ u32x4_t aux_chunk<f16_t>(float e0, float e1) { return u32x4_t{pack_f16x2(e0, e1), 0u, 0u, 0u}; }
-template <typename TM> __device__ __forceinline__ TM op_from_float(float x);
-template <> __device__ __forceinline__ float op_from_float<float>(float x) { return x; }
-template <> __device__ __forceinline__ bf16_t op_from_float<bf16_t>(float x) { bf16_t r; r.v = (uint16_t)pack_bf16x2(x, 0.f); return r; }
-template <> __device__ __forceinline__ f16_t op_from_float<f16_t>(float x) { f16_t r; r.v = (uint16_t)pack_f16x2(x, 0.f); return r; }
-
-__device__ __forceinline__ uint32_t pack_fp8x4(float a, float b, float c, float d) {
-  int v = __builtin_amdgcn_cvt_pk_fp8_f32(a, b, 0, false);
-  v = __builtin_amdgcn_cvt_pk_fp8_f32(c, d, v, true);
-  return (uint32_t)v;
-}
-typedef int i32x8_t __attribute__((ext_vector_type(8)));
-#ifndef NS2VC_ATTN_OPT
-#define NS2VC_ATTN_OPT 1
-#endif
-template <bool B> struct OptTag { static constexpr bool value = B; };
 __device__ int g_attn_exact_only = 0;
-__device__ __forceinline__ int vpos8(int key) { return ((key & 4) << 3) | ((key & 32) >> 1) | ((key & 24) >> 1) | (key & 3); }
 template <typename TM, int HD, int KEYS, bool P8, bool MASKED = false>
 __global__ __launch_bounds__(256) void attn_kernel(const AttnArgs a) {
   op_mode_init<TM>();
   static_assert(!P8 || (sizeof(TM) == 2 && KEYS == 64), "the fp8 PV path: 16-bit operand types, one 64-key tile per f8f6f4 MFMA");
-  constexpr int NSUB = KEYS / 32;
-  constexpr int SZ = AMma<TM>::SZ;
-  constexpr int EPC = 16 / SZ;
-  constexpr int NS = HD * SZ / 32;
-  constexpr int KROWB = HD * SZ + 48;
-  constexpr int VSZ = P8 ? 1 : SZ;
-  constexpr int VROWB = KEYS * VSZ + 16;
-  constexpr int HDX = (HD + 1 + 31) / 32 * 32;
-  constexpr int DT = HDX / 32;
-  constexpr int NSL = SZ;
-  constexpr int KBYTES = KEYS * KROWB, VBYTES = HDX * VROWB;
-  constexpr int STAGE = KBYTES + VBYTES;
-  constexpr int PPR = HD * SZ / 16;
-  constexpr int NPIECE = KEYS * PPR;
+  using G = AttnTile<TM, HD, KEYS, P8>;
+  constexpr int SZ = G::SZ, EPC = G::EPC, NS = G::NS, KROWB = G::KROWB, VROWB = G::VROWB, DT = G::DT, KBYTES = G::KBYTES, STAGE = G::STAGE, PPR = G::PPR,
+                NPIECE = G::NPIECE;
   constexpr int UPT = (NPIECE + 255) / 256;
-  constexpr float THRESH = P8 ? 8.0f : 12.0f;
   extern __shared__ __attribute__((aligned(16))) char smem[];
 
   const int tid = threadIdx.x, lane = tid & 63, wave = tid >> 6;
@@ -152,24 +55,10 @@
   }
 
   u32x4_t qf[NS];
-  {
-    const TM* qp = reinterpret_cast<const TM*>(a.q) + ((size_t)(b * a.Lq + min(q, Lqb - 1)) * a.ldq + h * HD);
-#pragma unroll
-    for (int s = 0; s < NS; ++s) {
-      const u32x4_t raw = *reinterpret_cast<const u32x4_t*>(qp + s * 2 * EPC + hi * EPC);
-      if constexpr (SZ == 4) {
-        qf[s] = u32x4_t{__float_as_uint(__uint_as_float(raw.x) * sc2), __float_as_uint(__uint_as_float(raw.y) * sc2),
-                        __float_as_uint(__uint_as_float(raw.z) * sc2), __float_as_uint(__uint_as_float(raw.w) * sc2)};
-      } else {
-        auto sc = [&](uint32_t w) __attribute__((always_inline)) { return Op16<TM>::pack(Op16<TM>::lo(w) * sc2, Op16<TM>::hi(w) * sc2); };
-        qf[s] = u32x4_t{sc(raw.x), sc(raw.y), sc(raw.z), sc(raw.w)};
-      }
-      if (q >= Lqb) qf[s] = u32x4_t{0, 0, 0, 0};
-    }
-  }
+  G::load_q(qf, reinterpret_cast<const TM*>(a.q) + ((size_t)(b * a.Lq + min(q, Lqb - 1)) * a.ldq + h * HD), sc2, hi, q >= Lqb);
   float m_ref = 0.f;
   u32x4_t qaux = hi == 0 ? aux_chunk<TM>(-m_ref, 1.0f) : u32x4_t{0, 0, 0, 0};
-  constexpr bool CINIT = HD == 16 && SZ == 2 && !P8;
+  constexpr bool CINIT = G::CINIT;
   f32x16_t cinit;
 #pragma unroll
   for (int r = 0; r < 16; ++r) cinit[r] = 0.f;
@@ -207,24 +96,8 @@
     for (int i = 0; i < UPT; ++i) {
       const int u = tid + 256 * i;
       if (u < NPIECE) {
-        {
-          const int key = u / PPR, pc = u - key * PPR;
-          *reinterpret_cast<u32x4_t*>(Ks + key * KROWB + pc * 16) = kraw[i];
-        }
-        {
-          const int key = u % KEYS, pc = u / KEYS;
-          if constexpr (P8) {
-            const u32x4_t w = vraw[i];
-            const uint32_t b0 = pack_fp8x4(Op16<TM>::lo(w.x), Op16<TM>::hi(w.x), Op16<TM>::lo(w.y), Op16<TM>::hi(w.y));
-            const uint32_t b1 = pack_fp8x4(Op16<TM>::lo(w.z), Op16<TM>::hi(w.z), Op16<TM>::lo(w.w), Op16<TM>::hi(w.w));
-            uint8_t* vp = reinterpret_cast<uint8_t*>(Vs + (pc * EPC) * VROWB + vpos8(key));
-#pragma unroll
-            for (int j = 0; j < 4; ++j) { vp[j * VROWB] = (uint8_t)(b0 >> (8 * j)); vp[(4 + j) * VROWB] = (uint8_t)(b1 >> (8 * j)); }
-          } else {
-            const int pos = (key & ~31) + AMma<TM>::vpos(key & 31);
-            vt_scatter<TM>(Vs + (pc * EPC) * VROWB + pos * SZ, VROWB, vraw[i]);
-          }
-        }
+        G::store_k_piece(Ks, u, kraw[i]);
+        G::store_v_piece(Vs, u, vraw[i]);
       }
     }
     if (tid < KEYS) {
@@ -236,7 +109,11 @@
   f32x16_t o[DT];
   const int ntile = (Lkb + KEYS - 1) / KEYS;
   constexpr bool OPT = NS2VC_ATTN_OPT && !P8 && sizeof(TM) == 2;
-  constexpr float OPT_MARGIN = 4.0f;
+#if defined(NS2VC_ATTN_ABLATE_RESIDENT)
+  constexpr bool ABL_RES = HD <= 32 && sizeof(TM) == 2 && !P8 && !MASKED;
+#else
+  constexpr bool ABL_RES = false;
+#endif
   auto run = [&](auto optimistic, const bool compute) __attribute__((always_inline)) {
   constexpr bool O = decltype(optimistic)::value;
   if (compute) {
@@ -257,107 +134,19 @@
   __syncthreads();
 
   for (int t = 0; t < ntile; ++t) {
-    if (t + 1 < ntile) load_tile(t + 1);
-    const char* Ks = smem + (t & 1) * STAGE;
+    if (!ABL_RES && t + 1 < ntile) load_tile(t + 1);
+    const char* Ks = smem + (ABL_RES ? 0 : (t & 1)) * STAGE;
     const char* Vs = Ks + KBYTES;
-    if (compute) {
-
-    f32x16_t s[NSUB];
-    if (CINIT && !bias && (t + 1 < ntile || Lkb % KEYS == 0)) {
-#pragma unroll
-      for (int k2 = 0; k2 < NSUB; ++k2) {
-        const char* kr = Ks + (k2 * 32 + l31) * KROWB + hi * 16;
-        s[k2] = cinit;
-#pragma unroll
-        for (int sl = 0; sl < NS; ++sl) AMma<TM>::mma(s[k2], *reinterpret_cast<const u32x4_t*>(kr + sl * 32), qf[sl]);
-      }
-    } else {
-#pragma unroll
-    for (int k2 = 0; k2 < NSUB; ++k2) {
-      const char* kr = Ks + (k2 * 32 + l31) * KROWB + hi * 16;
-      s[k2] = AMma<TM>::mma0(*reinterpret_cast<const u32x4_t*>(kr + NS * 32), qaux);
-#pragma unroll
-      for (int sl = 0; sl < NS; ++sl) AMma<TM>::mma(s[k2], *reinterpret_cast<const u32x4_t*>(kr + sl * 32), qf[sl]);
-    }
-    }
-    if (!O || t == 0) {
-      float mx = s[0][0];
-#pragma unroll
-      for (int k2 = 0; k2 < NSUB; ++k2)
-#pragma unroll
-        for (int r = 0; r < 16; ++r) mx = fmaxf(mx, s[k2][r]);
-      mx = half_max(mx);
-      if (t == 0 || __any(mx > THRESH)) {
-        float target = t == 0 ? mx : fmaxf(mx, 0.f);
-        if (!(target > -INFINITY)) target = 0.f;
-        if (O) target += OPT_MARGIN;
-        const float m_new = round_op<TM>(m_ref + target);
-        const float dsh = m_new - m_ref;
-        if (t > 0) {
-          const float alpha = __builtin_amdgcn_exp2f(-dsh);
-#pragma unroll
-          for (int d = 0; d < DT; ++d)
-#pragma unroll
-            for (int r = 0; r < 16; ++r) o[d][r] *= alpha;
-        }
-#pragma unroll
-        for (int k2 = 0; k2 < NSUB; ++k2)
-#pragma unroll
-          for (int r = 0; r < 16; ++r) s[k2][r] -= dsh;
-        m_ref = m_new;
-        if (hi == 0) qaux = aux_chunk<TM>(-m_ref, 1.0f);
-        if constexpr (CINIT) {
-#pragma unroll
-          for (int r = 0; r < 16; ++r) cinit[r] = -m_ref;
-        }
-      }
-    }
-#pragma unroll
-    for (int k2 = 0; k2 < NSUB; ++k2)
-#pragma unroll
-      for (int r = 0; r < 16; ++r) s[k2][r] = __builtin_amdgcn_exp2f(s[k2][r]);
-
-    if constexpr (P8) {
-      i32x8_t pf;
-#pragma unroll
-      for (int v = 0; v < 8; ++v)
-        pf[v] = (int)pack_fp8x4(s[v >> 2][4 * (v & 3) + 0], s[v >> 2][4 * (v & 3) + 1], s[v >> 2][4 * (v & 3) + 2], s[v >> 2][4 * (v & 3) + 3]);
-#pragma unroll
-      for (int d = 0; d < DT; ++d) {
-        const char* vr = Vs + (d * 32 + l31) * VROWB + hi * 32;
-        const u32x4_t v0 = *reinterpret_cast<const u32x4_t*>(vr), v1 = *reinterpret_cast<const u32x4_t*>(vr + 16);
-        const i32x8_t vf = {(int)v0.x, (int)v0.y, (int)v0.z, (int)v0.w, (int)v1.x, (int)v1.y, (int)v1.z, (int)v1.w};
-        o[d] = __builtin_amdgcn_mfma_scale_f32_32x32x64_f8f6f4(vf, pf, o[d], 0, 0, 0, 0x7f7f7f7f, 0, 0x7f7f7f7f);
-      }
-    } else {
-#pragma unroll
-    for (int k2 = 0; k2 < NSUB; ++k2) {
-#pragma unroll
-      for (int sl = 0; sl < NSL; ++sl) {
-        u32x4_t pf;
-        if constexpr (SZ == 4) {
-          pf = u32x4_t{__float_as_uint(s[k2][4 * sl + 0]), __float_as_uint(s[k2][4 * sl + 1]),
-                       __float_as_uint(s[k2][4 * sl + 2]), __float_as_uint(s[k2][4 * sl + 3])};
-        } else {
-          pf = u32x4_t{Op16<TM>::pack(s[k2][8 * sl + 0], s[k2][8 * sl + 1]), Op16<TM>::pack(s[k2][8 * sl + 2], s[k2][8 * sl + 3]),
-                       Op16<TM>::pack(s[k2][8 * sl + 4], s[k2][8 * sl + 5]), Op16<TM>::pack(s[k2][8 * sl + 6], s[k2][8 * sl + 7])};
-        }
-#pragma unroll
-        for (int d = 0; d < DT; ++d) {
-          const u32x4_t vf = *reinterpret_cast<const u32x4_t*>(Vs + (d * 32 + l31) * VROWB + k2 * 32 * SZ + sl * 32 + hi * 16);
-          AMma<TM>::mma(o[d], vf, pf);
-        }
-      }
-    }
-    }
-    }
-    if (t + 1 < ntile) store_tile((t + 1) & 1, (t + 1) * KEYS);
-    __syncthreads();
+    if (compute)
+      G::template step<O>(Ks, Vs, t, CINIT && !bias && (t + 1 < ntile || Lkb % KEYS == 0), qf, qaux, cinit, m_ref, o, l31, hi);
+    if constexpr (!ABL_RES) {
+      if (t + 1 < ntile) store_tile((t + 1) & 1, (t + 1) * KEYS);
+      __syncthreads();
+    }
   }
   };
 
-  constexpr int LB = HD / 32, LR = ((HD % 32) / 8) * 4;
-  static_assert(HD % 32 == 0 || HD % 32 == 16, "ones row must sit at row 0 or 16 of its 32-row block");
+  constexpr int LB = G::LB, LR = G::LR;
   if (OPT && !g_attn_exact_only && !a.exact_only) {
     run(OptTag<true>{}, true);
     const float lq = o[LB][LR];
@@ -371,45 +160,11 @@
     run(OptTag<false>{}, true);
   }
 
-  const auto lsw = __builtin_amdgcn_permlane32_swap(__float_as_uint(o[LB][LR]), __float_as_uint(o[LB][LR]), false, false);
-  const float l_tot = __uint_as_float(lsw[0]);
-  const float inv = 1.0f / l_tot;
   TM* op = reinterpret_cast<TM*>(a.out) + ((size_t)(b * a.Lq + min(q, a.Lq - 1)) * a.ldo + h * HD);
-  const bool padded = MASKED && q >= Lqb;
-  if constexpr (SZ == 2) {
-#pragma unroll
-    for (int d = 0; d < DT; ++d)
-#pragma unroll
-      for (int gp = 0; gp < 2; ++gp) {
-        if (d * 32 + 16 * gp < HD) {
-          const uint32_t a0 = Op16<TM>::pack(o[d][8 * gp] * inv, o[d][8 * gp + 1] * inv), a1 = Op16<TM>::pack(o[d][8 * gp + 2] * inv, o[d][8 * gp + 3] * inv);
-          const uint32_t b0 = Op16<TM>::pack(o[d][8 * gp + 4] * inv, o[d][8 * gp + 5] * inv), b1 = Op16<TM>::pack(o[d][8 * gp + 6] * inv, o[d][8 * gp + 7] * inv);
-          const auto x0 = __builtin_amdgcn_permlane32_swap(a0, b0, false, false);
-          const auto x1 = __builtin_amdgcn_permlane32_swap(a1, b1, false, false);
-#if defined(NS2VC_ATTN_ABLATE_STORE)
-          asm volatile("" :: "v"(x0[0]), "v"(x1[0]), "v"(x0[1]), "v"(x1[1]));
-#else
-          if (q < a.Lq) *reinterpret_cast<u32x4_t*>(op + d * 32 + 8 * (2 * gp + hi)) = padded ? u32x4_t{0, 0, 0, 0} : u32x4_t{x0[0], x1[0], x0[1], x1[1]};
-#endif
-        }
-      }
-  } else if (q < a.Lq) {
-#pragma unroll
-    for (int d = 0; d < DT; ++d)
-#pragma unroll
-      for (int gq = 0; gq < 4; ++gq) {
-        const int d0 = d * 32 + 8 * gq + 4 * hi;
-        if (d0 < HD) store_op4<TM>(op + d0, padded ? 0.f : o[d][4 * gq] * inv, padded ? 0.f : o[d][4 * gq + 1] * inv, padded ? 0.f : o[d][4 * gq + 2] * inv,
-                                   padded ? 0.f : o[d][4 * gq + 3] * inv);
-      }
-  }
-}
-
-template <typename TM, int HD, int KEYS> static constexpr size_t attn_lds() {
-  constexpr int SZ = AMma<TM>::SZ;
-  constexpr int HDX = (HD + 1 + 31) / 32 * 32;
-  return 2 * (size_t)(KEYS * (HD * SZ + 48) + HDX * (KEYS * SZ + 16));
-}
+  G::store_out(o, op, hi, q < a.Lq, MASKED && q >= Lqb);
+}
+
+template <typename TM, int HD, int KEYS> static constexpr size_t attn_lds() { return 2 * (size_t)AttnTile<TM, HD, KEYS, false>::STAGE; }
 
 #define NS2VC_ATTN_ROW(TM, PREC, HD, KEYS, FP8, MK) \
   {kernel_key(PREC, HD, KEYS, FP8, MK), reinterpret_cast<const void*>(attn_kernel<TM, HD, KEYS, FP8, MK>), (uint32_t)attn_lds<TM, HD, KEYS>(), 256}
@@ -432,7 +187,11 @@
 
 static int g_force_keys = 0;
 void set_forced_attn_keys(int keys) { g_force_keys = keys; }
-void set_attn_optimistic(int on) { const int v = on ? 0 : 1; (void)hipMemcpyToSymbol(HIP_SYMBOL(g_attn_exact_only), &v, sizeof(v)); }
+void set_attn_optimistic(int on) {
+  const int v = on ? 0 : 1;
+  (void)hipMemcpyToSymbol(HIP_SYMBOL(g_attn_exact_only), &v, sizeof(v));
+  set_attnres_optimistic(on);
+}
 
 hipError_t init_attn_attributes() { return set_lds_all(k_attn_table); }
 
@@ -440,13 +199,14 @@
   return find(k_attn_table, kernel_key(prec, head_dim, 64, a.pv_fp8 != 0, true)) != nullptr;
 }
 
-hipError_t launch_attention(const AttnArgs& a, int head_dim, int prec, hipStream_t s) {
+hipError_t launch_attention(const AttnArgs& a, int head_dim, int prec, hipStream_t s, bool resident) {
   const int al = prec == PREC_F32 ? 3 : 7;
   if (!a.q || !a.k || !a.v || !a.out) return hipErrorInvalidValue;
   const bool masked = a.q_lens || a.k_lens, fp8 = a.pv_fp8 != 0;
   if (masked && !attention_masks_rows(a, head_dim, prec)) return hipErrorInvalidValue;
   if (a.Lq <= 0 || a.Lk <= 0 || (a.ldq & al) || (a.ldk & al) || (a.ldv & al) || (a.ldo & al)) return hipErrorInvalidValue;
   if (reinterpret_cast<uintptr_t>(a.out) & 15) return hipErrorInvalidValue;
+  if (attention_resident_eligible(a, head_dim, prec, resident)) return launch_attention_resident(a, head_dim, prec, s);
   const int keys = !fp8 && g_force_keys == 128 && find(k_attn_table, kernel_key(prec, head_dim, 128, false, masked)) ? 128 : 64;
   const KernelRow* row = find(k_attn_table, kernel_key(prec, head_dim, keys, fp8, masked));
   if (!row) return hipErrorInvalidValue;
diff --git a/ns2vc_amd/csrc/attn_common.h b/ns2vc_amd/csrc/attn_common.h
--- /dev/null
+++ b/ns2vc_amd/csrc/attn_common.h
@@ -0,0 +1,273 @@
+#pragma once
+#include "common.h"
+#include "mma.h"
+
+namespace ns2vc {
+
+template <typename T> struct AMma;
+template <> struct AMma<float> {
+  static constexpr int SZ = 4;
+  __device__ static __forceinline__ void mma(f32x16_t& acc, const u32x4_t& a, const u32x4_t& b) {
+    acc = __builtin_amdgcn_mfma_f32_32x32x2f32(__uint_as_float(a.x), __uint_as_float(b.x), acc, 0, 0, 0);
+    acc = __builtin_amdgcn_mfma_f32_32x32x2f32(__uint_as_float(a.y), __uint_as_float(b.y), acc, 0, 0, 0);
+    acc = __builtin_amdgcn_mfma_f32_32x32x2f32(__uint_as_float(a.z), __uint_as_float(b.z), acc, 0, 0, 0);
+    acc = __builtin_amdgcn_mfma_f32_32x32x2f32(__uint_as_float(a.w), __uint_as_float(b.w), acc, 0, 0, 0);
+  }
+  __device__ static __forceinline__ f32x16_t mma0(const u32x4_t& a, const u32x4_t& b) {
+    f32x16_t acc = __builtin_amdgcn_mfma_f32_32x32x2f32(__uint_as_float(a.x), __uint_as_float(b.x), f32x16_t{0.f, 0.f, 0.f, 0.f, 0.f, 0.f, 0.f, 0.f, 0.f, 0.f, 0.f, 0.f, 0.f, 0.f, 0.f, 0.f}, 0, 0, 0);
+    acc = __builtin_amdgcn_mfma_f32_32x32x2f32(__uint_as_float(a.y), __uint_as_float(b.y), acc, 0, 0, 0);
+    acc = __builtin_amdgcn_mfma_f32_32x32x2f32(__uint_as_float(a.z), __uint_as_float(b.z), acc, 0, 0, 0);
+    acc = __builtin_amdgcn_mfma_f32_32x32x2f32(__uint_as_float(a.w), __uint_as_float(b.w), acc, 0, 0, 0);
+    return acc;
+  }
+  __device__ static __forceinline__ int vpos(int key) { return key; }
+};
+template <typename TM> struct AMma16 {
+  static constexpr int SZ = 2;
+  __device__ static __forceinline__ void mma(f32x16_t& acc, const u32x4_t& a, const u32x4_t& b) { MmaT<TM>::mma(acc, a, b); }
+  __device__ static __forceinline__ f32x16_t mma0(const u32x4_t& a, const u32x4_t& b) {
+    f32x16_t acc = {0.f, 0.f, 0.f, 0.f, 0.f, 0.f, 0.f, 0.f, 0.f, 0.f, 0.f, 0.f, 0.f, 0.f, 0.f, 0.f};
+    MmaT<TM>::mma(acc, a, b);
+    return acc;
+  }
+  __device__ static __forceinline__ int vpos(int key) { return (key & ~12) | ((key & 4) << 1) | ((key & 8) >> 1); }
+};
+template <> struct AMma<bf16_t> : AMma16<bf16_t> {};
+template <> struct AMma<f16_t> : AMma16<f16_t> {};
+
+template <typename TM> __device__ __forceinline__ void vt_scatter(char* vp, int rowb, const u32x4_t& v);
+template <> __device__ __forceinline__ void vt_scatter<float>(char* vp, int rowb, const u32x4_t& v) {
+  *reinterpret_cast<uint32_t*>(vp) = v.x;
+  *reinterpret_cast<uint32_t*>(vp + rowb) = v.y;
+  *reinterpret_cast<uint32_t*>(vp + 2 * rowb) = v.z;
+  *reinterpret_cast<uint32_t*>(vp + 3 * rowb) = v.w;
+}
+__device__ __forceinline__ void vt_scatter16(char* vp, int rowb, const u32x4_t& v) {
+  *reinterpret_cast<uint16_t*>(vp) = (uint16_t)v.x;
+  *reinterpret_cast<uint16_t*>(vp + rowb) = (uint16_t)(v.x >> 16);
+  *reinterpret_cast<uint16_t*>(vp + 2 * rowb) = (uint16_t)v.y;
+  *reinterpret_cast<uint16_t*>(vp + 3 * rowb) = (uint16_t)(v.y >> 16);
+  *reinterpret_cast<uint16_t*>(vp + 4 * rowb) = (uint16_t)v.z;
+  *reinterpret_cast<uint16_t*>(vp + 5 * rowb) = (uint16_t)(v.z >> 16);
+  *reinterpret_cast<uint16_t*>(vp + 6 * rowb) = (uint16_t)v.w;
+  *reinterpret_cast<uint16_t*>(vp + 7 * rowb) = (uint16_t)(v.w >> 16);
+}
+template <> __device__ __forceinline__ void vt_scatter<bf16_t>(char* vp, int rowb, const u32x4_t& v) { vt_scatter16(vp, rowb, v); }
+template <> __device__ __forceinline__ void vt_scatter<f16_t>(char* vp, int rowb, const u32x4_t& v) { vt_scatter16(vp, rowb, v); }
+
+__device__ __forceinline__ float half_max(float v) {
+  const auto r = __builtin_amdgcn_permlane32_swap(__float_as_uint(v), __float_as_uint(v), false, false);
+  return fmaxf(__uint_as_float(r[0]), __uint_as_float(r[1]));
+}
+__device__ __forceinline__ float half_sum(float v) {
+  const auto r = __builtin_amdgcn_permlane32_swap(__float_as_uint(v), __float_as_uint(v), false, false);
+  return __uint_as_float(r[0]) + __uint_as_float(r[1]);
+}
+
+template <typename TM> __device__ __forceinline__ float round_op(float x);
+template <> __device__ __forceinline__ float round_op<float>(float x) { return x; }
+template <> __device__ __forceinline__ float round_op<bf16_t>(float x) { return __uint_as_float(pack_bf16x2(0.f, x) & 0xffff0000u); }
+template <> __device__ __forceinline__ float round_op<f16_t>(float x) { return f16_lo(pack_f16x2(x, 0.f)); }
+template <typename TM> __device__ __forceinline__ u32x4_t aux_chunk(float e0, float e1);
+template <> __device__ __forceinline__ u32x4_t aux_chunk<float>(float e0, float e1) { return u32x4_t{__float_as_uint(e0), __float_as_uint(e1), 0u, 0u}; }
+template <> __device__ __forceinline__ u32x4_t aux_chunk<bf16_t>(float e0, float e1) { return u32x4_t{pack_bf16x2(e0, e1), 0u, 0u, 0u}; }
+template <> __device__ __forceinline__ u32x4_t aux_chunk<f16_t>(float e0, float e1) { return u32x4_t{pack_f16x2(e0, e1), 0u, 0u, 0u}; }
+template <typename TM> __device__ __forceinline__ TM op_from_float(float x);
+template <> __device__ __forceinline__ float op_from_float<float>(float x) { return x; }
+template <> __device__ __forceinline__ bf16_t op_from_float<bf16_t>(float x) { bf16_t r; r.v = (uint16_t)pack_bf16x2(x, 0.f); return r; }
+template <> __device__ __forceinline__ f16_t op_from_float<f16_t>(float x) { f16_t r; r.v = (uint16_t)pack_f16x2(x, 0.f); return r; }
+
+__device__ __forceinline__ uint32_t pack_fp8x4(float a, float b, float c, float d) {
+  int v = __builtin_amdgcn_cvt_pk_fp8_f32(a, b, 0, false);
+  v = __builtin_amdgcn_cvt_pk_fp8_f32(c, d, v, true);
+  return (uint32_t)v;
+}
+typedef int i32x8_t __attribute__((ext_vector_type(8)));
+#ifndef NS2VC_ATTN_OPT
+#define NS2VC_ATTN_OPT 1
+#endif
+template <bool B> struct OptTag { static constexpr bool value = B; };
+__device__ __forceinline__ int vpos8(int key) { return ((key & 4) << 3) | ((key & 32) >> 1) | ((key & 24) >> 1) | (key & 3); }
+
+template <typename TM, int HD, int KEYS, bool P8> struct AttnTile {
+  static constexpr int NSUB = KEYS / 32;
+  static constexpr int SZ = AMma<TM>::SZ;
+  static constexpr int EPC = 16 / SZ;
+  static constexpr int NS = HD * SZ / 32;
+  static constexpr int KROWB = HD * SZ + 48;
+  static constexpr int VSZ = P8 ? 1 : SZ;
+  static constexpr int VROWB = KEYS * VSZ + 16;
+  static constexpr int HDX = (HD + 1 + 31) / 32 * 32;
+  static constexpr int DT = HDX / 32;
+  static constexpr int NSL = SZ;
+  static constexpr int KBYTES = KEYS * KROWB, VBYTES = HDX * VROWB;
+  static constexpr int STAGE = KBYTES + VBYTES;
+  static constexpr int PPR = HD * SZ / 16;
+  static constexpr int NPIECE = KEYS * PPR;
+  static constexpr float THRESH = P8 ? 8.0f : 12.0f;
+  static constexpr float OPT_MARGIN = 4.0f;
+  static constexpr bool CINIT = HD == 16 && SZ == 2 && !P8;
+  static constexpr int LB = HD / 32, LR = ((HD % 32) / 8) * 4;
+  static_assert(HD % 32 == 0 || HD % 32 == 16, "ones row must sit at row 0 or 16 of its 32-row block");
+
+  __device__ static __forceinline__ void store_k_piece(char* Ks, int u, const u32x4_t& raw) {
+    const int key = u / PPR, pc = u - key * PPR;
+    *reinterpret_cast<u32x4_t*>(Ks + key * KROWB + pc * 16) = raw;
+  }
+  __device__ static __forceinline__ void store_v_piece(char* Vs, int u, const u32x4_t& w) {
+    const int key = u % KEYS, pc = u / KEYS;
+    if constexpr (P8) {
+      const uint32_t b0 = pack_fp8x4(Op16<TM>::lo(w.x), Op16<TM>::hi(w.x), Op16<TM>::lo(w.y), Op16<TM>::hi(w.y));
+      const uint32_t b1 = pack_fp8x4(Op16<TM>::lo(w.z), Op16<TM>::hi(w.z), Op16<TM>::lo(w.w), Op16<TM>::hi(w.w));
+      uint8_t* vp = reinterpret_cast<uint8_t*>(Vs + (pc * EPC) * VROWB + vpos8(key));
+#pragma unroll
+      for (int j = 0; j < 4; ++j) { vp[j * VROWB] = (uint8_t)(b0 >> (8 * j)); vp[(4 + j) * VROWB] = (uint8_t)(b1 >> (8 * j)); }
+    } else {
+      const int pos = (key & ~31) + AMma<TM>::vpos(key & 31);
+      vt_scatter<TM>(Vs + (pc * EPC) * VROWB + pos * SZ, VROWB, w);
+    }
+  }
+
+  template <bool O>
+  __device__ static __forceinline__ void step(const char* Ks, const char* Vs, const int t, const bool cform, const u32x4_t (&qf)[NS], u32x4_t& qaux,
+                                              f32x16_t& cinit, float& m_ref, f32x16_t (&o)[DT], const int l31, const int hi) {
+    f32x16_t s[NSUB];
+    if (CINIT && cform) {
+#pragma unroll
+      for (int k2 = 0; k2 < NSUB; ++k2) {
+        const char* kr = Ks + (k2 * 32 + l31) * KROWB + hi * 16;
+        s[k2] = cinit;
+#pragma unroll
+        for (int sl = 0; sl < NS; ++sl) AMma<TM>::mma(s[k2], *reinterpret_cast<const u32x4_t*>(kr + sl * 32), qf[sl]);
+      }
+    } else {
+#pragma unroll
+    for (int k2 = 0; k2 < NSUB; ++k2) {
+      const char* kr = Ks + (k2 * 32 + l31) * KROWB + hi * 16;
+      s[k2] = AMma<TM>::mma0(*reinterpret_cast<const u32x4_t*>(kr + NS * 32), qaux);
+#pragma unroll
+      for (int sl = 0; sl < NS; ++sl) AMma<TM>::mma(s[k2], *reinterpret_cast<const u32x4_t*>(kr + sl * 32), qf[sl]);
+    }
+    }
+    if (!O || t == 0) {
+      float mx = s[0][0];
+#pragma unroll
+      for (int k2 = 0; k2 < NSUB; ++k2)
+#pragma unroll
+        for (int r = 0; r < 16; ++r) mx = fmaxf(mx, s[k2][r]);
+      mx = half_max(mx);
+      if (t == 0 || __any(mx > THRESH)) {
+        float target = t == 0 ? mx : fmaxf(mx, 0.f);
+        if (!(target > -INFINITY)) target = 0.f;
+        if (O) target += OPT_MARGIN;
+        const float m_new = round_op<TM>(m_ref + target);
+        const float dsh = m_new - m_ref;
+        if (t > 0) {
+          const float alpha = __builtin_amdgcn_exp2f(-dsh);
+#pragma unroll
+          for (int d = 0; d < DT; ++d)
+#pragma unroll
+            for (int r = 0; r < 16; ++r) o[d][r] *= alpha;
+        }
+#pragma unroll
+        for (int k2 = 0; k2 < NSUB; ++k2)
+#pragma unroll
+          for (int r = 0; r < 16; ++r) s[k2][r] -= dsh;
+        m_ref = m_new;
+        if (hi == 0) qaux = aux_chunk<TM>(-m_ref, 1.0f);
+        if constexpr (CINIT) {
+#pragma unroll
+          for (int r = 0; r < 16; ++r) cinit[r] = -m_ref;
+        }
+      }
+    }
+#pragma unroll
+    for (int k2 = 0; k2 < NSUB; ++k2)
+#pragma unroll
+      for (int r = 0; r < 16; ++r) s[k2][r] = __builtin_amdgcn_exp2f(s[k2][r]);
+
+    if constexpr (P8) {
+      i32x8_t pf;
+#pragma unroll
+      for (int v = 0; v < 8; ++v)
+        pf[v] = (int)pack_fp8x4(s[v >> 2][4 * (v & 3) + 0], s[v >> 2][4 * (v & 3) + 1], s[v >> 2][4 * (v & 3) + 2], s[v >> 2][4 * (v & 3) + 3]);
+#pragma unroll
+      for (int d = 0; d < DT; ++d) {
+        const char* vr = Vs + (d * 32 + l31) * VROWB + hi * 32;
+        const u32x4_t v0 = *reinterpret_cast<const u32x4_t*>(vr), v1 = *reinterpret_cast<const u32x4_t*>(vr + 16);
+        const i32x8_t vf = {(int)v0.x, (int)v0.y, (int)v0.z, (int)v0.w, (int)v1.x, (int)v1.y, (int)v1.z, (int)v1.w};
+        o[d] = __builtin_amdgcn_mfma_scale_f32_32x32x64_f8f6f4(vf, pf, o[d], 0, 0, 0, 0x7f7f7f7f, 0, 0x7f7f7f7f);
+      }
+    } else {
+#pragma unroll
+    for (int k2 = 0; k2 < NSUB; ++k2) {
+#pragma unroll
+      for (int sl = 0; sl < NSL; ++sl) {
+        u32x4_t pf;
+        if constexpr (SZ == 4) {
+          pf = u32x4_t{__float_as_uint(s[k2][4 * sl + 0]), __float_as_uint(s[k2][4 * sl + 1]),
+                       __float_as_uint(s[k2][4 * sl + 2]), __float_as_uint(s[k2][4 * sl + 3])};
+        } else {
+          pf = u32x4_t{Op16<TM>::pack(s[k2][8 * sl + 0], s[k2][8 * sl + 1]), Op16<TM>::pack(s[k2][8 * sl + 2], s[k2][8 * sl + 3]),
+                       Op16<TM>::pack(s[k2][8 * sl + 4], s[k2][8 * sl + 5]), Op16<TM>::pack(s[k2][8 * sl + 6], s[k2][8 * sl + 7])};
+        }
+#pragma unroll
+        for (int d = 0; d < DT; ++d) {
+          const u32x4_t vf = *reinterpret_cast<const u32x4_t*>(Vs + (d * 32 + l31) * VROWB + k2 * 32 * SZ + sl * 32 + hi * 16);
+          AMma<TM>::mma(o[d], vf, pf);
+        }
+      }
+    }
+    }
+  }
+
+  __device__ static __forceinline__ void load_q(u32x4_t (&qf)[NS], const TM* qp, const float sc2, const int hi, const bool dead) {
+#pragma unroll
+    for (int s = 0; s < NS; ++s) {
+      const u32x4_t raw = *reinterpret_cast<const u32x4_t*>(qp + s * 2 * EPC + hi * EPC);
+      if constexpr (SZ == 4) {
+        qf[s] = u32x4_t{__float_as_uint(__uint_as_float(raw.x) * sc2), __float_as_uint(__uint_as_float(raw.y) * sc2),
+                        __float_as_uint(__uint_as_float(raw.z) * sc2), __float_as_uint(__uint_as_float(raw.w) * sc2)};
+      } else {
+        auto sc = [&](uint32_t w) __attribute__((always_inline)) { return Op16<TM>::pack(Op16<TM>::lo(w) * sc2, Op16<TM>::hi(w) * sc2); };
+        qf[s] = u32x4_t{sc(raw.x), sc(raw.y), sc(raw.z), sc(raw.w)};
+      }
+      if (dead) qf[s] = u32x4_t{0, 0, 0, 0};
+    }
+  }
+
+  __device__ static __forceinline__ void store_out(const f32x16_t (&o)[DT], TM* op, const int hi, const bool live, const bool padded) {
+    const auto lsw = __builtin_amdgcn_permlane32_swap(__float_as_uint(o[LB][LR]), __float_as_uint(o[LB][LR]), false, false);
+    const float l_tot = __uint_as_float(lsw[0]);
+    const float inv = 1.0f / l_tot;
+    if constexpr (SZ == 2) {
+#pragma unroll
+      for (int d = 0; d < DT; ++d)
+#pragma unroll
+        for (int gp = 0; gp < 2; ++gp) {
+          if (d * 32 + 16 * gp < HD) {
+            const uint32_t a0 = Op16<TM>::pack(o[d][8 * gp] * inv, o[d][8 * gp + 1] * inv), a1 = Op16<TM>::pack(o[d][8 * gp + 2] * inv, o[d][8 * gp + 3] * inv);
+            const uint32_t b0 = Op16<TM>::pack(o[d][8 * gp + 4] * inv, o[d][8 * gp + 5] * inv), b1 = Op16<TM>::pack(o[d][8 * gp + 6] * inv, o[d][8 * gp + 7] * inv);
+            const auto x0 = __builtin_amdgcn_permlane32_swap(a0, b0, false, false);
+            const auto x1 = __builtin_amdgcn_permlane32_swap(a1, b1, false, false);
+#if defined(NS2VC_ATTN_ABLATE_STORE)
+            asm volatile("" :: "v"(x0[0]), "v"(x1[0]), "v"(x0[1]), "v"(x1[1]));
+#else
+            if (live) *reinterpret_cast<u32x4_t*>(op + d * 32 + 8 * (2 * gp + hi)) = padded ? u32x4_t{0, 0, 0, 0} : u32x4_t{x0[0], x1[0], x0[1], x1[1]};
+#endif
+          }
+        }
+    } else if (live) {
+#pragma unroll
+      for (int d = 0; d < DT; ++d)
+#pragma unroll
+        for (int gq = 0; gq < 4; ++gq) {
+          const int d0 = d * 32 + 8 * gq + 4 * hi;
+          if (d0 < HD) store_op4<TM>(op + d0, padded ? 0.f : o[d][4 * gq] * inv, padded ? 0.f : o[d][4 * gq + 1] * inv, padded ? 0.f : o[d][4 * gq + 2] * inv,
+                                     padded ? 0.f : o[d][4 * gq + 3] * inv);
+        }
+    }
+  }
+};
+
+}
diff --git a/ns2vc_amd/csrc/attn_resident.hip b/ns2vc_amd/csrc/attn_resident.hip
--- /dev/null
+++ b/ns2vc_amd/csrc/attn_resident.hip
@@ -0,0 +1,192 @@
+#include "attn_common.h"
+#include "kernel_table.h"
+#include <atomic>
+
+namespace ns2vc {
+
+__device__ int g_attnres_exact_only = 0;
+
+constexpr int ATTNRES_LDS = 160 * 1024;
+constexpr int ATTNRES_WAVES = 16;
+constexpr int ATTNRES_MAX_QBLOCKS = 256;
+
+template <typename TM, int HD> struct AttnResGeom {
+  using G = AttnTile<TM, HD, 64, false>;
+  static constexpr int MAXT = ATTNRES_LDS / G::STAGE;
+  static constexpr int TPP = 1024 / G::NPIECE;
+  static constexpr int NPASS = (MAXT + TPP - 1) / TPP;
+  static_assert(1024 % G::NPIECE == 0 && MAXT * 64 <= 1024, "one thread per staged key row");
+};
+
+template <typename TM, int HD>
+__global__ __launch_bounds__(1024) void attnres_kernel(const AttnArgs a) {
+  op_mode_init<TM>();
+  using R = AttnResGeom<TM, HD>;
+  using G = typename R::G;
+  constexpr int KEYS = 64, SZ = G::SZ, EPC = G::EPC, NS = G::NS, KROWB = G::KROWB, VROWB = G::VROWB, DT = G::DT, KBYTES = G::KBYTES, STAGE = G::STAGE,
+                PPR = G::PPR, NPIECE = G::NPIECE, HDX = G::HDX;
+  constexpr int TPP = R::TPP, NPASS = R::NPASS;
+  static_assert(SZ == 2, "16-bit operand types");
+  extern __shared__ __attribute__((aligned(16))) char smem[];
+
+  const int tid = threadIdx.x, lane = tid & 63, wave = tid >> 6;
+  const int l31 = lane & 31, hi = lane >> 5;
+  int b, h;
+  {
+    const int nwg = gridDim.x, bid = blockIdx.x;
+    const int qn = nwg >> 3, rn = nwg & 7, xcd = bid & 7, idx = bid >> 3;
+    const int swz = (xcd < rn ? xcd * (qn + 1) : rn * (qn + 1) + (xcd - rn) * qn) + idx;
+    b = swz / a.H;
+    h = swz - b * a.H;
+  }
+  const int Lq = a.Lq, Lk = a.Lk;
+  const int ntile = (Lk + KEYS - 1) / KEYS;
+  const float LOG2E = 1.4426950408889634f;
+  const float sc2 = a.scale * LOG2E;
+
+  {
+    const TM* kbase = reinterpret_cast<const TM*>(a.k) + (size_t)b * Lk * a.ldk + h * HD;
+    const TM* vbase = reinterpret_cast<const TM*>(a.v) + (size_t)b * Lk * a.ldv + h * HD;
+    const float* bias = a.bias ? a.bias + (size_t)b * Lk : nullptr;
+    const int u = tid % NPIECE, tsub = tid / NPIECE;
+    u32x4_t kraw[NPASS], vraw[NPASS];
+#pragma unroll
+    for (int i = 0; i < NPASS; ++i) {
+      const int t = tsub + i * TPP;
+      if (t < ntile) {
+        {
+          const int key = u / PPR, pc = u - key * PPR;
+          const int kk = min(t * KEYS + key, Lk - 1);
+          kraw[i] = *reinterpret_cast<const u32x4_t*>(kbase + (size_t)kk * a.ldk + pc * EPC);
+        }
+        {
+          const int key = u % KEYS, pc = u / KEYS;
+          const int kk = min(t * KEYS + key, Lk - 1);
+          vraw[i] = *reinterpret_cast<const u32x4_t*>(vbase + (size_t)kk * a.ldv + pc * EPC);
+        }
+      }
+    }
+    float braw = 0.f;
+    const bool keyrow = tid < ntile * KEYS;
+    if (keyrow && bias) braw = bias[min(tid, Lk - 1)];
+    constexpr int NZC = (HDX - HD - 1) * (KEYS * SZ / 16);
+    for (int i = tid; i < ntile * NZC; i += 1024) {
+      const int t = i / NZC, r = i - t * NZC;
+      *reinterpret_cast<u32x4_t*>(smem + t * STAGE + KBYTES + (HD + 1 + r / 8) * VROWB + (r & 7) * 16) = u32x4_t{0, 0, 0, 0};
+    }
+    if (keyrow) {
+      const int st = tid / KEYS, key = tid - st * KEYS;
+      const float bl = tid < Lk ? (bias ? braw * LOG2E : 0.f) : -INFINITY;
+      char* aux = smem + st * STAGE + key * KROWB + HD * SZ;
+      *reinterpret_cast<u32x4_t*>(aux) = aux_chunk<TM>(1.0f, bl);
+      *reinterpret_cast<u32x4_t*>(aux + 16) = u32x4_t{0, 0, 0, 0};
+      *reinterpret_cast<u32x4_t*>(aux + 32) = u32x4_t{0, 0, 0, 0};
+      *reinterpret_cast<TM*>(smem + st * STAGE + KBYTES + HD * VROWB + key * SZ) = op_from_float<TM>(1.0f);
+    }
+#pragma unroll
+    for (int i = 0; i < NPASS; ++i) {
+      const int t = tsub + i * TPP;
+      if (t < ntile) {
+        G::store_k_piece(smem + t * STAGE, u, kraw[i]);
+        G::store_v_piece(smem + t * STAGE + KBYTES, u, vraw[i]);
+      }
+    }
+  }
+  __syncthreads();
+
+  const bool cform_all = G::CINIT && !a.bias;
+  const bool exact_only = !NS2VC_ATTN_OPT || g_attnres_exact_only || a.exact_only;
+  const int nqt = (Lq + 31) >> 5;
+  for (int qt = wave; qt < nqt; qt += ATTNRES_WAVES) {
+    const int q = qt * 32 + l31;
+    u32x4_t qf[NS];
+    G::load_q(qf, reinterpret_cast<const TM*>(a.q) + ((size_t)(b * Lq + min(q, Lq - 1)) * a.ldq + h * HD), sc2, hi, q >= Lq);
+    float m_ref;
+    u32x4_t qaux;
+    f32x16_t cinit, o[DT];
+    auto run = [&](auto optimistic) __attribute__((always_inline)) {
+      constexpr bool O = decltype(optimistic)::value;
+#pragma unroll
+      for (int d = 0; d < DT; ++d)
+#pragma unroll
+        for (int r = 0; r < 16; ++r) o[d][r] = 0.f;
+      m_ref = 0.f;
+      qaux = hi == 0 ? aux_chunk<TM>(-m_ref, 1.0f) : u32x4_t{0, 0, 0, 0};
+#pragma unroll
+      for (int r = 0; r < 16; ++r) cinit[r] = 0.f;
+      for (int t = 0; t < ntile; ++t) {
+        const char* Ks = smem + t * STAGE;
+        G::template step<O>(Ks, Ks + KBYTES, t, cform_all && (t + 1 < ntile || Lk % KEYS == 0), qf, qaux, cinit, m_ref, o, l31, hi);
+      }
+    };
+    if (!exact_only) {
+      run(OptTag<true>{});
+      const float lq = o[G::LB][G::LR];
+      const int bad = (hi == 0 && q < Lq && !(lq > 0.f && lq < 16384.f)) ? 1 : 0;
+      if (__any(bad)) {
+        if (lane == 0) *reinterpret_cast<uint32_t*>(smem + (qt >> 4) * KROWB + HD * SZ + 32 + ((qt >> 2) & 3) * 4) = 1u;
+        run(OptTag<false>{});
+      }
+    } else {
+      run(OptTag<false>{});
+    }
+    TM* op = reinterpret_cast<TM*>(a.out) + ((size_t)(b * Lq + min(q, Lq - 1)) * a.ldo + h * HD);
+    G::store_out(o, op, hi, q < Lq, false);
+  }
+
+  if (a.fallbacks && !exact_only) {
+    __syncthreads();
+    if (tid == 0) {
+      unsigned n = 0;
+      const int nqb = (Lq + 127) >> 7;
+      for (int j = 0; j < nqb; ++j) n += *reinterpret_cast<const uint32_t*>(smem + (j >> 2) * KROWB + HD * SZ + 32 + (j & 3) * 4);
+      if (n) atomicAdd(a.fallbacks, n);
+    }
+  }
+}
+
+#define NS2VC_ATTNRES_ROW(TM, PREC, HD) {kernel_key(PREC, HD), reinterpret_cast<const void*>(attnres_kernel<TM, HD>), (uint32_t)ATTNRES_LDS, 1024}
+static const KernelRow attnres_rows[] = {
+  NS2VC_ATTNRES_ROW(bf16_t, PREC_BF16, 16), NS2VC_ATTNRES_ROW(bf16_t, PREC_BF16, 32),
+  NS2VC_ATTNRES_ROW(f16_t, PREC_F16, 16), NS2VC_ATTNRES_ROW(f16_t, PREC_F16, 32),
+};
+#undef NS2VC_ATTNRES_ROW
+static const KernelTable k_attnres_table(attnres_rows);
+const KernelTable& attnres_kernel_table() { return k_attnres_table; }
+static int g_min_grid = 256;
+hipError_t init_attnres_attributes() {
+  int dev = 0, cus = 0;
+  if (hipGetDevice(&dev) == hipSuccess && hipDeviceGetAttribute(&cus, hipDeviceAttributeMultiprocessorCount, dev) == hipSuccess && cus > 0) g_min_grid = cus;
+  return set_lds_all(k_attnres_table);
+}
+
+void set_attnres_optimistic(int on) { const int v = on ? 0 : 1; (void)hipMemcpyToSymbol(HIP_SYMBOL(g_attnres_exact_only), &v, sizeof(v)); }
+
+static int g_resident_mode = -1;
+void set_attn_resident_mode(int mode) { g_resident_mode = mode; }
+
+static int resident_max_tiles(int head_dim, int prec) {
+  if (prec == PREC_BF16) return head_dim == 16 ? AttnResGeom<bf16_t, 16>::MAXT : head_dim == 32 ? AttnResGeom<bf16_t, 32>::MAXT : 0;
+  if (prec == PREC_F16) return head_dim == 16 ? AttnResGeom<f16_t, 16>::MAXT : head_dim == 32 ? AttnResGeom<f16_t, 32>::MAXT : 0;
+  return 0;
+}
+bool attention_resident_eligible(const AttnArgs& a, int head_dim, int prec, bool allow) {
+  if (!allow || g_resident_mode == 0) return false;
+  if (a.q_lens || a.k_lens || a.pv_fp8) return false;
+  if (!find(k_attnres_table, kernel_key(prec, head_dim))) return false;
+  if ((a.Lk + 63) / 64 > resident_max_tiles(head_dim, prec) || (a.Lq + 127) / 128 > ATTNRES_MAX_QBLOCKS) return false;
+  if (g_resident_mode == 1) return true;
+  return (long long)a.B * a.H >= g_min_grid;
+}
+
+static std::atomic<unsigned long long> g_resident_launches{0};
+unsigned long long attn_resident_launches() { return g_resident_launches.load(); }
+
+hipError_t launch_attention_resident(const AttnArgs& a, int head_dim, int prec, hipStream_t s) {
+  const KernelRow* row = find(k_attnres_table, kernel_key(prec, head_dim));
+  if (!row) return hipErrorInvalidValue;
+  ++g_resident_launches;
+  return launch(*row, dim3(a.B * a.H), s, a);
+}
+
+}
diff --git a/ns2vc_amd/csrc/common.h b/ns2vc_amd/csrc/common.h
--- a/ns2vc_amd/csrc/common.h
+++ b/ns2vc_amd/csrc/common.h
@@ -270,7 +270,13 @@
 bool gemm_masks_rows(const GemmArgs& g, int prec);
 bool gemm_uses_convts(const GemmArgs& g, int prec);
 int last_gemm_refusal_line();
-hipError_t launch_attention(const AttnArgs& a, int head_dim, int prec, hipStream_t s);
+hipError_t launch_attention(const AttnArgs& a, int head_dim, int prec, hipStream_t s, bool resident = true);
+bool attention_resident_eligible(const AttnArgs& a, int head_dim, int prec, bool allow);
+hipError_t launch_attention_resident(const AttnArgs& a, int head_dim, int prec, hipStream_t s);
+hipError_t init_attnres_attributes();
+void set_attn_resident_mode(int mode);
+unsigned long long attn_resident_launches();
+void set_attnres_optimistic(int on);
 bool attention_masks_rows(const AttnArgs& a, int head_dim, int prec);
 hipError_t init_gemm_attributes();
 bool convts_eligible(const GemmArgs& g, int prec);
diff --git a/ns2vc_amd/csrc/engine.cpp b/ns2vc_amd/csrc/engine.cpp
--- a/ns2vc_amd/csrc/engine.cpp
+++ b/ns2vc_amd/csrc/engine.cpp
@@ -43,7 +43,8 @@
   {"fork_temb", "NS2VC_FORK_TEMB", &ns2vc_unet::fork_temb}, {"exact_io", "NS2VC_EXACT_IO", &ns2vc_unet::exact_io},
   {"split_io", "NS2VC_SPLIT_IO", &ns2vc_unet::split_io}, {"masked_fuse", "NS2VC_MASKED_FUSE", &ns2vc_unet::masked_fuse},
   {"masked_attn", "NS2VC_MASKED_ATTN", &ns2vc_unet::masked_attn}, {"masked_rows", "NS2VC_MASKED_ROWS", &ns2vc_unet::masked_rows},
-  {"masked_ffn", "NS2VC_MASKED_FFN", &ns2vc_unet::masked_ffn}, {"masked_geglu", "NS2VC_MASKED_GEGLU", &ns2vc_unet::masked_geglu}};
+  {"masked_ffn", "NS2VC_MASKED_FFN", &ns2vc_unet::masked_ffn}, {"masked_geglu", "NS2VC_MASKED_GEGLU", &ns2vc_unet::masked_geglu},
+  {"attn_resident", "NS2VC_ATTN_RESIDENT", &ns2vc_unet::attn_resident}};
 static bool* option_ptr(ns2vc_unet* h, const char* name) {
   for (const auto& o : kOptions)
     if (!strcmp(name, o.name)) return &(h->*o.member);
diff --git a/ns2vc_amd/csrc/engine_internal.h b/ns2vc_amd/csrc/engine_internal.h
--- a/ns2vc_amd/csrc/engine_internal.h
+++ b/ns2vc_amd/csrc/engine_internal.h
@@ -194,6 +194,7 @@
   bool slice_rows = true;
   unsigned* ln_health = nullptr;
   bool attn_optimistic = true;
+  bool attn_resident = true;
   unsigned* attn_fallbacks = nullptr;
   unsigned long long coef_hash = 0;
   std::vector<ns2vc::Tap> taps;
diff --git a/ns2vc_amd/csrc/kernel_table.h b/ns2vc_amd/csrc/kernel_table.h
--- a/ns2vc_amd/csrc/kernel_table.h
+++ b/ns2vc_amd/csrc/kernel_table.h
@@ -50,5 +50,6 @@
 const KernelTable& ffn_kernel_table();
 const KernelTable& geglu_kernel_table();
 const KernelTable& rowchain_kernel_table();
+const KernelTable& attnres_kernel_table();
 
 }
diff --git a/ns2vc_amd/csrc/plan.cpp b/ns2vc_amd/csrc/plan.cpp
--- a/ns2vc_amd/csrc/plan.cpp
+++ b/ns2vc_amd/csrc/plan.cpp
@@ -260,7 +260,8 @@
       a.k_lens = cross_lens;
       if (!h->has_mask) a.bias = nullptr;
     }
-    add(name, [=](hipStream_t s) { return launch_attention(a, hd, pr, s); }, 2, 4.0 * B * a.H * (double)Lq * Lk * hd,
+    const bool resident = h->attn_resident;
+    add(name, [=](hipStream_t s) { return launch_attention(a, hd, pr, s, resident); }, 2, 4.0 * B * a.H * (double)Lq * Lk * hd,
         (double)opsz * B * a.H * hd * (2.0 * Lq + 2.0 * Lk));
     if (!self_mask) mask(name, out, ldo, a.H * hd, opsz, Lq);
   }
```

Result: faster. 284.7 denoiser-steps/s (batch 32 per GPU, whole job), median of 6 (+1.3%).
